# adobe-research/DiffusionHandles

Measured on AMD Instinct MI355X. Metric: guided-denoise steps/sec at 512x512 (SD2-depth), higher is better.
Workload: dtype f16; 1 GPU; single 512x512 edit per GPU, SD2-depth (865.9M params, seeded random weights), guided phase: 3 x (fwd + energy + bwd-to-latent) + CFG fwd (B=2) + DDIM step; resolution=512, edits_per_gpu=1, correspondences=24906, parallelism=independent edits, one process per GPU, no collectives

## Files before the change

diffusionhandles_amd/_lib.py:

```python
import ctypes
import os

import torch

_HERE = os.path.dirname(os.path.abspath(__file__))
LIB_PATH = os.environ.get("DIFFHANDLES_LIB") or os.path.join(_HERE, "libdiffhandles_hip.so")
_LIB = None

c_p = ctypes.c_void_p
c_i = ctypes.c_int
c_f = ctypes.c_float
c_d = ctypes.c_double
c_sz = ctypes.c_size_t


class UNetConfig(ctypes.Structure):
    _fields_ = [("in_channels", c_i), ("out_channels", c_i), ("n_levels", c_i),
                ("block_out_channels", c_i * 4), ("layers_per_block", c_i), ("heads", c_i * 4),
                ("cross_attention_dim", c_i), ("norm_groups", c_i), ("sample_size", c_i),
                ("text_len", c_i), ("max_batch", c_i), ("dtype", c_i), ("max_diff_batch", c_i)]


class VAEConfig(ctypes.Structure):
    _fields_ = [("latent_channels", c_i), ("out_channels", c_i), ("block_out_channels", c_i * 4),
# ... 46 lines not shown
    "dh_vae_decoder_create": (c_i, [c_p, ctypes.POINTER(c_p)]),
    "dh_vae_decoder_destroy": (None, [c_p]),
    "dh_vae_decoder_num_params": (c_i, [c_p]),
    "dh_vae_decoder_param_info": (c_i, [c_p, c_i, ctypes.POINTER(ctypes.c_char_p), ctypes.POINTER(c_i),
                                        ctypes.POINTER(ctypes.c_int64)]),
    "dh_vae_decoder_load_param": (c_i, [c_p, c_i, c_p, c_p]),
    "dh_vae_decoder_bytes": (c_sz, [c_p]),
    "dh_vae_decoder_decode": (c_i, [c_p, c_p, c_i, c_p, c_p]),
    "dh_vae_encoder_create": (c_i, [c_p, ctypes.POINTER(c_p)]),
    "dh_vae_encoder_encode": (c_i, [c_p, c_p, c_i, c_p, c_p]),
    "dh_text_encoder_create": (c_i, [c_p, ctypes.POINTER(c_p)]),
    "dh_text_encoder_destroy": (None, [c_p]),
    "dh_text_encoder_num_params": (c_i, [c_p]),
    "dh_text_encoder_param_info": (c_i, [c_p, c_i, ctypes.POINTER(ctypes.c_char_p), ctypes.POINTER(c_i),
                                         ctypes.POINTER(ctypes.c_int64)]),
    "dh_text_encoder_load_param": (c_i, [c_p, c_i, c_p, c_p]),
    "dh_text_encoder_bytes": (c_sz, [c_p]),
    "dh_text_encoder_encode": (c_i, [c_p, c_p, c_i, c_i, c_p, c_p]),
    "dh_gemm_profile_begin": (c_i, []),
    "dh_gemm_profile_end": (c_i, [ctypes.POINTER(c_d), ctypes.POINTER(ctypes.c_int64), ctypes.POINTER(c_d)]),
    "dh_gemm_profile_bytes": (c_i, [ctypes.POINTER(c_d)]),
    "dh_ddim_cfg_step": (c_i, [c_p, c_p, c_p, c_p, c_f, c_f, c_f, c_i, c_p]),
    "dh_latent_update": (c_i, [c_p, c_p, c_p, c_f, c_f, c_i, c_p]),
    "dh_adam_step": (c_i, [c_p, c_p, c_p, c_p, c_f, c_f, c_f, c_f, c_i, c_i, c_p]),
    "dh_mse_fwd_bwd": (c_i, [c_p, c_p, c_i, c_p, c_p, c_p]),
    "dh_latent_update_strided": (c_i, [c_p, c_p, c_p, c_i, c_i, c_f, c_f, c_i, c_p]),
    "dh_pack_sample": (c_i, [c_p, c_p, c_i, c_i, c_p, c_i, c_i, c_i, c_i, c_p]),
    "dh_unet_io_ptr": (c_i, [c_p, c_i, c_i, ctypes.POINTER(c_p), ctypes.POINTER(c_sz)]),
    "dh_mse_cotangent": (c_i, [c_p, c_p, c_i, c_f, c_f, c_p, c_p, c_p, c_p]),
    "dh_adam_step_scaled": (c_i, [c_p, c_p, c_p, c_p, c_p, c_f, c_f, c_f, c_f, c_i, c_i, c_p]),
    "dh_mse_cotangent_batch": (c_i, [c_p, c_p, c_i, c_i, c_f, c_f, c_d, c_p, c_p, c_p, c_p, c_p, c_p]),
    "dh_adam_step_scaled_batch": (c_i, [c_p, c_p, c_p, c_p, c_p, c_p, c_f, c_f, c_f, c_f, c_i, c_i, c_i, c_p]),
    "dh_latent_update_guarded": (c_i, [c_p, c_p, c_p, c_i, c_i, c_f, c_i, c_i, c_p, c_i, c_i, c_p, c_p, c_i, c_i, c_p]),
    "dh_ddim_cfg_step_flagged": (c_i, [c_p, c_p, c_p, c_p, c_f, c_f, c_f, c_i, c_i, c_p, c_i, c_i, c_p]),
}

c_l = ctypes.c_long
DEBUG_SIGNATURES = {
    "dh_dbg_gemm": (c_i, [c_i, c_p, c_l, c_p, c_i, c_i, c_i, c_i, c_i, c_i, c_i, c_i, c_i, c_i, c_i, c_p, c_p, c_i, c_i,
                          c_p, c_l, c_p, c_l, c_i, c_p, c_sz, c_p]),
    "dh_dbg_gemm_groupnorm": (c_i, [c_i, c_p, c_l, c_p, c_i, c_i, c_i, c_i, c_i, c_i, c_i, c_p, c_p, c_p, c_sz, c_i, c_i, c_p, c_p, c_f, c_i,
                                    c_p, c_p, c_p, ctypes.POINTER(c_i), c_p]),
    "dh_dbg_gemm_groupnorm_bwd": (c_i, [c_i, c_p, c_l, c_p, c_i, c_i, c_i, c_i, c_i, c_i, c_i, c_p, c_p, c_sz, c_i, c_i, c_p, c_p, c_p, c_p, c_i,
                                        c_p, c_p, ctypes.POINTER(c_i), c_p]),
    "dh_dbg_gemm_groupnorm_res": (c_i, [c_i, c_p, c_l, c_p, c_i, c_i, c_i, c_i, c_i, c_i, c_i, c_p, c_p, c_l, c_p, c_p, c_sz, c_i, c_i, c_p, c_p,
                                    c_f, c_i, c_p, c_p, c_p, ctypes.POINTER(c_i), c_p]),
    "dh_dbg_gemm_groupnorm_bwd_res": (c_i, [c_i, c_p, c_l, c_p, c_i, c_i, c_i, c_i, c_i, c_i, c_i, c_p, c_l, c_p, c_p, c_sz, c_i, c_i, c_p, c_p, c_p,
                                        c_p, c_i, c_p, c_p, ctypes.POINTER(c_i), c_p]),
    "dh_dbg_concat_groupnorm": (c_i, [c_i, c_p, c_i, c_p, c_i, c_p, c_i, c_i, c_i, c_p, c_p, c_f, c_i, c_p, c_p, c_p, c_p]),
    "dh_dbg_gemm_last_tile": (c_i, [ctypes.POINTER(c_i)]),
    "dh_dbg_unet_concat_ops": (c_i, [ctypes.POINTER(UNetConfig), ctypes.POINTER(c_i), c_i, ctypes.POINTER(c_i)]),
    "dh_dbg_gemm_lnfold": (c_i, [c_i, c_p, c_l, c_p, c_i, c_i, c_i, c_p, c_p, c_p, c_f, c_p, c_l, c_p]),
    "dh_dbg_gemm_glu": (c_i, [c_i, c_i, c_p, c_l, c_p, c_i, c_i, c_i, c_p, c_p, c_p, c_p, c_p, c_p]),
    "dh_dbg_gemm_family": (c_i, [c_i]),
    "dh_dbg_gemm_stage": (c_i, [c_i]),
    "dh_dbg_gemm_pp_variant": (c_i, [c_i, c_p]),
    "dh_dbg_gemm_pp_ablate": (c_i, [c_i]),
    "dh_dbg_gemm_pp_persist": (c_i, [c_i]),
    "dh_dbg_gemm_pp_glu": (c_i, [c_i]),
    "dh_dbg_gemm_pp_plan": (c_i, [c_i, c_i, c_i, c_i, c_i, c_i, c_sz, ctypes.POINTER(c_i), ctypes.POINTER(c_i), ctypes.POINTER(c_i)]),
    "dh_dbg_touch_tiled": (c_i, [c_sz, c_p]),
    "dh_dbg_groupnorm": (c_i, [c_i, c_p, c_p, c_p, c_p, c_p, c_p, c_p, c_p, c_i, c_i, c_i, c_i, c_f, c_i, c_i, c_p]),
    "dh_dbg_layernorm": (c_i, [c_i, c_p, c_p, c_p, c_p, c_p, c_p, c_p, c_p, c_i, c_i, c_f, c_p]),
    "dh_dbg_geglu": (c_i, [c_i, c_p, c_p, c_p, c_p, c_i, c_i, c_p]),
    "dh_dbg_attention": (c_i, [c_i, c_p, c_l, c_p, c_p, c_l, c_p, c_l, c_p, c_p, c_p, c_p, c_p, c_p, c_i, c_i, c_i, c_i, c_p]),
    "dh_dbg_attention_bwd_pair": (c_i, [c_i, c_p, c_l, c_p, c_p, c_l, c_p, c_l, c_p, c_p, c_p, c_p, c_p, c_p, c_i, c_i, c_i, c_i, c_p, c_p]),
    "dh_dbg_pool2x2": (c_i, [c_i, c_p, c_p, c_i, c_i, c_i, c_i, c_i, c_p]),
    "dh_dbg_ellipse_offsets": (c_i, [c_i, ctypes.POINTER(ctypes.c_int32), c_i, ctypes.POINTER(c_i)]),
    "dh_dbg_lane_ops": (c_i, [c_p, c_p, c_p, c_p]),
}


def lib():
    global _LIB
    if _LIB is None:
        if not os.path.exists(LIB_PATH):
            raise RuntimeError(
                f"native HIP library not found at {LIB_PATH}; build it with "
                "`python -c 'import __graft_entry__ as g; g.build()'` (there is no CPU fallback)")
        handle = ctypes.CDLL(LIB_PATH)
        missing = []
        for name, (res, args) in list(SIGNATURES.items()) + list(DEBUG_SIGNATURES.items()):
            try:
                fn = getattr(handle, name)
            except AttributeError:
                missing.append(name)
                continue
            fn.restype = res
            fn.argtypes = args
        handle.dh_missing_symbols = missing
        for env, fn in (("DH_GEMM_FAMILY", "dh_dbg_gemm_family"), ("DH_PP_GLU", "dh_dbg_gemm_pp_glu"),
                        ("DH_PP_PERSIST", "dh_dbg_gemm_pp_persist"), ("DH_GEMM_STAGE", "dh_dbg_gemm_stage")):
            if os.environ.get(env) and fn not in missing:
                getattr(handle, fn)(int(os.environ[env]))
        _LIB = handle
    return _LIB


def check(rc, what=""):
    if rc != 0:
        raise RuntimeError(f"{what} failed ({rc}): {lib().dh_last_error().decode()}")


def require_gpu(t=None):
    if not torch.cuda.is_available():
        raise RuntimeError("diffusionhandles_amd needs a HIP device (MI355X); there is no CPU fallback")
# ... 15 lines not shown
```

diffusionhandles_amd/csrc/debug_api.cpp:

```cpp
#include <stdlib.h>

#include "unet_kernels.h"
using namespace dh;

static void* g_dbg_tiled = nullptr;

__global__ void k_dbg_touch(const uint4* p, size_t n16, unsigned* sink) {
  unsigned acc = 0;
  for (size_t i = (size_t)blockIdx.x * blockDim.x + threadIdx.x; i < n16; i += (size_t)gridDim.x * blockDim.x) { const uint4 v = p[i]; acc ^= v.x ^ v.y ^ v.z ^ v.w; }
  if (acc == 0x9e3779b9u && sink) sink[0] = acc;
}
extern "C" int dh_dbg_touch_tiled(size_t bytes, void* stream) {
  DH_REQUIRE(g_dbg_tiled != nullptr, "no tiled weights yet (call dh_dbg_gemm first)");
  hipLaunchKernelGGL(k_dbg_touch, dim3(512), dim3(256), 0, (hipStream_t)stream, (const uint4*)g_dbg_tiled, bytes / 16, (unsigned*)nullptr);
  DH_LAUNCH_CHECK();
  return DH_OK;
}

extern "C" int dh_dbg_gemm(int dtype, const void* A, long lda, const void* W, int M, int N, int K, int mode, int Hin,
                           int Win, int Cin, int Hout, int Wout, int stride, int up, const float* bias,
                           const float* rowvec, int rowvec_ld, int rows_per_batch, const void* R, long ldr, void* C,
                           long ldc, int act_silu, float* partial, size_t partial_elems, void* stream) {
  DH_REQUIRE(A && W && C && K % 64 == 0 && N % 64 == 0, "bad arguments (N, K must be multiples of 64)");
  void*& tiled = g_dbg_tiled;
// ... 83 lines not shown
                                         const float* gamma, const float* beta, const float* stats, int silu, void* dx,
                                         float* scratch, int* have_out, void* stream) {
  return dh_dbg_gemm_groupnorm_bwd_res(dtype, A, lda, W, M, N, K, mode, Hin, Win, Cin, nullptr, N, C, partial, partial_elems, HW, G, x,
                                       gamma, beta, stats, silu, dx, scratch, have_out, stream);
}
extern "C" int dh_dbg_concat_groupnorm(int dtype, const void* a, int Ca, const void* b, int Cb, void* out, int B, int HW, int G,
                                       const float* gamma, const float* beta, float eps, int silu, void* Y, float* stats,
                                       float* scratch, void* stream) {
  DH_REQUIRE(a && b && out && Y && stats && scratch && gamma && beta && B > 0 && HW > 0 && G > 0, "bad arguments");
  DH_REQUIRE(Ca % 8 == 0 && Cb % 8 == 0 && (Ca + Cb) % G == 0 && (GN_GB * ((Ca + Cb) / G)) % 8 == 0 && GN_GB * ((Ca + Cb) / G) <= 2048,
             "shape the fused concatenation does not take");
  launch_concat_gn(dtype, a, Ca, b, Cb, out, scratch, B, HW, G, (hipStream_t)stream);
  launch_groupnorm_fwd(dtype, out, gamma, beta, Y, stats, scratch, B, HW, Ca + Cb, G, eps, silu, (hipStream_t)stream, 1);
  DH_LAUNCH_CHECK();
  return DH_OK;
}
extern "C" int dh_dbg_gemm_lnfold(int dtype, const void* A, long lda, const void* W, int M, int N, int K, const float* ln_s,
                                  const float* ln_t, float* ln_stats, float ln_eps, void* C, long ldc, void* stream) {
  DH_REQUIRE(A && W && C && ln_s && ln_t && ln_stats && K % 64 == 0 && N % 64 == 0, "bad arguments (N, K must be multiples of 64)");
  static void* tiled = nullptr;
  static size_t tiled_cap = 0;
  const size_t need = (size_t)N * K * 2;
  if (need > tiled_cap) {
    if (tiled) (void)hipFree(tiled);
    DH_CHECK_HIP(hipMalloc(&tiled, need));
    tiled_cap = need;
  }
  launch_tile_weights(dtype, W, tiled, N, K, (hipStream_t)stream);
  GemmArgs g;
  g.A = A; g.lda = lda; g.W = tiled; g.M = M; g.N = N; g.K = K; g.mode = A_DENSE; g.C = C; g.ldc = ldc;
  g.ln_s = ln_s; g.ln_t = ln_t; g.ln_stats = ln_stats; g.ln_eps = ln_eps;
  launch_gemm(dtype, g, (hipStream_t)stream);
  DH_LAUNCH_CHECK();
  return DH_OK;
}
extern "C" int dh_dbg_gemm_glu(int dtype, int bwd, const void* A, long lda, const void* W, int M, int N, int K, const float* bias,
                               void* C, void* y, const void* x, void* dx, void* stream) {
  DH_REQUIRE(A && W && K % 64 == 0 && N % 128 == 0, "bad arguments (K % 64, N % 128)");
  DH_REQUIRE(bwd ? (x && dx) : (y != nullptr), "missing output");
  static void* tiled = nullptr;
  static size_t tiled_cap = 0;
  const size_t need = (size_t)N * K * 2;
  if (need > tiled_cap) {
    if (tiled) (void)hipFree(tiled);
    DH_CHECK_HIP(hipMalloc(&tiled, need));
    tiled_cap = need;
  }
  launch_tile_weights(dtype, W, tiled, N, K, (hipStream_t)stream);
  GemmArgs g;
  g.A = A; g.lda = lda; g.W = tiled; g.M = M; g.N = N; g.K = K; g.mode = A_DENSE; g.bias = bias;
  if (bwd) { g.glub_x = x; g.glub_dx = dx; }
  else { g.C = C; g.ldc = N; g.glu_y = y; g.glu_ldy = N / 2; }
  launch_gemm(dtype, g, (hipStream_t)stream);
  DH_LAUNCH_CHECK();
  return DH_OK;
}
extern "C" int dh_dbg_groupnorm(int dtype, const void* x, const float* gamma, const float* beta, void* y, float* stats,
                                const void* dy, void* dx, float* scratch, int B, int HW, int C, int G, float eps,
                                int silu, int accumulate, void* stream) {
  launch_groupnorm_fwd(dtype, x, gamma, beta, y, stats, scratch, B, HW, C, G, eps, silu, (hipStream_t)stream);
  if (dy && dx)
    launch_groupnorm_bwd(dtype, x, dy, gamma, beta, stats, dx, scratch, B, HW, C, G, silu, accumulate, (hipStream_t)stream);
  DH_LAUNCH_CHECK();
  return DH_OK;
}
extern "C" int dh_dbg_layernorm(int dtype, const void* x, const float* gamma, const float* beta, void* y, float* stats,
                                const void* dy, const void* add, void* dx, int rows, int C, float eps, void* stream) {
  launch_layernorm_fwd(dtype, x, gamma, beta, y, stats, rows, C, eps, (hipStream_t)stream);
  if (dy && dx) launch_layernorm_bwd(dtype, x, dy, gamma, stats, add, dx, rows, C, (hipStream_t)stream);
  DH_LAUNCH_CHECK();
  return DH_OK;
}
extern "C" int dh_dbg_geglu(int dtype, const void* x, void* y, const void* dy, void* dx, int rows, int F, void* stream) {
  launch_geglu_fwd(dtype, x, y, rows, F, (hipStream_t)stream);
  if (dy && dx) launch_geglu_bwd(dtype, x, dy, dx, rows, F, (hipStream_t)stream);
  DH_LAUNCH_CHECK();
  return DH_OK;
}
extern "C" int dh_dbg_attention(int dtype, const void* q, long ldq, const void* k, const void* v, long ldk, void* o,
                                long ldo, float* lse, const void* d_o, float* delta, void* dq, void* dk, void* dv,
                                int B, int H, int Nq, int Nk, void* stream) {
  hipStream_t st = (hipStream_t)stream;
  launch_attention_fwd(dtype, q, ldq, k, v, ldk, o, ldo, lse, B, H, Nq, Nk, st);
  if (d_o) {
    if (dq) launch_attention_bwd_dq(dtype, q, ldq, k, v, ldk, o, ldo, d_o, ldo, lse, delta, dq, ldq, B, H, Nq, Nk, st);
    else launch_attention_delta(dtype, o, ldo, d_o, ldo, delta, B, H, Nq, st);
    if (dk && dv) {
      static float* scratch = nullptr;
      constexpr size_t kScratch = (size_t)16 << 20;
      if (!scratch && hipMalloc((void**)&scratch, kScratch * sizeof(float)) != hipSuccess) scratch = nullptr;
      launch_attention_bwd_dkv(dtype, q, ldq, k, v, ldk, d_o, ldo, lse, delta, dk, dv, ldk, B, H, Nq, Nk, st, scratch,
                               scratch ? kScratch : 0);
    }
  }
  DH_LAUNCH_CHECK();
  return DH_OK;
}
extern "C" int dh_dbg_attention_bwd_pair(int dtype, const void* q, long ldq, const void* k, const void* v, long ldk, const void* o,
                                         long ldo, const float* lse, const void* d_o, float* delta, void* dq, void* dk, void* dv,
                                         int B, int H, int Nq, int Nk, void* stream, void* stream2) {
  hipStream_t st = (hipStream_t)stream, s2 = (hipStream_t)stream2;
  if (!s2) {
    launch_attention_bwd_dq(dtype, q, ldq, k, v, ldk, o, ldo, d_o, ldo, lse, delta, dq, ldq, B, H, Nq, Nk, st);
    launch_attention_bwd_dkv(dtype, q, ldq, k, v, ldk, d_o, ldo, lse, delta, dk, dv, ldk, B, H, Nq, Nk, st, nullptr, 0);
  } else {
    static hipEvent_t fork = nullptr, join = nullptr;
// ... 23 lines not shown
```

diffusionhandles_amd/csrc/gemm.hip:

```cpp
#include <stdlib.h>

#include <vector>

#include <hip/hip_ext.h>

#include "gemm_k.h"

namespace dh {

struct GemmProf {
  bool on = false;
  std::vector<hipEvent_t> ev;
  size_t used = 0;
  double flops = 0;
  double bytes = 0;
  hipEvent_t e0 = nullptr, e1 = nullptr;
};
static GemmProf g_prof;
static int g_buf_stage = 1;
static int g_pp_force = 0;
struct GemmTileReport {
  int bm, bn, kg, stages, mw, splits, pp, gn_epi, reduce_gn;
};
static thread_local GemmTileReport g_last_tile;
// ... 295 lines not shown
          sy = ty >> 1; sx = tx >> 1;
        }
        sy = sy < 0 ? 0 : (sy >= p.Hin ? p.Hin - 1 : sy);
        sx = sx < 0 ? 0 : (sx >= p.Win ? p.Win - 1 : sx);
        const T* ptr = Ag + (a_off[j] + (long)sy * p.Win + sx) * p.lda + c0 + lchunk * 8;
        dma16(ok ? ptr : zero, sbase + (j * WG + grp) * (NWV * 1024));
      }
    } else {
      const int j = q - NPA;
#ifdef DH_TUNING
      if (p.w_nt) dma16_nt(b_ptr[j] + (size_t)(k0 >> 6) * 4096, sbase + BM * 128 + (j * WG + grp) * (NWV * 1024));
      else
#endif
      dma16(b_ptr[j] + (size_t)(k0 >> 6) * 4096, sbase + BM * 128 + (j * WG + grp) * (NWV * 1024));
    }
  };
  auto next_tile = [&]() {
    if constexpr (BUF && MODE == GM_CONV_S1) {
      ++tap; ++bs_kx;
      const bool row_end = bs_kx == 3;
      bs_tap += row_end ? bs_step_row : bs_step_px;
      bs_kx = row_end ? 0 : bs_kx;
      if (tap == 9) { tap = 0; c0 += BK; bs_tap = (unsigned)c0 * 2u; }
      bs_sh = 31u - (unsigned)tap;
      return;
    }
    if (MODE != GM_DENSE) { if (++tap == 9) { tap = 0; c0 += BK; } }
  };
  auto issue = [&](int kt, int stage) {
#pragma unroll
    for (int q = 0; q < NP; ++q) issue_piece(kt, stage, q);
    next_tile();
  };

  v16f acc[TM][TN];
#pragma unroll
  for (int i = 0; i < TM; ++i)
#pragma unroll
    for (int j = 0; j < TN; ++j)
#pragma unroll
      for (int r = 0; r < 16; ++r) acc[i][j][r] = 0.f;

  const int wn_u = __builtin_amdgcn_readfirstlane(wn);
  float ln1[TM], ln2[TM];
#pragma unroll
  for (int i = 0; i < TM; ++i) { ln1[i] = 0.f; ln2[i] = 0.f; }

#pragma unroll
  for (int s = 0; s < ST - 1; ++s)
    if (s < ntiles) issue(s, s);
  DH_STAMP(1);

  constexpr bool PRE = TM * TN <= 8;
  const bool pre_r = PRE && p.R != nullptr && p.pre_r && p.splits == 1 && (WG == 1 || grp == 0) && (KG == 1 || kg == 0);
  constexpr bool PRE_B = PRE && !(MW == 2 && BN == 320) && WNS == 2;
  const bool pre_b = PRE_B && p.bias != nullptr && p.pre_r && p.splits == 1;
  float4 bpre[PRE_B ? TN : 1][4];
  if (pre_b) {
#pragma unroll
    for (int j = 0; j < TN; ++j)
#pragma unroll
      for (int g = 0; g < 4; ++g) {
        const int n = n0 + wn * CPW + j * 32 + 8 * g + 4 * hi;
        bpre[PRE_B ? j : 0][g] = n < p.N ? *reinterpret_cast<const float4*>(p.bias + n) : make_float4(0.f, 0.f, 0.f, 0.f);
      }
  }
  constexpr bool PRE_LN = LNF && PRE && !(MW == 2 && BM == 256);
  float4 lsp[PRE_LN ? TN : 1][4], ltp[PRE_LN ? TN : 1][4];
  if (PRE_LN) {
#pragma unroll
    for (int j = 0; j < TN; ++j)
#pragma unroll
      for (int g = 0; g < 4; ++g) {
        const int n = n0 + wn * CPW + j * 32 + 8 * g + 4 * hi;
        lsp[PRE_LN ? j : 0][g] = n < p.N ? *reinterpret_cast<const float4*>(p.ln_s + n) : make_float4(0.f, 0.f, 0.f, 0.f);
        ltp[PRE_LN ? j : 0][g] = n < p.N ? *reinterpret_cast<const float4*>(p.ln_t + n) : make_float4(0.f, 0.f, 0.f, 0.f);
      }
  }
  constexpr bool GNB = gn_epi_bwd_tile(BM, BN, WG, GLU, LNF);
  static_assert(!GNB || (PRE && WNS == 2), "the backward form carries the GroupNorm input tile in the residual's prefetch registers");
  const bool gnb = GNB && p.gn_epi == 2 && p.splits == 1;
  const bool pre_x = gnb && (KG == 1 || kg == 0);
  float4 gnb_col = make_float4(0.f, 0.f, 0.f, 0.f);
  if (GNB && pre_x && tid < BN) {
    const int n = n0 + tid, grp_n = (int)(((float)n + 0.5f) / (float)p.gn_cpg);
    const float2 st2 = *reinterpret_cast<const float2*>(p.gnb_stats + 2 * ((m0 / p.gn_HW) * p.gn_G + grp_n));
    gnb_col = make_float4(p.gnb_gamma[n], p.gnb_beta[n], st2.x, st2.y);
  }
  uint2 rpre[TM][TN][4];
  if (pre_r || pre_x) {
    const T* rsrc = reinterpret_cast<const T*>(pre_x ? p.gnb_x : p.R);
    const long rld = pre_x ? p.gnb_ldx : p.ldr;
#pragma unroll
    for (int i = 0; i < TM; ++i) {
      const int m = m0 + wm * RPW + i * 32 + ln;
#pragma unroll
      for (int j = 0; j < TN; ++j)
#pragma unroll
        for (int g = 0; g < 4; ++g) {
          const int n = n0 + wn * CPW + j * 32 + 8 * g + 4 * hi;
          rpre[i][j][g] = (m < p.M && n < p.N) ? *reinterpret_cast<const uint2*>(rsrc + (size_t)m * rld + n) : make_uint2(0, 0);
        }
    }
  }

  constexpr int KK = BK / 16 / WG;
  const int kk0 = grp * KK;
// ... 132 lines not shown
          acc[i][j][4 * g + 2] = rstd * (acc[i][j][4 * g + 2] - mean * sv.z) + tv.z;
          acc[i][j][4 * g + 3] = rstd * (acc[i][j][4 * g + 3] - mean * sv.w) + tv.w;
        }
    }
  }


  if constexpr (GLU == 1) {
    typedef T T4 __attribute__((ext_vector_type(4)));
    const bool hb = p.bias != nullptr;
    T* Y = reinterpret_cast<T*>(p.glu_y);
#pragma unroll
    for (int i = 0; i < TM; ++i) {
      const int m = m0 + wm * RPW + i * 32 + ln;
      if (m >= p.M) continue;
#pragma unroll
      for (int j = 0; j < TN; ++j) {
        const int nb = n0 + wn * CPW + j * 32;
        if (nb >= p.N) continue;
        uint2 w[4];
        float pv[4][4];
#pragma unroll
        for (int g = 0; g < 4; ++g) {
          float v0 = acc[i][j][4 * g], v1 = acc[i][j][4 * g + 1], v2 = acc[i][j][4 * g + 2], v3 = acc[i][j][4 * g + 3];
          if (hb) {
            float4 b = bpre[PRE_B ? j : 0][g];
            if (!pre_b) b = *reinterpret_cast<const float4*>(p.bias + nb + 8 * g + 4 * hi);
            v0 += b.x; v1 += b.y; v2 += b.z; v3 += b.w;
          }
          T4 o;
          o[0] = from_f32<T>(v0); o[1] = from_f32<T>(v1); o[2] = from_f32<T>(v2); o[3] = from_f32<T>(v3);
          w[g] = __builtin_bit_cast(uint2, o);
#pragma unroll
          for (int c = 0; c < 4; ++c) pv[g][c] = to_f32<T>(o[c]);
        }
        if (p.C) {
          T* out = reinterpret_cast<T*>(p.C) + (size_t)m * p.ldc + nb + 8 * hi;
          *reinterpret_cast<uint4*>(out) = half_exchange(w[0], w[1]);
          *reinterpret_cast<uint4*>(out + 16) = half_exchange(w[2], w[3]);
        }
        uint2 y[2];
#pragma unroll
        for (int q = 0; q < 2; ++q) {
          T4 o;
#pragma unroll
          for (int c = 0; c < 4; ++c) o[c] = from_f32<T>(pv[q][c] * gelu_f(pv[q + 2][c]));
          y[q] = __builtin_bit_cast(uint2, o);
        }
        *reinterpret_cast<uint4*>(Y + (size_t)m * p.glu_ldy + (nb >> 1) + 8 * hi) = half_exchange(y[0], y[1]);
      }
    }
    return;
  }
  if constexpr (GLU == 2) {
    typedef T T4 __attribute__((ext_vector_type(4)));
    const T* X = reinterpret_cast<const T*>(p.glub_x);
    T* DX = reinterpret_cast<T*>(p.glub_dx);
    const size_t ldx = 2 * (size_t)p.N;
    uint4 Hc[TM][TN][2], Gc[TM][TN][2];
#pragma unroll
    for (int i = 0; i < TM; ++i) {
      const int m = m0 + wm * RPW + i * 32 + ln;
      const int mc = m < p.M ? m : p.M - 1;
#pragma unroll
      for (int j = 0; j < TN; ++j) {
        int nb = n0 + wn * CPW + j * 32;
        if (nb >= p.N) nb = 0;
#pragma unroll
        for (int q = 0; q < 2; ++q) {
          const T* src = X + (size_t)mc * ldx + 2 * nb + 32 * q + 8 * hi;
          Hc[i][j][q] = *reinterpret_cast<const uint4*>(src);
          Gc[i][j][q] = *reinterpret_cast<const uint4*>(src + 16);
        }
      }
    }
#pragma unroll
    for (int i = 0; i < TM; ++i) {
      const int m = m0 + wm * RPW + i * 32 + ln;
      if (m >= p.M) continue;
#pragma unroll
      for (int j = 0; j < TN; ++j) {
        const int nb = n0 + wn * CPW + j * 32;
        if (nb >= p.N) continue;
#pragma unroll
        for (int q = 0; q < 2; ++q) {
          const uint4 hc = Hc[i][j][q], gc = Gc[i][j][q];
          const uint4 hx = half_exchange(make_uint2(hc.x, hc.y), make_uint2(hc.z, hc.w));
          const uint4 gx = half_exchange(make_uint2(gc.x, gc.y), make_uint2(gc.z, gc.w));
          uint2 dh[2], dg[2];
#pragma unroll
          for (int s2 = 0; s2 < 2; ++s2) {
            const int g = 2 * q + s2;
            const T4 hh = __builtin_bit_cast(T4, s2 ? make_uint2(hx.z, hx.w) : make_uint2(hx.x, hx.y));
            const T4 gg = __builtin_bit_cast(T4, s2 ? make_uint2(gx.z, gx.w) : make_uint2(gx.x, gx.y));
            T4 oh, og;
#pragma unroll
            for (int c = 0; c < 4; ++c) {
              const float dy = acc[i][j][4 * g + c], gate = to_f32<T>(gg[c]);
              const GeluParts gp = gelu_parts(gate);
              oh[c] = from_f32<T>(dy * gate * gp.Phi);
              og[c] = from_f32<T>(dy * to_f32<T>(hh[c]) * fmaf(gate, gp.pdf, gp.Phi));
            }
            dh[s2] = __builtin_bit_cast(uint2, oh);
            dg[s2] = __builtin_bit_cast(uint2, og);
          }
          T* dst = DX + (size_t)m * ldx + 2 * nb + 32 * q + 8 * hi;
          *reinterpret_cast<uint4*>(dst) = half_exchange(dh[0], dh[1]);
          *reinterpret_cast<uint4*>(dst + 16) = half_exchange(dg[0], dg[1]);
        }
      }
    }
    return;
  }
  DH_STAMP(5);
  constexpr bool GNE = gn_epi_fwd_tile(BN, GLU, LNF);
  const bool gn_epi = GNE && p.splits == 1 && (p.gn_epi == 1 || (GNB && p.gn_epi == 2));
  static_assert(!GNE || NWV * CPW * 4 <= KG * ST * STAGE - 4096, "the pivot table lies below the column-sum scratch");
  float* gpt = reinterpret_cast<float*>(smem_all) + wave * CPW;
  if (GNE && gn_epi && !(GNB && gnb)) __syncthreads();
  float gsa[GNE ? TN : 1][16], gsq[GNE ? TN : 1][16];
  if (GNE) {
#pragma unroll
    for (int j = 0; j < (GNE ? TN : 1); ++j)
#pragma unroll
      for (int r = 0; r < 16; ++r) { gsa[j][r] = 0.f; gsq[j][r] = 0.f; }
  }
  auto gn_acc = [&](int i, int j, int g, uint2 packed) {
    if constexpr (GNE) {
      typedef T T4g __attribute__((ext_vector_type(4)));
      const T4g ov = __builtin_bit_cast(T4g, packed);
      float v[4], pv[4];
#pragma unroll
      for (int c = 0; c < 4; ++c) v[c] = to_f32<T>(ov[c]);
      float4* pt = reinterpret_cast<float4*>(gpt + j * 32 + 8 * g + 4 * hi);
      if (i == 0) {
#pragma unroll
// ... 422 lines not shown
  } else if (gm == GM_CONV_S1) {
    DH_GEMM_LAUNCH((k_gemm_dma<T, BM, BN, ST, GM_CONV_S1, 0, WG, KG, MW, false, 0, BUF>));
  } else {
    DH_GEMM_LAUNCH((k_gemm_dma<T, BM, BN, ST, GM_GENERIC, 0, WG, KG, MW>));
  }
}
template <class T, int BM, int BN, int ST, int WG, int KG, int MW>
static void launch_tile(int gm, bool lnf, dim3 grid, hipStream_t st, const GemmK& k, int glu = 0) {
  g_last_tile.bm = BM; g_last_tile.bn = BN; g_last_tile.kg = KG; g_last_tile.stages = ST; g_last_tile.mw = MW;
  if (k.pp_a_bytes != 0 && gm != GM_GENERIC) launch_tile_b<T, BM, BN, ST, WG, KG, MW, true>(gm, lnf, grid, st, k, glu);
  else launch_tile_b<T, BM, BN, ST, WG, KG, MW, false>(gm, lnf, grid, st, k, glu);
}
#undef DH_GEMM_LAUNCH

#ifdef DH_TUNING
#define DH_KNOB(name, env, dflt) static const int name = getenv(env) ? atoi(getenv(env)) : (dflt)
#else
#define DH_KNOB(name, env, dflt) constexpr int name = (dflt)
#endif

template <class T>
static void gemm_dispatch(GemmK k, size_t partial_elems, hipStream_t st, int* gn_done, int* lnb_done, int dtype) {
  DH_KNOB(kSplitTiles, "DH_SPLITK_TILES", 200);
  DH_KNOB(kSplitMinK, "DH_SPLITK_MINKT", 32);
  DH_KNOB(kSplitTarget, "DH_SPLITK_TARGET", 256);
  DH_KNOB(kBigTiles, "DH_BIG_TILES", 128);
  DH_KNOB(kNarrowTiles, "DH_NARROW_TILES", 40);
  DH_KNOB(kN320, "DH_GEMM_N320", 224);
  DH_KNOB(kMwBlocks, "DH_GEMM_MW", 64);
  DH_KNOB(kKg2MinKt, "DH_KG2_MINKT", 4);
  DH_KNOB(kManyBlocks, "DH_GEMM_MANY", 512);
  DH_KNOB(kMw128, "DH_GEMM_MW128", 1);
  DH_KNOB(kTwoPerCu, "DH_GEMM_TWO_PER_CU", 1);
#ifdef DH_TUNING
  DH_KNOB(kWnt, "DH_W_NT", 0);
#endif
  const bool lnf = k.ln_s != nullptr;
  g_last_tile = GemmTileReport{};
  int BM = 128, BN = (k.N % 128 == 0) ? 128 : 64;
  const int ktiles = k.K / BK;
  PpPlan pp;
  const bool use_pp = gemm_pp_plan(k, partial_elems, g_pp_force, &pp);
  if (BN == 128 && ktiles >= 16 && cdiv(k.M, 128) * cdiv(k.N, 128) <= kNarrowTiles) BN = 64;
  if (k.M <= 64 || (cdiv(k.M, 128) * cdiv(k.N, BN) < kBigTiles && ktiles < kSplitMinK)) { BM = 64; BN = 64; }
  const bool n320 = kN320 > 0 && k.N % 320 == 0 && k.N <= 960 && !lnf && BM == 128 && BN == 64 && cdiv(k.M, 128) >= kN320;
  if (n320) BN = 320;
  DH_KNOB(kMwShortK, "DH_GEMM_MW_SHORTK", 128);
  const long tiles256 = (long)cdiv(k.M, 256) * cdiv(k.N, 128);
  const bool mw2 = kMwBlocks > 0 && k.N % 128 == 0 && tiles256 >= kMwBlocks &&
                   !(k.M <= 256 && k.M > 128 && cdiv(k.N, 128) < 128) && (tiles256 >= kMwShortK || ktiles >= kSplitMinK);
  if (mw2) { BM = 256; BN = 128; }
  const int glu = k.glu_y ? 1 : (k.glub_x ? 2 : 0);
  if (glu && !(BM == 64 && BN == 64)) { BM = mw2 ? 256 : 128; BN = 128; }
  DH_KNOB(kT160, "DH_GEMM_T160", 224);
  const long tiles160 = (long)cdiv(k.M, 128) * (k.N / 160);
  const bool t160 = kT160 > 0 && k.N % 160 == 0 && !lnf && !glu && !n320 && BM != 64 && tiles160 >= kT160 && tiles160 <= 256;
  if (t160) { BM = 128; BN = 160; }
  if (use_pp) { BM = pp.bm; BN = pp.bn; }
  const int tm = cdiv(k.M, BM), tn = cdiv(k.N, BN), tiles = tm * tn;
  int splits = 1;
  if (use_pp) splits = pp.splits;
  else if (k.partial && !lnf && !glu && tiles < kSplitTiles && ktiles >= kSplitMinK) {
    splits = kSplitTarget / tiles;
    if (splits > ktiles / 4) splits = ktiles / 4;
    if (splits > 32) splits = 32;
    const size_t fit = partial_elems / ((size_t)k.M * k.N);
    if ((size_t)splits > fit) splits = (int)fit;
    if (splits < 1) splits = 1;
  }
#ifdef DH_TUNING
  static const int kLog = getenv("DH_GEMM_LOG") ? atoi(getenv("DH_GEMM_LOG")) : 0;
  const int kForceTile = getenv("DH_FORCE_TILE") ? atoi(getenv("DH_FORCE_TILE")) : 0;
  const int kForceSplits = getenv("DH_FORCE_SPLITS") ? atoi(getenv("DH_FORCE_SPLITS")) : 0;
  int force_tile = 0;
  if (kForceTile && !use_pp && !(k.glu_y || k.glub_x)) {
    const int fbm = kForceTile == 1 ? 64 : (kForceTile == 6 ? 256 : 128), fbn = kForceTile == 7 ? 160 : ((kForceTile <= 3) ? 64 : 128);
    if ((k.N % fbn == 0 || fbn == 64) && !(fbn == 160 && lnf)) { BM = fbm; BN = fbn; force_tile = kForceTile; }
  }
  if (kForceSplits && !use_pp && k.partial && !lnf) {
    splits = kForceSplits;
    if (splits > ktiles / 2) splits = ktiles / 2 > 0 ? ktiles / 2 : 1;
    const size_t fit = partial_elems / ((size_t)k.M * k.N);
    if ((size_t)splits > fit) splits = (int)fit;
    if (splits < 1) splits = 1;
  }
  if (kLog) fprintf(stderr, "GEMMLOG M=%d N=%d K=%d mode=%d lnf=%d gn=%d gnb=%d bias=%d R=%d rowvec=%d | pp=%d BM=%d BN=%d splits=%d\n", k.M, k.N, k.K,
                    k.mode == A_DENSE ? 0 : (k.mode == A_CONV3 && k.stride == 1 && k.up == 0 ? 1 : 2), (int)lnf, k.gn_part != nullptr,
                    k.gnb_x != nullptr, k.bias != nullptr, k.R != nullptr, k.rowvec != nullptr, (int)use_pp, BM, BN, splits);
#endif
  const int tiles_per_split = cdiv(ktiles, splits);
  splits = cdiv(ktiles, tiles_per_split);
  k.splits = splits;
  k.k_per_split = tiles_per_split * BK;
  k.gn_epi = 0; k.gn_cpg = 0;
  if ((g_buf_stage & 4) == 0 && splits == 1 && !use_pp && gn_epi_fwd_tile(BN, glu, lnf) && k.gn_part && !k.gnb_x && gn_done && k.gn_G > 0 &&
      k.gn_HW > 0 && k.C && k.wide_store && k.M % k.gn_HW == 0 && k.gn_HW % BM == 0 && k.N % k.gn_G == 0 && k.N % BN == 0) {
    const int cpg = k.N / k.gn_G, sx = 2 * (k.gn_HW / BM);
    if (cpg >= 8 && cpg <= BN && sx <= 64) { k.gn_epi = 1; k.gn_cpg = cpg; k.gn_S = sx; }
  }
  if ((g_buf_stage & 8) == 0 && splits == 1 && !use_pp && gn_epi_bwd_tile(BM, BN, 1, glu, lnf) && k.gn_part && k.gnb_x && gn_done && k.gn_G > 0 &&
      k.gn_HW > 0 && k.C && k.wide_store && k.pre_r && !k.R && !k.bias && !k.rowvec && !k.act_silu && k.M % k.gn_HW == 0 && k.gn_HW % BM == 0 &&
      k.N % k.gn_G == 0 && k.N % BN == 0 && (((size_t)k.gnb_x | (size_t)(k.gnb_ldx * 2)) & 7) == 0) {
    const int cpg = k.N / k.gn_G, sx = 2 * (k.gn_HW / BM);
    if (cpg >= 8 && cpg <= BN && sx <= 64) { k.gn_epi = 2; k.gn_cpg = cpg; k.gn_S = sx; }
  }
#ifdef DH_TUNING
  k.w_nt = kWnt > 0 && tm <= kWnt;
  static const int kLnfAbl = getenv("DH_LNF_ABL") ? atoi(getenv("DH_LNF_ABL")) : 0;
  k.lnf_abl = kLnfAbl;
  k.ts = g_gemm_ts;
#endif
#ifdef DH_TUNING
  dim3 grid(force_tile ? cdiv(k.M, BM) : tm, force_tile ? cdiv(k.N, BN) : tn, splits);
#else
  dim3 grid(tm, tn, splits);
#endif
  hipEvent_t e0 = nullptr, e1 = nullptr;
  if (g_prof.on) {
    if (g_prof.used + 2 > g_prof.ev.size()) {
      const size_t old = g_prof.ev.size();
      g_prof.ev.resize(old + 4096);
      for (size_t i = old; i < g_prof.ev.size(); ++i) (void)hipEventCreate(&g_prof.ev[i]);
    }
    e0 = g_prof.ev[g_prof.used++];
    e1 = g_prof.ev[g_prof.used++];
    g_prof.flops += 2.0 * (double)k.M * (double)k.N * (double)k.K;
    const double esz = 2.0;
    double a_elems = (double)k.M * k.K;
    if (k.mode != A_DENSE && k.Hout > 0 && k.Wout > 0) a_elems = (double)k.M / ((double)k.Hout * k.Wout) * k.Hin * k.Win * k.Cin;
    double c_elems = (double)k.M * k.N * (k.C ? 1.0 : 0.0) + (k.R ? (double)k.M * k.N : 0.0);
    if (k.glu_y) c_elems += 0.5 * (double)k.M * k.N;
    if (k.glub_x) c_elems += 4.0 * (double)k.M * k.N;
    if (k.gn_epi == 2) c_elems += (double)k.M * k.N;
    g_prof.bytes += esz * (a_elems + (double)k.N * k.K + c_elems);
    g_prof.e0 = e0; g_prof.e1 = e1;
  }
  int gm = GM_GENERIC;
  if (k.mode == A_DENSE) gm = GM_DENSE;
  else if (k.mode == A_CONV3 && k.stride == 1 && k.up == 0 && k.pad == 1) gm = GM_CONV_S1;
  if (!use_pp) {
    k.pp_a_bytes = 0; k.pp_w_bytes = 0;
    size_t ab = 0;
    if (k.mode == A_DENSE) ab = ((size_t)(k.M - 1) * k.lda + k.K) * 2;
    else if (k.Hout > 0 && k.Wout > 0 && k.M % (k.Hout * k.Wout) == 0)
      ab = (size_t)(k.M / (k.Hout * k.Wout)) * k.Hin * k.Win * (size_t)k.lda * 2;
    const size_t wb = (size_t)align_up((size_t)k.N, 64) * k.K * 2;
    const bool conv_ok = k.mode == A_DENSE || (k.Cin % 64 == 0 && k.K == 9 * k.Cin);
    if ((g_buf_stage & 1) && ab > 0 && conv_ok && ab + (size_t)(k.Win + 1) * k.lda * 2 < 0x7ff00000ull && wb < 0x7ff00000ull && k.lda % 8 == 0 &&
        ((size_t)k.A & 15) == 0 && ((size_t)k.W & 15) == 0) {
      k.pp_a_bytes = (unsigned)ab; k.pp_w_bytes = (unsigned)wb;
    }
  }
#ifdef DH_TUNING
  static const int kAbl = getenv("DH_GEMM_ABLATE") ? atoi(getenv("DH_GEMM_ABLATE")) : 0;
  if (kAbl == 1 && BM == 128 && BN == 128) { hipLaunchKernelGGL((k_gemm_dma<T, 128, 128, 4, GM_CONV_S1, 1>), grid, dim3(256), 0, st, k); }
  else if (kAbl == 2 && BM == 128 && BN == 128) { hipLaunchKernelGGL((k_gemm_dma<T, 128, 128, 4, GM_CONV_S1, 2>), grid, dim3(256), 0, st, k); }
  else if (kAbl == 3 && BM == 128 && BN == 128) { hipLaunchKernelGGL((k_gemm_dma<T, 128, 128, 4, GM_DENSE, 1>), grid, dim3(256), 0, st, k); }
  else if (kAbl == 1 && mw2 && gm == GM_CONV_S1) { hipLaunchKernelGGL((k_gemm_dma<T, 256, 128, 3, GM_CONV_S1, 1, 1, 1, 2>), grid, dim3(512), 0, st, k); }
  else if (kAbl == 2 && mw2 && gm == GM_CONV_S1) { hipLaunchKernelGGL((k_gemm_dma<T, 256, 128, 3, GM_CONV_S1, 2, 1, 1, 2>), grid, dim3(512), 0, st, k); }
  else if (kAbl == 1 && mw2 && gm == GM_DENSE && !lnf) { hipLaunchKernelGGL((k_gemm_dma<T, 256, 128, 3, GM_DENSE, 1, 1, 1, 2>), grid, dim3(512), 0, st, k); }
  else if (kAbl == 2 && mw2 && gm == GM_DENSE && !lnf) { hipLaunchKernelGGL((k_gemm_dma<T, 256, 128, 3, GM_DENSE, 2, 1, 1, 2>), grid, dim3(512), 0, st, k); }
  else if (force_tile == 1) launch_tile<T, 64, 64, 4, 1, 1, 1>(gm, lnf, grid, st, k);
  else if (force_tile == 2) launch_tile<T, 128, 64, 3, 1, 2, 1>(gm, lnf, grid, st, k);
  else if (force_tile == 3) launch_tile<T, 128, 64, 5, 1, 1, 1>(gm, lnf, grid, st, k);
  else if (force_tile == 4) launch_tile<T, 128, 128, 4, 1, 1, 2>(gm, lnf, grid, st, k);
  else if (force_tile == 5) launch_tile<T, 128, 128, 4, 1, 1, 1>(gm, lnf, grid, st, k);
  else if (force_tile == 6) launch_tile<T, 256, 128, 3, 1, 1, 2>(gm, lnf, grid, st, k);
  else if (force_tile == 7) launch_tile<T, 128, 160, 4, 1, 1, 1>(gm, false, grid, st, k);
  else
#endif
  if (use_pp) { pp.splits = splits; g_last_tile.bm = pp.bm; g_last_tile.bn = pp.bn; launch_gemm_pp(dtype, k, pp, st, g_prof.e0, g_prof.e1); }
  else if (t160) launch_tile<T, 128, 160, 4, 1, 1, 1>(gm, false, grid, st, k);
  else if (mw2) launch_tile<T, 256, 128, 3, 1, 1, 2>(gm, lnf, grid, st, k, glu);
  else if (BM == 128 && BN == 128 && (glu || (kMw128 && tiles_per_split >= kMw128))) launch_tile<T, 128, 128, 4, 1, 1, 2>(gm, lnf, grid, st, k, glu);
  else if (kTwoPerCu && BM == 128 && BN == 64 && tiles * splits > 256 && tiles * splits <= 512)
    launch_tile<T, 128, 64, 3, 1, 1, 1>(gm, lnf, grid, st, k);
  else if (BM == 128 && BN == 64 && tiles_per_split >= kKg2MinKt) launch_tile<T, 128, 64, 3, 1, 2, 1>(gm, lnf, grid, st, k);
  else if (BN == 320) launch_tile<T, 128, 320, 2, 1, 1, 2>(gm, false, grid, st, k);
  else if (BM == 64) launch_tile<T, 64, 64, 4, 1, 1, 1>(gm, lnf, grid, st, k, glu);
  else if (BN == 128 && kManyBlocks > 0 && tiles * splits >= kManyBlocks) launch_tile<T, 128, 128, 2, 1, 1, 1>(gm, lnf, grid, st, k);
  else if (BN == 128) launch_tile<T, 128, 128, 4, 1, 1, 1>(gm, lnf, grid, st, k);
  else launch_tile<T, 128, 64, 5, 1, 1, 1>(gm, lnf, grid, st, k);
  g_prof.e0 = g_prof.e1 = nullptr;
  g_last_tile.splits = splits; g_last_tile.pp = use_pp ? 1 : 0; g_last_tile.gn_epi = k.gn_epi;
  if (k.gn_epi) *gn_done = k.gn_S;
  if (splits > 1) {
    if (k.gn_part && k.gn_G > 0 && k.gn_HW > 0 && k.N % k.gn_G == 0 && (GN_GB * (k.N / k.gn_G)) % 8 == 0 &&
        GN_GB * (k.N / k.gn_G) <= 2048 && k.M % k.gn_HW == 0) {
      k.gn_S = gn_slices(k.gn_HW, k.M / k.gn_HW);
      if (k.gnb_x) hipLaunchKernelGGL((k_splitk_reduce_gn<T, true>), dim3(k.gn_S, cdiv(k.gn_G, GN_GB), k.M / k.gn_HW), dim3(256), 0, st, k);
      else hipLaunchKernelGGL((k_splitk_reduce_gn<T, false>), dim3(k.gn_S, cdiv(k.gn_G, GN_GB), k.M / k.gn_HW), dim3(256), 0, st, k);
      g_last_tile.reduce_gn = 1;
      if (gn_done) *gn_done = 1;
    } else if (k.lnb_x && lnb_done && !k.bias && !k.rowvec && !k.R && !k.act_silu && k.N % 8 == 0 && k.ldc == k.N) {
      launch_splitk_reduce_ln_bwd(dtype, k.partial, splits, k.lnb_x, k.lnb_gamma, k.lnb_stats, k.lnb_add, k.lnb_dx, k.M, k.N, st);
      *lnb_done = 1;
    } else {
      const size_t groups = (size_t)k.M * k.N / 4;
      hipLaunchKernelGGL((k_splitk_reduce<T>), dim3((unsigned)((groups + 255) / 256)), dim3(256), 0, st, k);
    }
  }
}
#undef DH_KNOB

double launch_gemm(int dtype, const GemmArgs& a, hipStream_t st) {
  GemmK k;
  k.A = a.A; k.lda = a.lda; k.W = a.W; k.M = a.M; k.N = a.N; k.K = a.K;
  k.mode = a.mode; k.Hin = a.Hin; k.Win = a.Win; k.Cin = a.Cin; k.Hout = a.Hout; k.Wout = a.Wout;
  k.stride = a.stride; k.up = a.up; k.pad = a.pad;
  k.bias = a.bias; k.rowvec = a.rowvec; k.rowvec_ld = a.rowvec_ld;
  k.rows_per_batch = a.rows_per_batch > 0 ? a.rows_per_batch : 1;
  k.inv_rows_per_batch = 1.f / (float)k.rows_per_batch;
  k.R = a.R; k.ldr = a.ldr; k.C = a.C; k.ldc = a.ldc; k.act_silu = a.act_silu;
  k.partial = a.partial; k.splits = 1; k.k_per_split = a.K;
  k.pre_r = 1;
  k.wide_store = a.N % 32 == 0 && a.ldc % 8 == 0 && ((size_t)a.C & 15) == 0;
  k.ln_s = a.ln_s; k.ln_t = a.ln_t; k.ln_stats = a.ln_stats; k.ln_eps = a.ln_eps;
  k.gn_part = a.gn_part; k.gn_HW = a.gn_HW; k.gn_G = a.gn_G; k.gn_S = 0;
  k.gnb_x = a.gnb_x; k.gnb_ldx = a.gnb_ldx; k.gnb_gamma = a.gnb_gamma; k.gnb_beta = a.gnb_beta; k.gnb_stats = a.gnb_stats;
  k.gnb_silu = a.gnb_silu;
  k.lnb_x = a.lnb_x; k.lnb_gamma = a.lnb_gamma; k.lnb_stats = a.lnb_stats; k.lnb_add = a.lnb_add; k.lnb_dx = a.lnb_dx;
  k.glu_y = a.glu_y; k.glu_ldy = a.glu_ldy; k.glub_x = a.glub_x; k.glub_dx = a.glub_dx;
  if (a.gn_done) *a.gn_done = 0;
  if (a.lnb_done) *a.lnb_done = 0;
  if (dtype == DH_DTYPE_F16) gemm_dispatch<f16>(k, a.partial_elems, st, a.gn_done, a.lnb_done, dtype);
  else gemm_dispatch<bf16>(k, a.partial_elems, st, a.gn_done, a.lnb_done, dtype);
  return 2.0 * (double)a.M * (double)a.N * (double)a.K;
}

}

#ifdef DH_TUNING
extern "C" int dh_dbg_gemm_timeline(unsigned long long* ts) { dh::g_gemm_ts = ts; return DH_OK; }
#endif

extern "C" int dh_dbg_gemm_family(int force) {
  DH_REQUIRE(force >= 0 && force <= 2, "family: 0 policy, 1 k_gemm_dma, 2 k_gemm_pp");
  dh::g_pp_force = force;
  return DH_OK;
}

extern "C" int dh_dbg_gemm_stage(int buf) {
  dh::g_buf_stage = buf;
  return DH_OK;
}

extern "C" int dh_dbg_gemm_last_tile(int* out) {
  DH_REQUIRE(out != nullptr, "null pointer");
  const dh::GemmTileReport& r = dh::g_last_tile;
  const int v[9] = {r.bm, r.bn, r.kg, r.stages, r.mw, r.splits, r.pp, r.gn_epi, r.reduce_gn};
  for (int i = 0; i < 9; ++i) out[i] = v[i];
  return DH_OK;
}

extern "C" int dh_gemm_profile_begin(void) {
  dh::g_prof.on = true;
  dh::g_prof.used = 0;
  dh::g_prof.flops = 0;
  dh::g_prof.bytes = 0;
  return DH_OK;
}
extern "C" int dh_gemm_profile_bytes(double* bytes) {
  if (bytes) *bytes = dh::g_prof.bytes;
  return DH_OK;
}
extern "C" int dh_gemm_profile_end(double* ms_total, int64_t* launches, double* flops) {
  using namespace dh;
  g_prof.on = false;
  double ms = 0;
  if (g_prof.used >= 2) DH_CHECK_HIP(hipEventSynchronize(g_prof.ev[g_prof.used - 1]));
  for (size_t i = 0; i + 1 < g_prof.used; i += 2) {
    float t = 0;
    DH_CHECK_HIP(hipEventElapsedTime(&t, g_prof.ev[i], g_prof.ev[i + 1]));
    ms += t;
  }
// ... 6 lines not shown
```

diffusionhandles_amd/csrc/gemm_k.h:

```cpp
#pragma once
#include "unet_kernels.h"

namespace dh {

typedef _Float16 v8h __attribute__((ext_vector_type(8)));
typedef __bf16 v8b __attribute__((ext_vector_type(8)));
typedef float v16f __attribute__((ext_vector_type(16)));

template <class T> struct Mfma;
template <> struct Mfma<f16> {
  static __device__ __forceinline__ v16f run(uint4 a, uint4 b, v16f c) {
    return __builtin_amdgcn_mfma_f32_32x32x16_f16(__builtin_bit_cast(v8h, a), __builtin_bit_cast(v8h, b), c, 0, 0, 0);
  }
};
template <> struct Mfma<bf16> {
  static __device__ __forceinline__ v16f run(uint4 a, uint4 b, v16f c) {
    return __builtin_amdgcn_mfma_f32_32x32x16_bf16(__builtin_bit_cast(v8b, a), __builtin_bit_cast(v8b, b), c, 0, 0, 0);
  }
};

struct GemmK {
  const void* A; long lda;
  const void* W;
  int M, N, K;
  int mode, Hin, Win, Cin, Hout, Wout, stride, up, pad;
  const float* bias;
  const float* rowvec; int rowvec_ld; int rows_per_batch; float inv_rows_per_batch;
  const void* R; long ldr;
  void* C; long ldc;
  int act_silu;
  int pre_r;
  int wide_store;
#ifdef DH_TUNING
  int w_nt;
  unsigned long long* ts;
  int lnf_abl;
#endif
  const float* ln_s; const float* ln_t; float* ln_stats; float ln_eps;
  float* partial;
  int splits, k_per_split;
  float* gn_part; int gn_HW, gn_G, gn_S;
  int gn_epi, gn_cpg;
  const void* gnb_x; long gnb_ldx; const float *gnb_gamma, *gnb_beta, *gnb_stats; int gnb_silu;
  const void* lnb_x; const float *lnb_gamma, *lnb_stats; const void* lnb_add; void* lnb_dx;
  void* glu_y; long glu_ldy; const void* glub_x; void* glub_dx;
  int pp_tm, pp_tn, pp_order, pp_nwork; unsigned pp_a_bytes, pp_w_bytes;
  unsigned long long* pp_ts;
};


struct PpPlan { int bm = 0, bn = 0, splits = 1; };
bool gemm_pp_plan(const GemmK& k, size_t partial_elems, int force, PpPlan* plan);
void launch_gemm_pp(int dtype, const GemmK& k, const PpPlan& plan, hipStream_t st, hipEvent_t e0, hipEvent_t e1);

}
```

diffusionhandles_amd/csrc/gemm_pp.hip:

```cpp
#include <hip/hip_ext.h>

#include <type_traits>
#include <utility>

#include "gemm_k.h"

namespace dh {

typedef float v4f __attribute__((ext_vector_type(4)));
typedef int v4i __attribute__((ext_vector_type(4)));
typedef unsigned lane_u2p __attribute__((ext_vector_type(2)));

template <class T> struct Mfma16;
template <> struct Mfma16<f16> {
  typedef v8h frag;
  static __device__ __forceinline__ v4f run(frag a, frag b, v4f c) { return __builtin_amdgcn_mfma_f32_16x16x32_f16(a, b, c, 0, 0, 0); }
};
template <> struct Mfma16<bf16> {
  typedef v8b frag;
  static __device__ __forceinline__ v4f run(frag a, frag b, v4f c) { return __builtin_amdgcn_mfma_f32_16x16x32_bf16(a, b, c, 0, 0, 0); }
};

constexpr unsigned PP_OOB = 0x80000000u;

// ... 497 lines not shown
        *reinterpret_cast<uint2*>(ctail) = __builtin_bit_cast(uint2, o);
      }
      __builtin_amdgcn_sched_barrier(0);
      stamp();
    }
  };
  if (has_r) { if (hv_rows) rows(std::true_type{}, std::true_type{}); else rows(std::true_type{}, std::false_type{}); }
  else       { if (hv_rows) rows(std::false_type{}, std::true_type{}); else rows(std::false_type{}, std::false_type{}); }
  {
    constexpr int CPR = CPW / 8, NCH = RPW * CPR;
    static_assert(NCH % 64 == 0, "whole store instructions");
    T* cw = reinterpret_cast<T*>(p.C) + (size_t)(m0 + wm * RPW) * p.ldc + nb;
    const int mleft = p.M - (m0 + wm * RPW);
#pragma unroll
    for (int k = 0; k < NCH / 64; ++k) {
      const int c = 64 * k + lane_e, row = c / CPR, cc = c - row * CPR;
      const uint4 v = *reinterpret_cast<const uint4*>(stg + row * SPITCH + cc * 16);
      if (row < mleft) *reinterpret_cast<uint4*>(cw + (size_t)row * p.ldc + cc * 8) = v;
    }
  }
  stamp();
  }
}

static int pp_mode(const GemmK& k) {
  if (k.mode == A_DENSE) return PP_DENSE;
  if (k.mode == A_CONV3 && k.stride == 1 && k.up == 0 && k.pad == 1) return PP_CONV_S1;
  return PP_GENERIC;
}

static size_t pp_a_bytes(const GemmK& k) {
  if (k.mode == A_DENSE) return ((size_t)(k.M - 1) * k.lda + k.K) * 2;
  const size_t B = (size_t)k.M / ((size_t)k.Hout * k.Wout);
  return B * k.Hin * k.Win * (size_t)k.lda * 2;
}

static int pp_device_cus() {
  static int cus = 0;
  if (cus == 0) {
    int dev = 0, n = 0;
    if (hipGetDevice(&dev) == hipSuccess && hipDeviceGetAttribute(&n, hipDeviceAttributeMultiprocessorCount, dev) == hipSuccess && n >= 8) cus = n - n % 8;
    else { (void)hipGetLastError(); cus = 256; }
  }
  return cus;
}

static int g_pp_glu = -1;
bool gemm_pp_plan(const GemmK& k, size_t partial_elems, int force, PpPlan* plan) {
  if (force == 1) return false;
  if (k.ln_s || k.act_silu) return false;
  const int glu = k.glu_y ? 1 : (k.glub_x ? 2 : 0);
  const bool glu_here = force == 2 || g_pp_glu > 0 || (g_pp_glu < 0 && ((glu == 1 && k.M >= 2048) || k.M >= 32768));
  if (glu && !glu_here) return false;
  if (glu && (k.mode != A_DENSE || k.N % 128 || k.rowvec || k.R || (glu == 1 && (k.glu_ldy % 8 || ((size_t)k.glu_y & 15))) ||
              (glu == 2 && (((size_t)k.glub_x & 15) || ((size_t)k.glub_dx & 15))))) return false;
  if (k.rowvec && (k.rowvec_ld % 4 || ((size_t)k.rowvec & 15))) return false;
  if (k.K % 64 || k.M <= 0 || (!k.C && !glu)) return false;
  if (k.N % 160 && k.N % 128) return false;
  if (k.N % 64) return false;
  if (k.bias && ((size_t)k.bias & 15)) return false;
  if ((k.C && (k.ldc % 8 || ((size_t)k.C & 15))) || k.lda % 8 || ((size_t)k.A & 15) || ((size_t)k.W & 15)) return false;
  if (k.R && (k.ldr % 8 || ((size_t)k.R & 15))) return false;
  if (k.mode != A_DENSE && (k.Hout <= 0 || k.Wout <= 0 || k.M % (k.Hout * k.Wout) || k.Cin % 64 || k.K != 9 * k.Cin)) return false;
  const size_t ab = pp_a_bytes(k) + (size_t)(k.Win + 1) * k.lda * 2, wb = (size_t)k.N * k.K * 2;
  if (ab >= 0x7ff00000ull || wb >= 0x7ff00000ull) return false;
  const int ktiles = k.K / 64;
  const int bn = (k.N % 160 == 0 && !glu) ? 160 : 128;
  const int tn = k.N / bn;
  const long t256 = (long)cdiv(k.M, 256) * tn, t128 = (long)cdiv(k.M, 128) * tn;
  int bm = 0, splits = 1;
  const int cus = pp_device_cus(), fill = cus - cus / 8;
  if (t256 >= fill) bm = 256;
  else if (t128 >= fill) bm = 128;
  else if (!glu && k.partial && ktiles >= 64 && t256 >= 64 && k.M >= 1024 && k.M <= 4096) {
    bm = 256;
    splits = (int)(cus / t256);
    if (splits > ktiles / 8) splits = ktiles / 8;
    if (splits > 8) splits = 8;
    const size_t fit = partial_elems / ((size_t)k.M * k.N);
    if ((size_t)splits > fit) splits = (int)fit;
    if (splits < 2) bm = 0;
  }
  if (force == 2 && bm == 0) { bm = k.M > 128 ? 256 : 128; splits = 1; }
  if (bm == 0) return false;
  plan->bm = bm; plan->bn = bn; plan->splits = splits;
  return true;
}

constexpr int PP_SHIP_256 = PPV_K64 | (1 << PPV_NDIM_SHIFT), PP_SHIP_128 = PPV_K64 | (3 << PPV_NDIM_SHIFT);
static int g_pp_persist = 1;
static int g_pp_ablate = 0;
static int g_pp_variant = -1;
static unsigned long long* g_pp_ts = nullptr;

template <class T, int BM, int BN, int NST, int VAR>
static void pp_launch_tile(int mode, dim3 grid, hipStream_t st, const GemmK& k, hipEvent_t e0, hipEvent_t e1) {
#define DH_PP_LAUNCH(KERNEL)                                                                      \
  do {                                                                                            \
    if (e0) hipExtLaunchKernelGGL(KERNEL, grid, dim3(512), 0, st, e0, e1, 0, k);                  \
    else hipLaunchKernelGGL(KERNEL, grid, dim3(512), 0, st, k);                                   \
  } while (0)
  if constexpr (BN == 128 && VAR == (BM == 256 ? PP_SHIP_256 : PP_SHIP_128)) {
    if (k.glu_y) { DH_PP_LAUNCH((k_gemm_pp<T, BM, BN, PP_DENSE, NST, VAR, 1>)); return; }
    if (k.glub_x) { DH_PP_LAUNCH((k_gemm_pp<T, BM, BN, PP_DENSE, NST, VAR, 2>)); return; }
  }
  if (mode == PP_DENSE) DH_PP_LAUNCH((k_gemm_pp<T, BM, BN, PP_DENSE, NST, VAR>));
// ... 103 lines not shown
```

diffusionhandles_amd/csrc/unet_engine.cpp:

```cpp
#include <stdlib.h>

#include <algorithm>
#include <map>
#include <numeric>
#include <vector>

#include "unet_kernels.h"

namespace dh {

enum OpType { OP_CONV_IN, OP_CONV_OUT, OP_GEMM, OP_GN, OP_LN, OP_ATTN, OP_GEGLU, OP_CONCAT, OP_TIMESTEP, OP_T2F };
enum ParamKind { PK_F32, PK_MAT };

struct Ten {
  size_t off = 0, goff = 0;
  size_t off_fo = 0;
  int rows = 0, C = 0;
  bool req_grad = true;
  bool persistent = false;
};

struct Wt {
  size_t fwd_off = 0, bwd_off = 0;
  int N = 0, K = 0, taps = 1;
  bool has_bwd = true, f32 = false;
  int glu_F = 0;
};

struct ParamInfo {
  std::string name;
  int ndim = 0;
  int64_t shape[4] = {0, 0, 0, 0};
  int kind = PK_F32;
  size_t f32_off = 0;
  int wt = -1;
  int row_off = 0;
  int glu_F = 0;
};

struct Op {
  int type = OP_GEMM;
  int in0 = -1, in1 = -1, out = -1, res = -1;
  int wt = -1;
  long bias_off = -1;
  long gamma_off = -1, beta_off = -1;
  int mode = A_DENSE, Hin = 0, Win = 0, Cin = 0, Hout = 0, Wout = 0, stride = 1, up = 0;
  int in_col = 0, in_cols = 0;
  long rowvec_off = -1; int rowvec_ld = 0;
  int act_silu = 0;
  float eps = 1e-5f; int silu = 0; int groups = 32; size_t stats_off = 0;
  int heads = 0, Nq = 0, Nk = 0, cross = 0, kv_col = 0; size_t lse_off = 0;
  int gn_next = -1;
  int ln_fold = -1, folded = 0;
  long ln_s_off = -1, ln_t_off = -1;
  int glu_op = -1, glub_op = -1;
};

}

using namespace dh;

struct dh_unet {
  dh_unet_config cfg;
  int dtype = DH_DTYPE_F16;
  std::vector<Ten> tens;
  std::vector<Wt> wts;
  std::vector<ParamInfo> params;
  std::vector<Op> ops;
  std::map<std::string, int> pindex;
  size_t w16_elems = 0, pf_elems = 0, act_elems = 0, grad_elems = 0, f32_elems = 0;
  size_t fo_elems = 0;
  size_t partial_elems = 0, scratch_elems = 0, small_elems = 0;
  unsigned short *w16 = nullptr, *act = nullptr, *grad = nullptr, *scratch = nullptr;
  float *pf = nullptr, *f32a = nullptr, *partial = nullptr, *small = nullptr;
  int t_text = -1, t_kv = -1, t_conv_in_out = -1, t_final = -1, act_ids[3] = {-1, -1, -1};
  int act_op_end[3] = {0, 0, 0};
  int first_cross_op = 0;
  int saved_ops = 0;
  int temb_ops = 0, temb_rows = 0;
  float temb_t = 0.f;
  hipStream_t temb_stream = nullptr;
  uint64_t text_key = 0, kv_key = 0;
  int kv_rows = 0;
  hipStream_t kv_stream = nullptr;
  long temb_f32_off = -1;
  int temb_total = 0, kv_total = 0;
  float *in_sample = nullptr, *in_text = nullptr, *io_eps = nullptr, *out_dsample = nullptr, *out_dtext = nullptr, *t_dev = nullptr;
  std::map<uint64_t, hipGraphExec_t> graphs;
  std::map<uint64_t, double> graph_flops;
  bool use_graphs = true;
  long ones_off = -1, zeros_off = -1;
  bool fold_dirty = true;
  bool owns_weights = true;
  int n_shared = 0;
  int saved_batch = 0;
  const float* saved_sample = nullptr;
  std::vector<char> gready;
  double flops_fwd = 0, flops_bwd = 0;
  int64_t launches = 0;

  bool fo_mode = false;
  unsigned short* aptr(int t, int B_unused = 0) { return act + (fo_mode && !tens[t].persistent ? tens[t].off_fo : tens[t].off); }
  std::vector<int> galias;
  unsigned short* gptr(int t) {
    while (galias[t] != t) t = galias[t];
    return grad + tens[t].goff;
  }
};

namespace {

struct Builder {
  dh_unet& u;
  int maxB, maxBd;
  explicit Builder(dh_unet& uu) : u(uu), maxB(uu.cfg.max_batch), maxBd(uu.cfg.max_diff_batch) {}

  int tensor(int rows, int C, bool req_grad = true) {
    Ten t;
    t.rows = rows; t.C = C; t.req_grad = req_grad;
    u.tens.push_back(t);
    return (int)u.tens.size() - 1;
  }
  size_t f32_slot(size_t n) { size_t o = u.f32_elems; u.f32_elems += align_up(n, 64); return o; }

  long param_f32(const std::string& name, int n) {
    ParamInfo p;
    p.name = name; p.ndim = 1; p.shape[0] = n; p.kind = PK_F32;
    p.f32_off = u.pf_elems;
    u.pf_elems += align_up((size_t)n, 64);
    u.pindex[name] = (int)u.params.size();
    u.params.push_back(p);
    return (long)p.f32_off;
  }
  void param_f32_at(const std::string& name, int n, size_t off) {
    ParamInfo p;
    p.name = name; p.ndim = 1; p.shape[0] = n; p.kind = PK_F32; p.f32_off = off;
    u.pindex[name] = (int)u.params.size();
    u.params.push_back(p);
  }
  int weight(int N, int K, int taps = 1, bool has_bwd = true, bool f32 = false) {
    Wt w;
    w.N = N; w.K = K; w.taps = taps; w.has_bwd = has_bwd; w.f32 = f32;
    size_t& arena = f32 ? u.pf_elems : u.w16_elems;
    w.fwd_off = arena; arena += align_up((size_t)N * K, 128);
    if (has_bwd) { w.bwd_off = arena; arena += align_up((size_t)N * K, 128); }
    u.wts.push_back(w);
    return (int)u.wts.size() - 1;
  }
  void bind_mat(const std::string& name, int wt, int rows, int row_off, int cin, int taps) {
    ParamInfo p;
    p.name = name; p.kind = PK_MAT; p.wt = wt; p.row_off = row_off;
    if (taps == 9) { p.ndim = 4; p.shape[0] = rows; p.shape[1] = cin; p.shape[2] = 3; p.shape[3] = 3; }
    else { p.ndim = 2; p.shape[0] = rows; p.shape[1] = cin; }
    u.pindex[name] = (int)u.params.size();
    u.params.push_back(p);
  }
  void bind_conv1x1(const std::string& name, int wt, int rows, int cin) {
    bind_mat(name, wt, rows, 0, cin, 1);
    ParamInfo& p = u.params.back();
    p.ndim = 4; p.shape[2] = 1; p.shape[3] = 1;
  }

  int gn(int x, const std::string& pre, float eps, bool silu) {
    const Ten tx = u.tens[x];
    Op o;
    o.type = OP_GN; o.in0 = x; o.out = tensor(tx.rows, tx.C);
    o.gamma_off = param_f32(pre + ".weight", tx.C);
    o.beta_off = param_f32(pre + ".bias", tx.C);
    o.eps = eps; o.silu = silu; o.groups = u.cfg.norm_groups;
    o.stats_off = f32_slot((size_t)maxB * o.groups * 2);
    u.ops.push_back(o);
    return o.out;
  }
  int ln(int x, const std::string& pre) {
    const Ten tx = u.tens[x];
    Op o;
    o.type = OP_LN; o.in0 = x; o.out = tensor(tx.rows, tx.C);
    o.gamma_off = param_f32(pre + ".weight", tx.C);
    o.beta_off = param_f32(pre + ".bias", tx.C);
    o.eps = 1e-5f;
    o.stats_off = f32_slot((size_t)maxB * tx.rows * 2);
    u.ops.push_back(o);
    return o.out;
  }
  int conv3(int x, const std::string& pre, int Cout, int Hs, int stride, int up, long temb_off, int res) {
    const Ten& tx = u.tens[x];
    const int Cin = tx.C;
    const int Hv = Hs << up, Ho = stride == 2 ? Hv / 2 : Hv;
    Op o;
    o.type = OP_GEMM; o.mode = A_CONV3; o.in0 = x; o.res = res;
    o.Hin = Hs; o.Win = Hs; o.Cin = Cin; o.Hout = Ho; o.Wout = Ho; o.stride = stride; o.up = up;
    o.wt = weight(Cout, 9 * Cin, 9);
    bind_mat(pre + ".weight", o.wt, Cout, 0, Cin, 9);
    o.bias_off = param_f32(pre + ".bias", Cout);
    if (temb_off >= 0) { o.rowvec_off = u.temb_f32_off + temb_off; o.rowvec_ld = u.temb_total; }
    o.out = tensor(Ho * Ho, Cout);
    u.ops.push_back(o);
    return o.out;
// ... 32 lines not shown
    g.ln_fold = li; l.folded = 1;
    g.ln_s_off = (long)u.pf_elems; u.pf_elems += align_up((size_t)N, 64);
    g.ln_t_off = (long)u.pf_elems; u.pf_elems += align_up((size_t)N, 64);
  }

  int temb_cursor = 0, kv_cursor = 0;
  int wt_temb = -1, wt_kv = -1;
  size_t temb_bias_off = 0;

  int resnet(int x, const std::string& pre, int Cout, int H) {
    const int Cin = u.tens[x].C;
    int h = gn(x, pre + ".norm1", 1e-5f, true);
    bind_mat(pre + ".time_emb_proj.weight", wt_temb, Cout, temb_cursor, u.cfg.block_out_channels[0] * 4, 1);
    param_f32_at(pre + ".time_emb_proj.bias", Cout, temb_bias_off + temb_cursor);
    const long toff = temb_cursor;
    temb_cursor += Cout;
    h = conv3(h, pre + ".conv1", Cout, H, 1, 0, toff, -1);
    h = gn(h, pre + ".norm2", 1e-5f, true);
    int sc = x;
    if (Cin != Cout) sc = linear(x, pre + ".conv_shortcut", Cout, true, -1, true);
    return conv3(h, pre + ".conv2", Cout, H, 1, 0, -1, sc);
  }

  int transformer(int x, const std::string& pre, int heads, int H) {
    const int C = u.tens[x].C, N = H * H;
    int h = gn(x, pre + ".norm", 1e-6f, false);
    int t0 = linear(h, pre + ".proj_in", C, true, -1);
    const std::string b = pre + ".transformer_blocks.0";
    int n1 = ln(t0, b + ".norm1");
    const int wqkv = weight(3 * C, C);
    bind_mat(b + ".attn1.to_q.weight", wqkv, C, 0, C, 1);
    bind_mat(b + ".attn1.to_k.weight", wqkv, C, C, C, 1);
    bind_mat(b + ".attn1.to_v.weight", wqkv, C, 2 * C, C, 1);
    int qkv = linear_w(n1, wqkv, -1, -1);
    fold_ln_into_last_gemm();
    Op a;
    a.type = OP_ATTN; a.in0 = qkv; a.heads = heads; a.Nq = N; a.Nk = N; a.cross = 0;
    a.out = tensor(N, C);
    a.lse_off = f32_slot((size_t)maxB * heads * N);
    u.ops.push_back(a);
    int t1 = linear(a.out, b + ".attn1.to_out.0", C, true, t0);
    int n2 = ln(t1, b + ".norm2");
    int q2 = linear(n2, b + ".attn2.to_q", C, false, -1);
    fold_ln_into_last_gemm();
    bind_mat(b + ".attn2.to_k.weight", wt_kv, C, kv_cursor, u.cfg.cross_attention_dim, 1);
    bind_mat(b + ".attn2.to_v.weight", wt_kv, C, kv_cursor + C, u.cfg.cross_attention_dim, 1);
    Op c;
    c.type = OP_ATTN; c.in0 = q2; c.in1 = u.t_kv; c.heads = heads; c.Nq = N; c.Nk = u.cfg.text_len; c.cross = 1;
    c.kv_col = kv_cursor;
    kv_cursor += 2 * C;
    c.out = tensor(N, C);
    c.lse_off = f32_slot((size_t)maxB * heads * N);
    u.ops.push_back(c);
    int t2 = linear(c.out, b + ".attn2.to_out.0", C, true, t1);
    int n3 = ln(t2, b + ".norm3");
    int gg = linear(n3, b + ".ff.net.0.proj", 8 * C, true, -1);
    fold_ln_into_last_gemm();
    const int ff1 = (int)u.ops.size() - 1;
    u.wts[u.ops[ff1].wt].glu_F = 4 * C;
    u.params[u.pindex[b + ".ff.net.0.proj.weight"]].glu_F = 4 * C;
    u.params[u.pindex[b + ".ff.net.0.proj.bias"]].glu_F = 4 * C;
    Op g;
    g.type = OP_GEGLU; g.in0 = gg; g.out = tensor(N, 4 * C);
    u.ops.push_back(g);
    u.ops[ff1].glu_op = (int)u.ops.size() - 1;
    int t3 = linear(g.out, b + ".ff.net.2", C, true, t2);
    u.ops.back().glub_op = u.ops[ff1].glu_op;
    return linear(t3, pre + ".proj_out", C, true, x);
  }
};

void count_fused(const dh_unet_config& c, int& temb_total, int& kv_total) {
  const int L = c.n_levels, n = c.layers_per_block;
  temb_total = 0; kv_total = 0;
  for (int i = 0; i < L; ++i) {
    temb_total += n * c.block_out_channels[i];
    if (i < L - 1) kv_total += n * 2 * c.block_out_channels[i];
  }
  temb_total += 2 * c.block_out_channels[L - 1];
  kv_total += 2 * c.block_out_channels[L - 1];
  for (int i = 0; i < L; ++i) {
    const int ch = c.block_out_channels[L - 1 - i];
    temb_total += (n + 1) * ch;
    if (i > 0) kv_total += (n + 1) * 2 * ch;
  }
}

static void layout_tensors(dh_unet& u);

int build(dh_unet& u) {
  const dh_unet_config& c = u.cfg;
  Builder b(u);
  const int L = c.n_levels, n = c.layers_per_block, S = c.sample_size;
  const int* ch = c.block_out_channels;
  const int temb_dim = ch[0] * 4;
  count_fused(c, u.temb_total, u.kv_total);

  int t_sin = b.tensor(1, ch[0], false);
  { Op o; o.type = OP_TIMESTEP; o.out = t_sin; u.ops.push_back(o); }
  const int w1 = b.weight(temb_dim, ch[0], 1, false);
  b.bind_mat("time_embedding.linear_1.weight", w1, temb_dim, 0, ch[0], 1);
  int e1 = b.linear_w(t_sin, w1, b.param_f32("time_embedding.linear_1.bias", temb_dim), -1, 0, 0, true, false);
  const int w2 = b.weight(temb_dim, temb_dim, 1, false);
  b.bind_mat("time_embedding.linear_2.weight", w2, temb_dim, 0, temb_dim, 1);
  int e2 = b.linear_w(e1, w2, b.param_f32("time_embedding.linear_2.bias", temb_dim), -1, 0, 0, true, false);
  b.wt_temb = b.weight(u.temb_total, temb_dim, 1, false);
  b.temb_bias_off = u.pf_elems;
  u.pf_elems += align_up((size_t)u.temb_total, 64);
  int t_temb = b.linear_w(e2, b.wt_temb, (long)b.temb_bias_off, -1, 0, 0, false, false);
  u.temb_f32_off = (long)b.f32_slot((size_t)c.max_batch * u.temb_total);
  { Op o; o.type = OP_T2F; o.in0 = t_temb; u.ops.push_back(o); }
  u.temb_ops = (int)u.ops.size();

  u.t_text = b.tensor(c.text_len, c.cross_attention_dim, true);
  b.wt_kv = b.weight(u.kv_total, c.cross_attention_dim);
  u.t_kv = b.linear_w(u.t_text, b.wt_kv, -1, -1);

  { Op o;
    o.type = OP_CONV_IN;
    o.wt = b.weight(ch[0], 9 * c.in_channels, 9, true, true);
    b.bind_mat("conv_in.weight", o.wt, ch[0], 0, c.in_channels, 9);
    o.bias_off = b.param_f32("conv_in.bias", ch[0]);
    o.Hin = S; o.Cin = c.in_channels;
    o.out = b.tensor(S * S, ch[0]);
    u.t_conv_in_out = o.out;
    u.ops.push_back(o); }
  int x = u.t_conv_in_out;
  std::vector<int> skips{x};
  int H = S;
  for (int i = 0; i < L; ++i) {
    const std::string pre = "down_blocks." + std::to_string(i);
    const bool attn = i < L - 1, down = i < L - 1;
    for (int j = 0; j < n; ++j) {
      x = b.resnet(x, pre + ".resnets." + std::to_string(j), ch[i], H);
      if (attn) x = b.transformer(x, pre + ".attentions." + std::to_string(j), c.heads[i], H);
      skips.push_back(x);
    }
    if (down) {
      x = b.conv3(x, pre + ".downsamplers.0.conv", ch[i], H, 2, 0, -1, -1);
      H /= 2;
      skips.push_back(x);
// ... 2 lines not shown
  x = b.resnet(x, "mid_block.resnets.0", ch[L - 1], H);
  x = b.transformer(x, "mid_block.attentions.0", c.heads[L - 1], H);
  x = b.resnet(x, "mid_block.resnets.1", ch[L - 1], H);
  int n_act = 0;
  for (int i = 0; i < L; ++i) {
    const std::string pre = "up_blocks." + std::to_string(i);
    const int co = ch[L - 1 - i];
    const bool attn = i > 0, up = i < L - 1;
    for (int j = 0; j < n + 1; ++j) {
      const int sk = skips.back();
      skips.pop_back();
      x = b.concat(x, sk);
      x = b.resnet(x, pre + ".resnets." + std::to_string(j), co, H);
      if (attn) x = b.transformer(x, pre + ".attentions." + std::to_string(j), c.heads[L - 1 - i], H);
    }
    if (up) {
      x = b.conv3(x, pre + ".upsamplers.0.conv", co, H, 1, 1, -1, -1);
      H *= 2;
    }
    if (attn && n_act < 3) {
      u.act_op_end[n_act] = (int)u.ops.size();
      u.act_ids[n_act++] = x;
    }
  }
  x = b.gn(x, "conv_norm_out", 1e-5f, true);
  u.t_final = x;
  { Op o;
    o.type = OP_CONV_OUT; o.in0 = x;
    o.wt = b.weight(c.out_channels, 9 * ch[0], 9, true, true);
    b.bind_mat("conv_out.weight", o.wt, c.out_channels, 0, ch[0], 9);
    o.bias_off = b.param_f32("conv_out.bias", c.out_channels);
    o.Hin = S; o.Cin = ch[0];
    u.ops.push_back(o); }
  if (b.temb_cursor != u.temb_total || b.kv_cursor != u.kv_total) {
    set_error("internal: fused projection sizes do not match");
    return DH_ERR_STATE;
  }
  u.first_cross_op = 0;
  for (size_t i = 0; i < u.ops.size(); ++i)
    if (u.ops[i].type == OP_ATTN && u.ops[i].cross) { u.first_cross_op = (int)i; break; }
  for (size_t i = 0; i + 1 < u.ops.size(); ++i) {
    Op& o = u.ops[i];
    const Op& nx = u.ops[i + 1];
    if (nx.type == OP_GN && nx.in0 == o.out && (o.type == OP_GEMM || o.type == OP_CONCAT)) o.gn_next = (int)(i + 1);
  }
  { int cmax = 0;
    for (const Op& o : u.ops) if (o.type == OP_LN) cmax = std::max(cmax, u.tens[o.in0].C);
    u.ones_off = (long)u.pf_elems; u.pf_elems += align_up((size_t)cmax, 64);
    u.zeros_off = (long)u.pf_elems; u.pf_elems += align_up((size_t)cmax, 64); }
  layout_tensors(u);
  size_t biggest = 0;
  for (const Ten& t : u.tens) biggest = std::max(biggest, (size_t)t.rows * t.C * c.max_diff_batch);
  u.scratch_elems = biggest * 4 + 1024;
  u.partial_elems = std::max<size_t>((size_t)48 << 20, biggest * 2);
  u.small_elems = (size_t)c.max_batch * 64 * 4096 + (size_t)c.max_batch * c.norm_groups * 4 + 4096;
  return DH_OK;
}


static void layout_tensors(dh_unet& u) {
  const size_t maxB = (size_t)u.cfg.max_batch, maxBd = (size_t)u.cfg.max_diff_batch;
  const int nt = (int)u.tens.size(), nops = (int)u.ops.size();
  u.tens[u.t_text].persistent = true;
  u.tens[u.t_kv].persistent = true;
  for (int i = 0; i < 3; ++i)
    if (u.act_ids[i] >= 0) u.tens[u.act_ids[i]].persistent = true;
  std::vector<int> first(nt, nops), last(nt, -1);
  auto rd = [&](int t, int oi) { if (t >= 0) { last[t] = std::max(last[t], oi); first[t] = std::min(first[t], oi); } };
  auto wr = [&](int t, int oi) { if (t >= 0) { first[t] = std::min(first[t], oi); last[t] = std::max(last[t], oi); } };
  for (int oi = 0; oi < nops; ++oi) {
    const Op& o = u.ops[oi];
    rd(o.in0, oi); rd(o.in1, oi); rd(o.res, oi); wr(o.out, oi);
    if (o.ln_fold >= 0) rd(u.ops[o.ln_fold].in0, oi);
    if (o.glu_op >= 0) wr(u.ops[o.glu_op].out, oi);
  }
  std::vector<char> written(nt, 0);
  for (const Op& o : u.ops) { if (o.out >= 0) written[o.out] = 1; if (o.glu_op >= 0) written[u.ops[o.glu_op].out] = 1; }
  for (int t = 0; t < nt; ++t)
    if (!written[t] || t == u.t_final) { first[t] = 0; last[t] = nops; u.tens[t].persistent = u.tens[t].persistent || !written[t]; }
  u.act_elems = 0; u.grad_elems = 0;
  for (Ten& t : u.tens) {
    t.off = u.act_elems;
    u.act_elems += align_up((size_t)t.rows * t.C * (t.persistent ? maxB : maxBd), 128);
    if (t.req_grad) { t.goff = u.grad_elems; u.grad_elems += align_up((size_t)t.rows * t.C * maxBd, 128); }
  }
  struct Live { size_t off, end; int last; };
  std::vector<Live> live;
  for (const Ten& t : u.tens)
    if (t.persistent) live.push_back({t.off, t.off + align_up((size_t)t.rows * t.C * maxB, 128), nops + 1});
  std::vector<int> order(nt);
  std::iota(order.begin(), order.end(), 0);
  std::stable_sort(order.begin(), order.end(), [&](int a, int b) { return first[a] < first[b]; });
  size_t fo_end = 0;
  for (const Live& l : live) fo_end = std::max(fo_end, l.end);
  for (int t : order) {
    Ten& tt = u.tens[t];
    if (tt.persistent) { tt.off_fo = tt.off; continue; }
    if (last[t] < 0) { tt.off_fo = 0; continue; }
    const size_t size = align_up((size_t)tt.rows * tt.C * maxB, 128);
    live.erase(std::remove_if(live.begin(), live.end(), [&](const Live& l) { return l.last < first[t]; }), live.end());
    std::sort(live.begin(), live.end(), [](const Live& a, const Live& b) { return a.off < b.off; });
    size_t pos = 0;
    for (const Live& l : live) {
      if (pos + size <= l.off) break;
      pos = std::max(pos, l.end);
    }
    tt.off_fo = pos;
    live.push_back({pos, pos + size, last[t]});
    fo_end = std::max(fo_end, pos + size);
  }
  u.fo_elems = fo_end;
  u.act_elems = std::max(u.act_elems, fo_end);
}

template <class D, bool TILED>
__global__ void k_load_weight(const float* src, int N, int C, int taps, D* fwd, long fwd_K, long row_off, D* bwd,
                              long bwd_K, long col_off, int Nb, float scale = 1.f, int glu_F = 0) {
  const size_t idx = (size_t)blockIdx.x * blockDim.x + threadIdx.x;
  if (idx >= (size_t)N * C * taps) return;
  const int tap = (int)(idx % taps);
  const int cc = (int)((idx / taps) % C);
  int nn = (int)(idx / ((size_t)taps * C));
  if (glu_F) nn = glu_col(nn >= glu_F ? nn - glu_F : nn, nn >= glu_F ? 1 : 0);
  const D v = from_f32<D>(src[idx] * scale);
  int fk = tap * C + cc, bk = (taps - 1 - tap) * Nb + (int)col_off + nn;
  if (TILED && taps == 9) { fk = conv_k_index(tap, cc); bk = conv_k_index(taps - 1 - tap, (int)col_off + nn); }
  const int fr = (int)row_off + nn;
  if (TILED) {
    fwd[wt_index(fr, fk, (int)fwd_K)] = v;
    if (bwd) bwd[wt_index(cc, bk, (int)bwd_K)] = v;
  } else {
    fwd[(size_t)fr * fwd_K + fk] = v;
    if (bwd) bwd[(size_t)cc * bwd_K + bk] = v;
  }
}

}
namespace dh {
void launch_load_weight(int dtype, const float* src, int N, int C, int taps, void* fwd, long fwd_K, long row_off, void* bwd,
                        long bwd_K, long col_off, int Nb, float scale, hipStream_t st) {
  const size_t total = (size_t)N * C * taps;
  const unsigned nb = (unsigned)((total + 255) / 256);
  if (dtype == DH_DTYPE_F32)
    hipLaunchKernelGGL((k_load_weight<float, false>), dim3(nb), dim3(256), 0, st, src, N, C, taps, (float*)fwd, fwd_K, row_off, (float*)bwd, bwd_K, col_off, Nb, scale);
  else if (dtype == DH_DTYPE_F16)
    hipLaunchKernelGGL((k_load_weight<f16, true>), dim3(nb), dim3(256), 0, st, src, N, C, taps, (f16*)fwd, fwd_K, row_off, (f16*)bwd, bwd_K, col_off, Nb, scale);
  else
    hipLaunchKernelGGL((k_load_weight<bf16, true>), dim3(nb), dim3(256), 0, st, src, N, C, taps, (bf16*)fwd, fwd_K, row_off, (bf16*)bwd, bwd_K, col_off, Nb, scale);
}
}
namespace {

template <class D>
__global__ void __launch_bounds__(256) k_fold_ln(const D* bwd, int bwd_K, const float* gamma, const float* beta, const float* bias,
                                                 D* fwd, int K, float* s_out, float* t_out) {
  __shared__ float sm[8];
  const int n = blockIdx.x;
  float s = 0.f, t = 0.f;
  for (int k = threadIdx.x; k < K; k += blockDim.x) {
    const float w = to_f32<D>(bwd[wt_index(k, n, bwd_K)]);
    const D wf = from_f32<D>(w * gamma[k]);
    fwd[wt_index(n, k, K)] = wf;
    s += to_f32<D>(wf);
    t += beta[k] * w;
  }
  s = block_sum(s, sm);
  __syncthreads();
  t = block_sum(t, sm);
  if (threadIdx.x == 0) { s_out[n] = s; t_out[n] = t + (bias ? bias[n] : 0.f); }
}

__global__ void k_load_glu_bias(const float* src, float* dst, int F) {
  const int n = blockIdx.x * blockDim.x + threadIdx.x;
  if (n < 2 * F) dst[n] = src[glu_src_row(n, F)];
}

__global__ void k_fill_f32(float* p, int n, float v) {
  const int i = blockIdx.x * blockDim.x + threadIdx.x;
  if (i < n) p[i] = v;
}

static bool use_ln_fold(const dh_unet* u, int B) {
#ifdef DH_TUNING
  static const long lim = getenv("DH_LN_FOLD_MAXROWS") ? atol(getenv("DH_LN_FOLD_MAXROWS")) : 12288;
#else
  constexpr long lim = 12288;
#endif
  return (long)B * u->cfg.sample_size * u->cfg.sample_size <= lim;
}

static void fold_layernorms(dh_unet* u, hipStream_t st) {
  { int cmax = 0;
    for (const Op& o : u->ops) if (o.type == OP_LN) cmax = std::max(cmax, u->tens[o.in0].C);
    if (cmax > 0) {
      hipLaunchKernelGGL(k_fill_f32, dim3(cdiv(cmax, 256)), dim3(256), 0, st, u->pf + u->ones_off, cmax, 1.f);
      hipLaunchKernelGGL(k_fill_f32, dim3(cdiv(cmax, 256)), dim3(256), 0, st, u->pf + u->zeros_off, cmax, 0.f);
    } }
  for (const Op& g : u->ops) {
    if (g.type != OP_GEMM || g.ln_fold < 0) continue;
    const Op& l = u->ops[g.ln_fold];
    const Wt& w = u->wts[g.wt];
    const float* bias = g.bias_off >= 0 ? u->pf + g.bias_off : nullptr;
    if (u->dtype == DH_DTYPE_F16)
      hipLaunchKernelGGL((k_fold_ln<f16>), dim3(w.N), dim3(256), 0, st, (const f16*)(u->w16 + w.bwd_off), w.N, u->pf + l.gamma_off,
                         u->pf + l.beta_off, bias, (f16*)(u->w16 + w.fwd_off), w.K, u->pf + g.ln_s_off, u->pf + g.ln_t_off);
    else
      hipLaunchKernelGGL((k_fold_ln<bf16>), dim3(w.N), dim3(256), 0, st, (const bf16*)(u->w16 + w.bwd_off), w.N, u->pf + l.gamma_off,
                         u->pf + l.beta_off, bias, (bf16*)(u->w16 + w.fwd_off), w.K, u->pf + g.ln_s_off, u->pf + g.ln_t_off);
  }
  u->fold_dirty = false;
}

}

static int create_engine(const dh_unet_config* cfg, dh_unet* parent, dh_unet** out);
extern "C" int dh_unet_create(const dh_unet_config* cfg, dh_unet** out) {
  DH_REQUIRE(cfg && out, "null pointer");
  DH_REQUIRE(cfg->n_levels == 4, "n_levels must be 4");
  DH_REQUIRE(cfg->dtype == DH_DTYPE_F16 || cfg->dtype == DH_DTYPE_BF16, "dtype must be f16 or bf16");
  DH_REQUIRE(cfg->max_batch >= 1 && cfg->max_batch < 4096 && cfg->sample_size % 8 == 0 && cfg->sample_size >= 8, "bad batch / sample size");
  DH_REQUIRE((long)cfg->max_batch * cfg->sample_size * cfg->sample_size < (1L << 21), "max_batch * sample_size^2 must stay below 2^21 rows");
  DH_REQUIRE(cfg->norm_groups >= 1 && cfg->norm_groups <= 32, "1..32 GroupNorm groups");
  DH_REQUIRE(cfg->in_channels <= 8 && cfg->out_channels <= 8, "in/out channels must be <= 8");
  DH_REQUIRE(cfg->block_out_channels[0] <= 2048, "block_out_channels[0] must be <= 2048 (few-channel convolutions)");
  DH_REQUIRE(cfg->cross_attention_dim % 64 == 0, "cross_attention_dim must be a multiple of 64");
  for (int i = 0; i < 4; ++i) {
    DH_REQUIRE(cfg->block_out_channels[i] % 64 == 0, "block_out_channels must be multiples of 64");
    DH_REQUIRE(cfg->block_out_channels[i] == cfg->heads[i] * 64, "head dim must be 64");
    DH_REQUIRE(cfg->block_out_channels[i] % cfg->norm_groups == 0, "channels must divide into norm groups");
  }
  return create_engine(cfg, nullptr, out);
}

static int create_engine(const dh_unet_config* cfg, dh_unet* parent, dh_unet** out) {
  dh_unet* u = new dh_unet();
  u->cfg = *cfg;
  if (u->cfg.max_diff_batch <= 0 || u->cfg.max_diff_batch > u->cfg.max_batch) u->cfg.max_diff_batch = u->cfg.max_batch;
  u->dtype = cfg->dtype;
  int rc = build(*u);
  if (rc != DH_OK) { delete u; return rc; }
  auto fail = [&](hipError_t e, const char* what) {
    set_error(std::string(what) + ": " + hipGetErrorString(e));
    dh_unet_destroy(u);
    return DH_ERR_HIP;
  };
  hipError_t e;
  if (parent) {
    if (u->w16_elems != parent->w16_elems || u->pf_elems != parent->pf_elems) {
      set_error("internal: shared engine lays its parameters out differently");
      delete u;
      return DH_ERR_STATE;
    }
    u->owns_weights = false;
    u->w16 = parent->w16; u->pf = parent->pf;
    u->fold_dirty = false;
  } else {
    if ((e = hipMalloc((void**)&u->w16, u->w16_elems * 2 + 256)) != hipSuccess) return fail(e, "hipMalloc weights");
    if ((e = hipMalloc((void**)&u->pf, u->pf_elems * 4 + 256)) != hipSuccess) return fail(e, "hipMalloc f32 params");
  }
  if ((e = hipMalloc((void**)&u->act, u->act_elems * 2 + 256)) != hipSuccess) return fail(e, "hipMalloc activations");
  if ((e = hipMalloc((void**)&u->grad, u->grad_elems * 2 + 256)) != hipSuccess) return fail(e, "hipMalloc gradients");
  if ((e = hipMalloc((void**)&u->f32a, u->f32_elems * 4 + 256)) != hipSuccess) return fail(e, "hipMalloc f32 arena");
// ... 63 lines not shown
extern "C" int dh_unet_load_param(dh_unet* u, int i, const float* src, void* stream) {
  DH_REQUIRE(u && src && i >= 0 && i < (int)u->params.size(), "bad arguments");
  if (!u->owns_weights || u->n_shared > 0) {
    set_error("dh_unet_load_param: the weights are shared (dh_unet_create_shared): load every parameter before sharing");
    return DH_ERR_STATE;
  }
  u->temb_rows = 0; u->fold_dirty = true; u->kv_key = 0;
  hipStream_t st = (hipStream_t)stream;
  const ParamInfo& p = u->params[i];
  if (p.kind == PK_F32) {
    if (p.glu_F) {
      hipLaunchKernelGGL(k_load_glu_bias, dim3(cdiv((int)p.shape[0], 256)), dim3(256), 0, st, src, u->pf + p.f32_off, p.glu_F);
      DH_LAUNCH_CHECK();
      return DH_OK;
    }
    DH_CHECK_HIP(hipMemcpyAsync(u->pf + p.f32_off, src, (size_t)p.shape[0] * 4, hipMemcpyDeviceToDevice, st));
    return DH_OK;
  }
  const Wt& w = u->wts[p.wt];
  const int N = (int)p.shape[0], C = (int)p.shape[1], taps = w.taps;
  const size_t total = (size_t)N * C * taps;
  const unsigned nb = (unsigned)((total + 255) / 256);
  const long fwd_ld = w.K;
  const long bwd_ld = (long)taps * w.N;
  if (w.f32) {
    float* f = u->pf + w.fwd_off;
    float* b = w.has_bwd ? u->pf + w.bwd_off : nullptr;
    hipLaunchKernelGGL((k_load_weight<float, false>), dim3(nb), dim3(256), 0, st, src, N, C, taps, f, fwd_ld, (long)p.row_off,
                       b, bwd_ld, (long)p.row_off, w.N);
  } else if (u->dtype == DH_DTYPE_F16) {
    f16* f = (f16*)(u->w16 + w.fwd_off);
    f16* b = w.has_bwd ? (f16*)(u->w16 + w.bwd_off) : nullptr;
    hipLaunchKernelGGL((k_load_weight<f16, true>), dim3(nb), dim3(256), 0, st, src, N, C, taps, f, fwd_ld, (long)p.row_off, b,
                       bwd_ld, (long)p.row_off, w.N, 1.f, w.glu_F);
  } else {
    bf16* f = (bf16*)(u->w16 + w.fwd_off);
    bf16* b = w.has_bwd ? (bf16*)(u->w16 + w.bwd_off) : nullptr;
    hipLaunchKernelGGL((k_load_weight<bf16, true>), dim3(nb), dim3(256), 0, st, src, N, C, taps, f, fwd_ld, (long)p.row_off, b,
                       bwd_ld, (long)p.row_off, w.N, 1.f, w.glu_F);
  }
  DH_LAUNCH_CHECK();
  return DH_OK;
}

extern "C" size_t dh_unet_weight_bytes(const dh_unet* u) { return u && u->owns_weights ? u->w16_elems * 2 + u->pf_elems * 4 : 0; }
extern "C" size_t dh_unet_workspace_bytes(const dh_unet* u) {
  return u ? (u->act_elems + u->grad_elems + u->scratch_elems) * 2 + (u->f32_elems + u->partial_elems + u->small_elems) * 4 : 0;
}

static void fill_gemm(dh_unet* u, const Op& o, int B, GemmArgs& g) {
  const Wt& w = u->wts[o.wt];
  const Ten& ti = u->tens[o.in0];
  const Ten& to = u->tens[o.out];
  g.A = u->aptr(o.in0) + o.in_col; g.lda = ti.C;
  g.W = u->w16 + w.fwd_off;
  g.M = B * to.rows; g.N = w.N; g.K = w.K;
  g.mode = o.mode; g.Hin = o.Hin; g.Win = o.Win; g.Cin = o.Cin; g.Hout = o.Hout; g.Wout = o.Wout;
  g.stride = o.stride; g.up = o.up;
  g.bias = o.bias_off >= 0 ? u->pf + o.bias_off : nullptr;
  if (o.rowvec_off >= 0) { g.rowvec = u->f32a + o.rowvec_off; g.rowvec_ld = o.rowvec_ld; g.rows_per_batch = to.rows; }
  if (o.res >= 0) { g.R = u->aptr(o.res); g.ldr = u->tens[o.res].C; }
  g.C = u->aptr(o.out); g.ldc = to.C;
  g.act_silu = o.act_silu;
  g.partial = u->partial; g.partial_elems = u->partial_elems;
  if (o.ln_fold >= 0) {
    const Op& l = u->ops[o.ln_fold];
    if (use_ln_fold(u, B)) {
      g.A = u->aptr(l.in0); g.lda = u->tens[l.in0].C;
      g.bias = nullptr;
      g.ln_s = u->pf + o.ln_s_off; g.ln_t = u->pf + o.ln_t_off; g.ln_stats = u->f32a + l.stats_off; g.ln_eps = l.eps;
    } else {
      g.bias = u->pf + o.ln_t_off;
    }
  }
}

static void forward_ops(dh_unet* u, int B, int n_ops, int first_op, bool kv_hit, bool save, hipStream_t st) {
  const int dt = u->dtype;
  const dh_unet_config& c = u->cfg;
  u->flops_fwd = 0;
  int gn_have = 0;
  if (!kv_hit) launch_f32_to_t(dt, u->in_text, u->aptr(u->t_text), (size_t)B * c.text_len * c.cross_attention_dim, st);
  for (int oi = first_op; oi < n_ops; ++oi) {
    const Op& o = u->ops[oi];
    if (kv_hit && oi == u->temb_ops) continue;
    switch (o.type) {
      case OP_TIMESTEP:
        launch_timestep_embedding(dt, u->t_dev, c.block_out_channels[0], B, u->aptr(o.out), st);
        break;
      case OP_T2F:
        launch_t_to_f32(dt, u->aptr(o.in0), u->f32a + u->temb_f32_off, (size_t)B * u->temb_total, 0, st);
        break;
      case OP_CONV_IN: {
        const Wt& w = u->wts[o.wt];
        launch_conv_small_fwd(dt, u->in_sample, 1, u->pf + w.fwd_off, u->pf + o.bias_off, u->aptr(o.out), 0, B, o.Hin, o.Hin,
                              o.Cin, w.N, st);
        u->flops_fwd += 2.0 * B * o.Hin * o.Hin * w.N * w.K;
        break;
      }
      case OP_CONV_OUT: {
        const Wt& w = u->wts[o.wt];
        launch_conv_small_fwd(dt, u->aptr(o.in0), 0, u->pf + w.fwd_off, u->pf + o.bias_off, u->io_eps, 1, B, o.Hin, o.Hin,
                              o.Cin, w.N, st);
        u->flops_fwd += 2.0 * B * o.Hin * o.Hin * w.N * w.K;
        break;
      }
      case OP_GEMM: {
        GemmArgs g;
        fill_gemm(u, o, B, g);
        gn_have = 0;
        if (o.gn_next >= 0 && oi + 1 < n_ops) {
          const Ten& to = u->tens[o.out];
          g.gn_part = u->small; g.gn_HW = to.rows; g.gn_G = u->ops[o.gn_next].groups; g.gn_done = &gn_have;
        }
        if (o.glu_op >= 0 && o.glu_op < n_ops) {
          const Op& ge = u->ops[o.glu_op];
          g.glu_y = u->aptr(ge.out); g.glu_ldy = u->tens[ge.out].C;
          if (!save) g.C = nullptr;
        }
        u->flops_fwd += launch_gemm(dt, g, st);
        break;
      }
      case OP_GN: {
        const Ten& t = u->tens[o.in0];
        const int have = (oi > 0 && u->ops[oi - 1].gn_next == oi) ? gn_have : 0;
        launch_groupnorm_fwd(dt, u->aptr(o.in0), u->pf + o.gamma_off, u->pf + o.beta_off, u->aptr(o.out),
                             u->f32a + o.stats_off, u->small, B, t.rows, t.C, o.groups, o.eps, o.silu, st, have);
        gn_have = 0;
        break;
      }
      case OP_LN: {
        if (o.folded && use_ln_fold(u, B)) break;
        const Ten& t = u->tens[o.in0];
        launch_layernorm_fwd(dt, u->aptr(o.in0), u->pf + (o.folded ? u->ones_off : o.gamma_off),
                             u->pf + (o.folded ? u->zeros_off : o.beta_off), u->aptr(o.out),
                             u->f32a + o.stats_off, B * t.rows, t.C, o.eps, st);
        break;
      }
      case OP_ATTN: {
        const Ten& tq = u->tens[o.in0];
        const int C = u->tens[o.out].C;
        if (!o.cross) {
          const unsigned short* qkv = u->aptr(o.in0);
          launch_attention_fwd(dt, qkv, tq.C, qkv + C, qkv + 2 * C, tq.C, u->aptr(o.out), C, u->f32a + o.lse_off, B,
                               o.heads, o.Nq, o.Nk, st);
        } else {
          const Ten& tkv = u->tens[o.in1];
          const unsigned short* kv = u->aptr(o.in1) + o.kv_col;
          launch_attention_fwd(dt, u->aptr(o.in0), tq.C, kv, kv + C, tkv.C, u->aptr(o.out), C, u->f32a + o.lse_off, B,
                               o.heads, o.Nq, o.Nk, st);
        }
        u->flops_fwd += 4.0 * B * o.heads * (double)o.Nq * o.Nk * 64;
        break;
      }
      case OP_GEGLU: {
        if (oi > 0 && u->ops[oi - 1].glu_op == oi) break;
        const Ten& t = u->tens[o.out];
        launch_geglu_fwd(dt, u->aptr(o.in0), u->aptr(o.out), B * t.rows, t.C, st);
        break;
      }
      case OP_CONCAT: {
        const Ten &a = u->tens[o.in0], &b2 = u->tens[o.in1], &t = u->tens[o.out];
        gn_have = 0;
        const int G = o.gn_next >= 0 ? u->ops[o.gn_next].groups : 0;
        if (o.gn_next >= 0 && oi + 1 < n_ops && a.C % 8 == 0 && b2.C % 8 == 0 && t.C % G == 0 &&
            (GN_GB * (t.C / G)) % 8 == 0 && GN_GB * (t.C / G) <= 2048) {
          launch_concat_gn(dt, u->aptr(o.in0), a.C, u->aptr(o.in1), b2.C, u->aptr(o.out), u->small, B, t.rows, G, st);
          gn_have = 1;
        } else {
          launch_copy_cols(dt, u->aptr(o.in0), a.C, u->aptr(o.out), t.C, B * t.rows, a.C, 0, st);
          launch_copy_cols(dt, u->aptr(o.in1), b2.C, u->aptr(o.out) + a.C, t.C, B * t.rows, b2.C, 0, st);
        }
        break;
      }
    }
  }
}

static uint64_t graph_key_fwd(int B, int n_ops, bool temb_hit, bool kv_hit, bool save) {
  return (uint64_t)B | ((uint64_t)n_ops << 12) | ((uint64_t)(temb_hit ? 1 : 0) << 34) | ((uint64_t)(kv_hit ? 1 : 0) << 36) |
         ((uint64_t)(save ? 1 : 0) << 37);
}
static uint64_t graph_key_bwd(int B, unsigned mask, bool eps, bool sample, bool text) {
  return (uint64_t)B | ((uint64_t)(mask & 7u) << 28) | ((uint64_t)(eps ? 1 : 0) << 31) | ((uint64_t)(sample ? 1 : 0) << 32) |
         ((uint64_t)(text ? 1 : 0) << 33) | (1ull << 35);
}

template <class F>
static int run_graphed(dh_unet* u, uint64_t key, hipStream_t st, double* flops_slot, F body) {
// ... 75 lines not shown
  void add_into(int t, const unsigned short* src, long lds_, int cols, int col_off = 0) {
    const Ten& tt = u->tens[t];
    launch_copy_cols(dt, src, lds_, u->gptr(t) + col_off, tt.C, B * tt.rows, cols, u->gready[t] ? 1 : 0, st);
  }
};
}

static void backward_ops(dh_unet* u, int B, unsigned act_mask, bool has_eps, bool want_sample, bool want_text,
                         hipStream_t st) {
  const int dt = u->dtype;
  const dh_unet_config& c = u->cfg;
  const float* d_eps = has_eps ? u->io_eps : nullptr;
  float* d_sample = want_sample ? u->out_dsample : nullptr;
  float* d_text = want_text ? u->out_dtext : nullptr;
  u->flops_bwd = 0;
  std::fill(u->gready.begin(), u->gready.end(), 0);
  for (int i = 0; i < 3; ++i)
    if (act_mask & (1u << i)) u->gready[u->act_ids[i]] = 1;
  Bwd bw{u, B, dt, st, d_text != nullptr};
  bool text_grad_written = false;
  int gnb_have = 0, gnb_for = -1;
  int lnb_have = 0, lnb_for = -1;
  int cat_done = -1;
  int glub_done = -1;
  for (int oi = (int)u->ops.size() - 1; oi >= 0; --oi) {
    const Op& o = u->ops[oi];
    if (!want_sample && oi < u->first_cross_op && o.out != u->t_kv) continue;
    switch (o.type) {
      case OP_CONV_OUT: {
        if (!d_eps) break;
        const Wt& w = u->wts[o.wt];
        launch_conv_small_bwd(dt, d_eps, 1, u->pf + w.bwd_off, u->gptr(o.in0), 0, 0, B, o.Hin, o.Hin, w.N, o.Cin, st);
        u->gready[o.in0] = 1;
        u->flops_bwd += 2.0 * B * o.Hin * o.Hin * w.N * w.K;
        break;
      }
      case OP_CONV_IN: {
        if (!d_sample || !u->gready[o.out]) break;
        const Wt& w = u->wts[o.wt];
        launch_conv_small_bwd(dt, u->gptr(o.out), 0, u->pf + w.bwd_off, d_sample, 1, 0, B, o.Hin, o.Hin, w.N, o.Cin, st);
        u->flops_bwd += 2.0 * B * o.Hin * o.Hin * w.N * w.K;
        break;
      }
      case OP_GEMM: {
        if (!u->tens[o.out].req_grad || !u->gready[o.out]) break;
        const Ten& to = u->tens[o.out];
        const Ten& ti = u->tens[o.in0];
        const Wt& w = u->wts[o.wt];
        if (o.res >= 0 && u->tens[o.res].req_grad) {
          if (u->gready[o.res]) bw.add_into(o.res, u->gptr(o.out), to.C, to.C);
          else u->galias[o.res] = o.out;
          u->gready[o.res] = 1;
        }
        if (!ti.req_grad || !w.has_bwd) break;
        if (o.in0 == u->t_text && !bw.need_text) break;
        GemmArgs g;
        g.A = u->gptr(o.out); g.lda = to.C;
        g.W = u->w16 + w.bwd_off;
        g.partial = u->partial; g.partial_elems = u->partial_elems;
        if (o.mode == A_DENSE) {
          g.mode = A_DENSE;
          g.M = B * to.rows; g.N = w.K; g.K = w.N;
          g.C = u->gptr(o.in0) + o.in_col; g.ldc = ti.C;
          if (u->gready[o.in0]) { g.R = g.C; g.ldr = ti.C; }
          lnb_have = 0;
          if (oi > 0 && u->ops[oi - 1].type == OP_LN && u->ops[oi - 1].out == o.in0 && !u->gready[o.in0] && o.in_col == 0 &&
              w.K == ti.C) {
            const Op& ln = u->ops[oi - 1];
            g.lnb_x = u->aptr(ln.in0); g.lnb_gamma = u->pf + ln.gamma_off; g.lnb_stats = u->f32a + ln.stats_off;
            g.lnb_add = u->gready[ln.in0] ? u->gptr(ln.in0) : nullptr; g.lnb_dx = u->gptr(ln.in0);
            g.lnb_done = &lnb_have;
            lnb_for = oi - 1;
          }
          if (oi > 0 && u->ops[oi - 1].type == OP_GN && u->ops[oi - 1].out == o.in0 && !u->gready[o.in0] && o.in_col == 0 &&
              w.K == ti.C) {
            const Op& gn = u->ops[oi - 1];
            const Ten& tx = u->tens[gn.in0];
            g.gnb_x = u->aptr(gn.in0); g.gnb_ldx = tx.C;
            g.gnb_gamma = u->pf + gn.gamma_off; g.gnb_beta = u->pf + gn.beta_off; g.gnb_stats = u->f32a + gn.stats_off;
            g.gnb_silu = gn.silu;
            g.gn_part = u->small; g.gn_HW = tx.rows; g.gn_G = gn.groups; g.gn_done = &gnb_have;
            gnb_have = 0;
            gnb_for = oi - 1;
          }
          if (o.glub_op >= 0 && o.glub_op == oi - 1 && !u->gready[o.in0] && o.in_col == 0 && w.K == ti.C) {
            const Op& ge = u->ops[o.glub_op];
            g.glub_x = u->aptr(ge.in0); g.glub_dx = u->gptr(ge.in0); g.C = nullptr;
            u->gready[ge.in0] = 1;
            glub_done = o.glub_op;
          }
          u->flops_bwd += launch_gemm(dt, g, st);
          u->gready[o.in0] = 1;
        } else if (o.up) {
          g.mode = A_CONV3; g.stride = 1; g.up = 0;
          g.Hin = o.Hout; g.Win = o.Wout; g.Cin = w.N; g.Hout = o.Hout; g.Wout = o.Wout;
          g.M = B * o.Hout * o.Wout; g.N = o.Cin; g.K = 9 * w.N;
          g.C = u->scratch; g.ldc = o.Cin;
          u->flops_bwd += launch_gemm(dt, g, st);
          launch_pool2x2_sum(dt, u->scratch, u->gptr(o.in0), B, o.Hin, o.Win, o.Cin, u->gready[o.in0] ? 1 : 0, st);
          u->gready[o.in0] = 1;
        } else {
          g.mode = o.stride == 2 ? A_CONVT2 : A_CONV3;
          g.stride = 1; g.up = 0;
          g.Hin = o.Hout; g.Win = o.Wout; g.Cin = w.N;
          g.Hout = o.Hin; g.Wout = o.Win;
          g.M = B * o.Hin * o.Win; g.N = o.Cin; g.K = 9 * w.N;
          g.C = u->gptr(o.in0); g.ldc = ti.C;
          if (u->gready[o.in0]) { g.R = g.C; g.ldr = ti.C; }
          gnb_have = 0;
          int gi = -1;
          if (oi > 0 && u->ops[oi - 1].type == OP_GN && u->ops[oi - 1].out == o.in0) gi = oi - 1;
          else if (oi > 1 && u->ops[oi - 1].type == OP_GEMM && u->ops[oi - 1].mode == A_DENSE && u->ops[oi - 1].out == o.res &&
                   u->ops[oi - 1].in0 != o.in0 && u->ops[oi - 2].type == OP_GN && u->ops[oi - 2].out == o.in0)
            gi = oi - 2;
          if (gi >= 0) {
            const Op& gn = u->ops[gi];
            const Ten& tx = u->tens[gn.in0];
            g.gnb_x = u->aptr(gn.in0); g.gnb_ldx = tx.C;
            g.gnb_gamma = u->pf + gn.gamma_off; g.gnb_beta = u->pf + gn.beta_off; g.gnb_stats = u->f32a + gn.stats_off;
            g.gnb_silu = gn.silu;
            g.gn_part = u->small; g.gn_HW = tx.rows; g.gn_G = gn.groups; g.gn_done = &gnb_have;
            gnb_for = gi;
          }
          u->flops_bwd += launch_gemm(dt, g, st);
          u->gready[o.in0] = 1;
        }
        if (o.in0 == u->t_text) text_grad_written = true;
        break;
      }
      case OP_GN: {
        if (!u->gready[o.out]) break;
        const Ten& t = u->tens[o.in0];
        GnBwdSplit split;
        if (oi > 0 && u->ops[oi - 1].type == OP_CONCAT && u->ops[oi - 1].out == o.in0) {
          const Op& cat = u->ops[oi - 1];
          const int ca = u->tens[cat.in0].C;
          if (!u->gready[cat.in0] && !u->gready[cat.in1] && ca % 8 == 0 && ca + u->tens[cat.in1].C == t.C) {
            split.out0 = u->gptr(cat.in0); split.out1 = u->gptr(cat.in1); split.split_c = ca;
            cat_done = oi - 1;
          }
        }
        launch_groupnorm_bwd(dt, u->aptr(o.in0), u->gptr(o.out), u->pf + o.gamma_off, u->pf + o.beta_off,
                             u->f32a + o.stats_off, u->gptr(o.in0), u->small, B, t.rows, t.C, o.groups, o.silu,
                             u->gready[o.in0] ? 1 : 0, st, gnb_for == oi ? gnb_have : 0, split);
        gnb_have = 0;
        u->gready[o.in0] = 1;
        if (split.out0) { u->gready[u->ops[oi - 1].in0] = 1; u->gready[u->ops[oi - 1].in1] = 1; }
        break;
      }
      case OP_LN: {
        if (!u->gready[o.out]) break;
        if (lnb_have && lnb_for == oi) {
          lnb_have = 0;
          u->gready[o.in0] = 1;
          break;
        }
        const Ten& t = u->tens[o.in0];
        launch_layernorm_bwd(dt, u->aptr(o.in0), u->gptr(o.out), u->pf + o.gamma_off, u->f32a + o.stats_off,
                             u->gready[o.in0] ? u->gptr(o.in0) : nullptr, u->gptr(o.in0), B * t.rows, t.C, st);
        u->gready[o.in0] = 1;
        break;
      }
      case OP_GEGLU: {
        if (!u->gready[o.out]) break;
        if (glub_done == oi) { glub_done = -1; break; }
        const Ten& t = u->tens[o.out];
        launch_geglu_bwd(dt, u->aptr(o.in0), u->gptr(o.out), u->gptr(o.in0), B * t.rows, t.C, st);
        u->gready[o.in0] = 1;
        break;
      }
      case OP_ATTN: {
        if (!u->gready[o.out]) break;
        const Ten& tq = u->tens[o.in0];
        const int C = u->tens[o.out].C;
        float* delta = u->small;
        if (!o.cross) {
          const unsigned short* qkv = u->aptr(o.in0);
          unsigned short* dqkv = u->gptr(o.in0);
          launch_attention_bwd_dq(dt, qkv, tq.C, qkv + C, qkv + 2 * C, tq.C, u->aptr(o.out), C, u->gptr(o.out), C,
                                  u->f32a + o.lse_off, delta, dqkv, tq.C, B, o.heads, o.Nq, o.Nk, st);
          launch_attention_bwd_dkv(dt, qkv, tq.C, qkv + C, qkv + 2 * C, tq.C, u->gptr(o.out), C, u->f32a + o.lse_off,
                                   delta, dqkv + C, dqkv + 2 * C, tq.C, B, o.heads, o.Nq, o.Nk, st);
          u->flops_bwd += 14.0 * B * o.heads * (double)o.Nq * o.Nk * 64;
        } else {
          const Ten& tkv = u->tens[o.in1];
          const unsigned short* kv = u->aptr(o.in1) + o.kv_col;
          launch_attention_bwd_dq(dt, u->aptr(o.in0), tq.C, kv, kv + C, tkv.C, u->aptr(o.out), C, u->gptr(o.out), C,
                                  u->f32a + o.lse_off, delta, u->gptr(o.in0), tq.C, B, o.heads, o.Nq, o.Nk, st);
          u->flops_bwd += 6.0 * B * o.heads * (double)o.Nq * o.Nk * 64;
          if (bw.need_text) {
            unsigned short* dkv = u->gptr(o.in1) + o.kv_col;
            launch_attention_bwd_dkv(dt, u->aptr(o.in0), tq.C, kv, kv + C, tkv.C, u->gptr(o.out), C,
                                     u->f32a + o.lse_off, delta, dkv, dkv + C, tkv.C, B, o.heads, o.Nq, o.Nk, st, u->partial,
                                     u->partial_elems);
            u->gready[o.in1] = 1;
            u->flops_bwd += 8.0 * B * o.heads * (double)o.Nq * o.Nk * 64;
          }
        }
        u->gready[o.in0] = 1;
        break;
      }
      case OP_CONCAT: {
        if (!u->gready[o.out]) break;
        if (cat_done == oi) { cat_done = -1; break; }
        const Ten &a = u->tens[o.in0], &b2 = u->tens[o.in1], &t = u->tens[o.out];
        launch_split_cols(dt, u->gptr(o.out), t.C, u->gptr(o.in0), a.C, a.C, u->gready[o.in0] ? 1 : 0, u->gptr(o.in1), b2.C,
                          b2.C, u->gready[o.in1] ? 1 : 0, B * t.rows, st);
        u->gready[o.in0] = 1;
        u->gready[o.in1] = 1;
        break;
      }
      default: break;
// ... 53 lines not shown
    case DH_IO_DSAMPLE: *ptr = u->out_dsample; n = ns * c.in_channels * 4; break;
    case DH_IO_DTEXT: *ptr = u->out_dtext; n = nt * 4; break;
    case DH_IO_ACT:
    case DH_IO_ACT_GRAD: {
      DH_REQUIRE(index >= 0 && index < 3 && u->act_ids[index] >= 0, "activation index out of range");
      const Ten& t = u->tens[u->act_ids[index]];
      *ptr = which == DH_IO_ACT ? (void*)(u->act + t.off) : (void*)(u->grad + t.goff);
      n = (size_t)(which == DH_IO_ACT ? c.max_batch : c.max_diff_batch) * t.rows * t.C * 2;
      break;
    }
    default: DH_REQUIRE(false, "unknown buffer");
  }
  if (bytes) *bytes = n;
  return DH_OK;
}

extern "C" int dh_unet_set_text_key(dh_unet* u, unsigned long long key) {
  DH_REQUIRE(u, "null engine");
  u->text_key = key;
  return DH_OK;
}

extern "C" int dh_unet_stats(const dh_unet* u, double* flops_fwd, double* flops_bwd, int64_t* launches) {
  DH_REQUIRE(u, "null engine");
  if (flops_fwd) *flops_fwd = u->flops_fwd;
  if (flops_bwd) *flops_bwd = u->flops_bwd;
  if (launches) *launches = (int64_t)u->ops.size();
  return DH_OK;
}

extern "C" int dh_dbg_unet_concat_ops(const dh_unet_config* cfg, int* out, int cap, int* n_out) {
  DH_REQUIRE(cfg && n_out && (out || cap == 0), "null pointer");
  dh_unet u;
  u.cfg = *cfg;
  const int rc = build(u);
  if (rc != DH_OK) return rc;
  int n = 0;
  for (size_t i = 0; i < u.ops.size(); ++i) {
    const Op& o = u.ops[i];
    if (o.type != OP_CONCAT) continue;
    const Ten &a = u.tens[o.in0], &b = u.tens[o.in1], &t = u.tens[o.out];
    const int G = o.gn_next >= 0 ? u.ops[o.gn_next].groups : 0;
    const bool fused = o.gn_next >= 0 && i + 1 < u.ops.size() && a.C % 8 == 0 && b.C % 8 == 0 && t.C % G == 0 &&
                       (GN_GB * (t.C / G)) % 8 == 0 && GN_GB * (t.C / G) <= 2048;
    if (n < cap) {
      int* e = out + 5 * n;
      e[0] = a.C; e[1] = b.C; e[2] = t.rows; e[3] = G; e[4] = fused ? 1 : 0;
    }
    ++n;
  }
  *n_out = n;
  return DH_OK;
}
```

diffusionhandles_amd/csrc/unet_kernels.h:

```cpp
#pragma once
#include "common.h"

namespace dh {

__device__ inline float silu_grad(float z) {
  const float s = 1.f / (1.f + __expf(-z));
  return s * (1.f + z * (1.f - s));
}

struct GeluParts { float Phi, pdf; };
__device__ __forceinline__ GeluParts gelu_parts(float g) {
  const float x = fabsf(g) * 0.70710678118654752f;
  const float t = __builtin_amdgcn_rcpf(fmaf(0.3275911f, x, 1.f));
  const float e = __expf(-x * x);
  const float poly = t * (0.254829592f + t * (-0.284496736f + t * (1.421413741f + t * (-1.453152027f + t * 1.061405429f))));
  const float q = 0.5f * poly * e;
  return {g < 0.f ? q : 1.f - q, e * 0.3989422804014327f};
}
__device__ __forceinline__ float gelu_f(float g) { return g * gelu_parts(g).Phi; }
__device__ __forceinline__ float gelu_grad(float g) { const GeluParts p = gelu_parts(g); return fmaf(g, p.pdf, p.Phi); }
__host__ __device__ inline int glu_col(int o, int gate) { return 32 * (o >> 4) + 16 * gate + (o & 15); }
__host__ __device__ inline int glu_src_row(int n, int F) { return ((n >> 4) & 1) * F + 16 * (n >> 5) + (n & 15); }

enum { A_DENSE = 0, A_CONV3 = 1, A_CONVT2 = 2 };

struct GemmArgs {
  const void* A = nullptr; long lda = 0;
  const void* W = nullptr;
  int M = 0, N = 0, K = 0;
  int mode = A_DENSE;
  int Hin = 0, Win = 0, Cin = 0;
  int Hout = 0, Wout = 0;
  int stride = 1, up = 0;
  int pad = 1;
  const float* bias = nullptr;
  const float* rowvec = nullptr; int rowvec_ld = 0; int rows_per_batch = 1;
  const void* R = nullptr; long ldr = 0;
  void* C = nullptr; long ldc = 0;
  int act_silu = 0;
  float* partial = nullptr; size_t partial_elems = 0;
  float* gn_part = nullptr; int gn_HW = 0, gn_G = 0; int* gn_done = nullptr;
  const void* gnb_x = nullptr; long gnb_ldx = 0; const float *gnb_gamma = nullptr, *gnb_beta = nullptr, *gnb_stats = nullptr;
  int gnb_silu = 0;
  const float* ln_s = nullptr; const float* ln_t = nullptr; float* ln_stats = nullptr; float ln_eps = 1e-5f;
  const void* lnb_x = nullptr; const float *lnb_gamma = nullptr, *lnb_stats = nullptr; const void* lnb_add = nullptr;
  void* lnb_dx = nullptr; int* lnb_done = nullptr;
  void* glu_y = nullptr; long glu_ldy = 0;
  const void* glub_x = nullptr; void* glub_dx = nullptr;
};
void launch_splitk_reduce_ln_bwd(int dtype, const float* partial, int splits, const void* x, const float* gamma,
                                 const float* stats, const void* add, void* dx, int rows, int C, hipStream_t st);
double launch_gemm(int dtype, const GemmArgs& a, hipStream_t st);
bool gemm_profiling_on();
void launch_tile_weights(int dtype, const void* src, void* dst, int N, int K, hipStream_t st, int conv_cin = 0);
__host__ __device__ inline size_t wt_index(int n, int k, int K) {
  const int r = n & 63, c = (k & 63) >> 3;
  return ((size_t)(n >> 6) * (K >> 6) + (k >> 6)) * 4096 + (size_t)r * 64 + (size_t)((c ^ ((r >> 1) & 7)) << 3) + (k & 7);
}

__host__ __device__ inline int conv_k_index(int tap, int c) { return (c >> 6) * 576 + tap * 64 + (c & 63); }

void launch_load_weight(int dtype, const float* src, int N, int C, int taps, void* fwd, long fwd_K, long row_off, void* bwd,
                        long bwd_K, long col_off, int Nb, float scale, hipStream_t st);

void launch_conv_small_fwd(int dtype, const void* x, int x_is_f32, const float* w, const float* bias, void* y,
                           int y_is_f32, int B, int H, int W, int Cin, int Cout, hipStream_t st);
void launch_conv_small_bwd(int dtype, const void* dy, int dy_is_f32, const float* w, void* dx, int dx_is_f32,
                           int accumulate, int B, int H, int W, int Cin, int Cout, hipStream_t st);

void launch_groupnorm_fwd(int dtype, const void* x, const float* gamma, const float* beta, void* y, float* stats,
                          float* scratch, int B, int HW, int C, int G, float eps, int silu, hipStream_t st,
                          int have_partials = 0);
int gn_slices(int HW, int B);
constexpr int GN_GB = 4;
void launch_concat_gn(int dtype, const void* a, int Ca, const void* b, int Cb, void* out, float* gn_part, int B, int HW,
                      int G, hipStream_t st);
struct GnBwdSplit { void* out0 = nullptr; void* out1 = nullptr; int split_c = 0; };
void launch_groupnorm_bwd(int dtype, const void* x, const void* dy, const float* gamma, const float* beta,
                          const float* stats, void* dx, float* scratch, int B, int HW, int C, int G, int silu,
                          int accumulate, hipStream_t st, int have_partials = 0, GnBwdSplit split = GnBwdSplit());
void launch_gelu(int dtype, const void* x, void* y, size_t n, hipStream_t st);
void launch_layernorm_fwd(int dtype, const void* x, const float* gamma, const float* beta, void* y, float* stats,
                          int rows, int C, float eps, hipStream_t st);
void launch_layernorm_bwd(int dtype, const void* x, const void* dy, const float* gamma, const float* stats,
                          const void* add, void* dx, int rows, int C, hipStream_t st);
void launch_geglu_fwd(int dtype, const void* x, void* y, int rows, int F, hipStream_t st);
void launch_geglu_bwd(int dtype, const void* x, const void* dy, void* dx, int rows, int F, hipStream_t st);
void launch_copy_cols(int dtype, const void* src, long lds, void* dst, long ldd, int rows, int cols, int accumulate,
                      hipStream_t st);
void launch_split_cols(int dtype, const void* src, long lds, void* dstA, long ldA, int colsA, int accA, void* dstB, long ldB,
                       int colsB, int accB, int rows, hipStream_t st);
void launch_lane_ops_probe(const float* in, float* out, unsigned* ex, hipStream_t st);
void launch_pool2x2_sum(int dtype, const void* src, void* dst, int B, int h, int w, int C, int accumulate,
                        hipStream_t st);
void launch_f32_to_t(int dtype, const float* src, void* dst, size_t n, hipStream_t st);
void launch_t_to_f32(int dtype, const void* src, float* dst, size_t n, int accumulate, hipStream_t st);
void launch_timestep_embedding(int dtype, const float* t_dev, int dim, int B, void* out, hipStream_t st);
void launch_set_scalar(float* p, float v, hipStream_t st);

void launch_attention_fwd(int dtype, const void* q, long ldq, const void* k, const void* v, long ldk, void* o,
                          long ldo, float* lse, int B, int H, int Nq, int Nk, hipStream_t st, int causal = 0);
void launch_attention_delta(int dtype, const void* o, long ldo, const void* d_o, long lddo, float* delta, int B,
                            int H, int Nq, hipStream_t st);
void launch_attention_bwd_dq(int dtype, const void* q, long ldq, const void* k, const void* v, long ldk, const void* o,
                             long ldo, const void* d_o, long lddo, const float* lse, float* delta, void* dq, long lddq,
                             int B, int H, int Nq, int Nk, hipStream_t st);
void launch_attention_bwd_dkv(int dtype, const void* q, long ldq, const void* k, const void* v, long ldk,
                              const void* d_o, long lddo, const float* lse, const float* delta, void* dk, void* dv,
                              long lddk, int B, int H, int Nq, int Nk, hipStream_t st, float* scratch = nullptr,
                              size_t scratch_elems = 0);

}
```

diffusionhandles_amd/csrc/unet_kernels.hip:

```cpp
#include "unet_kernels.h"

namespace dh {

#ifdef DH_TUNING
static int ablate_mask() { static const int m = getenv("DH_ABLATE_SKIP") ? atoi(getenv("DH_ABLATE_SKIP")) : 0; return m; }
__global__ void k_noop() {}
static int ablate_empty() { static const int m = getenv("DH_ABLATE_EMPTY") ? atoi(getenv("DH_ABLATE_EMPTY")) : 0; return m; }
#define DH_ABLATE(bit) do { if (ablate_mask() & (bit)) { if (ablate_empty()) hipLaunchKernelGGL(k_noop, dim3(1), dim3(64), 0, st); return; } } while (0)
#else
#define DH_ABLATE(bit) do { } while (0)
#endif

constexpr int CF_PIX = 4;
template <class T>
__global__ void k_conv_few_in(const float* x, const float* w, const float* bias, T* y, int B, int H, int W, int Ci,
                              int Co) {
  __shared__ float patch[CF_PIX][9 * 8];
  const int K = 9 * Ci, total = B * H * W;
  const int p0 = blockIdx.x * CF_PIX;
  for (int i = threadIdx.x; i < CF_PIX * K; i += blockDim.x) {
    const int lp = i / K, k = i - lp * K, p = p0 + lp;
    float v = 0.f;
    if (p < total) {
      const int b = p / (H * W), r = p - b * H * W, oy = r / W, ox = r - oy * W;
// ... 479 lines not shown
      for (int gl = 0; gl < GN_GB; ++gl) pv[i] = gi[i] == gl ? pg[gl] : pv[i];
    }
    for (int r = r0 + rr; r < r1; r += RP) {
      const size_t m = (size_t)b * HW + r;
      const uint4 raw = load8(m, n);
      *reinterpret_cast<uint4*>(out + m * C + n) = raw;
      const T* v = reinterpret_cast<const T*>(&raw);
#pragma unroll
      for (int i = 0; i < 8; ++i) { const float d = to_f32<T>(v[i]) - pv[i]; av[i] += d; qv[i] += d * d; }
    }
#pragma unroll
    for (int i = 0; i < 8; ++i)
#pragma unroll
      for (int gl = 0; gl < GN_GB; ++gl) {
        ga[gl] += gi[i] == gl ? av[i] : 0.f;
        gq[gl] += gi[i] == gl ? qv[i] : 0.f;
      }
  }
#pragma unroll
  for (int gl = 0; gl < GN_GB; ++gl) { ga[gl] = wave_sum(ga[gl]); gq[gl] = wave_sum(gq[gl]); }
  if ((threadIdx.x & 63) == 0) {
#pragma unroll
    for (int gl = 0; gl < GN_GB; ++gl) { sm_red[threadIdx.x >> 6][2 * gl] = ga[gl]; sm_red[threadIdx.x >> 6][2 * gl + 1] = gq[gl]; }
  }
  __syncthreads();
  if ((int)threadIdx.x < GN_GB && g0 + (int)threadIdx.x < G) {
    const int gl = threadIdx.x, g = g0 + gl;
    float sa = 0.f, sq = 0.f;
    for (int w = 0; w < 4; ++w) { sa += sm_red[w][2 * gl]; sq += sm_red[w][2 * gl + 1]; }
    const float n = (float)(r1 - r0) * (float)cpg;
    float piv = 0.f;
#pragma unroll
    for (int k = 0; k < GN_GB; ++k) piv = gl == k ? pg[k] : piv;
    float* o = part + ((size_t)(b * G + g) * 3) * S + s;
    o[0] = n; o[S] = piv + sa / n; o[2 * S] = sq - sa * sa / n;
  }
}

void launch_concat_gn(int dtype, const void* a, int Ca, const void* b, int Cb, void* out, float* gn_part, int B, int HW,
                      int G, hipStream_t st) {
  DH_ABLATE(8);
  const int S = gn_slices(HW, B);
  dim3 grid(S, cdiv(G, GN_GB), B);
  if (dtype == DH_DTYPE_F16)
    hipLaunchKernelGGL((k_concat_gn<f16>), grid, dim3(256), 0, st, (const f16*)a, Ca, (const f16*)b, Cb, (f16*)out, gn_part, HW, G, S);
  else
    hipLaunchKernelGGL((k_concat_gn<bf16>), grid, dim3(256), 0, st, (const bf16*)a, Ca, (const bf16*)b, Cb, (bf16*)out, gn_part, HW, G, S);
}

constexpr int LN_MAXCH = 8;

template <class T, int NCH>
__global__ void __launch_bounds__(256, NCH <= 3 ? 4 : 1) k_ln_fwd(const T* x, const float* gamma, const float* beta, T* y, float* stats, int rows, int C,
                         float eps) {
  const int lane = threadIdx.x & 63;
  const int row = blockIdx.x * (blockDim.x >> 6) + (threadIdx.x >> 6);
  if (row >= rows) return;
  const int nch = C / 8;
  uint4 raw[NCH];
  float s = 0.f;
#pragma unroll
  for (int k = 0; k < NCH; ++k) {
    const int ch = lane + 64 * k;
    if (ch < nch) {
      raw[k] = *reinterpret_cast<const uint4*>(x + (size_t)row * C + ch * 8);
      const T* v = reinterpret_cast<const T*>(&raw[k]);
#pragma unroll
      for (int i = 0; i < 8; ++i) s += to_f32<T>(v[i]);
    }
  }
  const float mean = wave_sum(s) / (float)C;
  float q = 0.f;
#pragma unroll
  for (int k = 0; k < NCH; ++k) {
    const int ch = lane + 64 * k;
    if (ch < nch) {
      const T* v = reinterpret_cast<const T*>(&raw[k]);
#pragma unroll
      for (int i = 0; i < 8; ++i) { const float d = to_f32<T>(v[i]) - mean; q += d * d; }
    }
  }
  const float rstd = rsqrtf(wave_sum(q) / (float)C + eps);
  if (lane == 0 && stats) { stats[2 * (size_t)row] = mean; stats[2 * (size_t)row + 1] = rstd; }
#pragma unroll
  for (int k = 0; k < NCH; ++k) {
    const int ch = lane + 64 * k;
    if (ch < nch) {
      const T* v = reinterpret_cast<const T*>(&raw[k]);
      T o[8];
#pragma unroll
      for (int i = 0; i < 8; ++i) {
        const int c = ch * 8 + i;
        o[i] = from_f32<T>((to_f32<T>(v[i]) - mean) * rstd * gamma[c] + beta[c]);
      }
      *reinterpret_cast<uint4*>(y + (size_t)row * C + ch * 8) = *reinterpret_cast<uint4*>(o);
    }
  }
}

template <class T, int NCH>
__global__ void __launch_bounds__(256, NCH == 1 ? 8 : (NCH <= 3 ? 4 : 1)) k_ln_bwd(const T* x, const T* dy, const float* gamma, const float* stats,
                                                                  const T* add, T* dx, int rows, int C) {
  const int lane = threadIdx.x & 63;
  const int row = blockIdx.x * (blockDim.x >> 6) + (threadIdx.x >> 6);
  if (row >= rows) return;
  const int nch = C / 8;
  const size_t base = (size_t)row * C;
  uint4 rx[NCH], rd[NCH];
#pragma unroll
  for (int k = 0; k < NCH; ++k) {
    const int ch = lane + 64 * k;
    if (ch < nch) {
      rx[k] = *reinterpret_cast<const uint4*>(x + base + ch * 8);
      rd[k] = *reinterpret_cast<const uint4*>(dy + base + ch * 8);
    }
  }
  const float mean = stats[2 * (size_t)row], rstd = stats[2 * (size_t)row + 1];
  float s1 = 0.f, s2 = 0.f;
#pragma unroll
  for (int k = 0; k < NCH; ++k) {
    const int ch = lane + 64 * k;
    if (ch < nch) {
      const float4 g0 = *reinterpret_cast<const float4*>(gamma + ch * 8);
      const float4 g1 = *reinterpret_cast<const float4*>(gamma + ch * 8 + 4);
      const float g[8] = {g0.x, g0.y, g0.z, g0.w, g1.x, g1.y, g1.z, g1.w};
      const T* xv = reinterpret_cast<const T*>(&rx[k]);
      const T* dv = reinterpret_cast<const T*>(&rd[k]);
#pragma unroll
      for (int i = 0; i < 8; ++i) {
        const float xh = (to_f32<T>(xv[i]) - mean) * rstd;
        const float d = to_f32<T>(dv[i]) * g[i];
        s1 += d;
        s2 += d * xh;
      }
    }
  }
  s1 = wave_sum(s1) / (float)C;
  s2 = wave_sum(s2) / (float)C;
#pragma unroll
  for (int k = 0; k < NCH; ++k) {
    const int ch = lane + 64 * k;
    if (ch < nch) {
      const float4 g0 = *reinterpret_cast<const float4*>(gamma + ch * 8);
      const float4 g1 = *reinterpret_cast<const float4*>(gamma + ch * 8 + 4);
      const float g[8] = {g0.x, g0.y, g0.z, g0.w, g1.x, g1.y, g1.z, g1.w};
      uint4 ra = make_uint4(0, 0, 0, 0);
      if (add) ra = *reinterpret_cast<const uint4*>(add + base + ch * 8);
      const T* xv = reinterpret_cast<const T*>(&rx[k]);
      const T* dv = reinterpret_cast<const T*>(&rd[k]);
      const T* av = reinterpret_cast<const T*>(&ra);
      T o[8];
#pragma unroll
      for (int i = 0; i < 8; ++i) {
        const float xh = (to_f32<T>(xv[i]) - mean) * rstd;
        const float d = to_f32<T>(dv[i]) * g[i];
        float r = rstd * (d - s1 - xh * s2);
        if (add) r += to_f32<T>(av[i]);
        o[i] = from_f32<T>(r);
      }
      *reinterpret_cast<uint4*>(dx + base + ch * 8) = *reinterpret_cast<uint4*>(o);
    }
  }
}

template <class T, int NCH>
__global__ void __launch_bounds__(256, NCH == 1 ? 4 : (NCH <= 3 ? 2 : 1)) k_splitk_reduce_ln_bwd(const float* part, int splits, const T* x, const float* gamma,
                                                                       const float* stats, const T* add, T* dx, int rows, int C) {
  const int lane = threadIdx.x & 63;
  const int row = blockIdx.x * (blockDim.x >> 6) + (threadIdx.x >> 6);
  if (row >= rows) return;
  const int nch = C / 8;
  const size_t base = (size_t)row * C, slab = (size_t)rows * C;
  uint4 rx[NCH];
  float d[NCH][8];
#pragma unroll
  for (int k = 0; k < NCH; ++k) {
    const int ch = lane + 64 * k;
    if (ch < nch) rx[k] = *reinterpret_cast<const uint4*>(x + base + ch * 8);
#pragma unroll
    for (int i = 0; i < 8; ++i) d[k][i] = 0.f;
  }
  int z = 0;
  for (; z + 4 <= splits; z += 4) {
    float4 v[NCH][4][2];
#pragma unroll
    for (int k = 0; k < NCH; ++k) {
      const int ch = lane + 64 * k;
      if (ch < nch) {
#pragma unroll
        for (int j = 0; j < 4; ++j) {
          const float* p = part + (size_t)(z + j) * slab + base + ch * 8;
          v[k][j][0] = *reinterpret_cast<const float4*>(p);
          v[k][j][1] = *reinterpret_cast<const float4*>(p + 4);
        }
      }
    }
#pragma unroll
    for (int k = 0; k < NCH; ++k) {
      const int ch = lane + 64 * k;
      if (ch < nch) {
#pragma unroll
        for (int j = 0; j < 4; ++j) {
          d[k][0] += v[k][j][0].x; d[k][1] += v[k][j][0].y; d[k][2] += v[k][j][0].z; d[k][3] += v[k][j][0].w;
          d[k][4] += v[k][j][1].x; d[k][5] += v[k][j][1].y; d[k][6] += v[k][j][1].z; d[k][7] += v[k][j][1].w;
        }
      }
    }
  }
  for (; z < splits; ++z) {
#pragma unroll
    for (int k = 0; k < NCH; ++k) {
      const int ch = lane + 64 * k;
      if (ch < nch) {
        const float* p = part + (size_t)z * slab + base + ch * 8;
        const float4 a0 = *reinterpret_cast<const float4*>(p), a1 = *reinterpret_cast<const float4*>(p + 4);
        d[k][0] += a0.x; d[k][1] += a0.y; d[k][2] += a0.z; d[k][3] += a0.w;
        d[k][4] += a1.x; d[k][5] += a1.y; d[k][6] += a1.z; d[k][7] += a1.w;
      }
    }
  }
#pragma unroll
  for (int k = 0; k < NCH; ++k)
#pragma unroll
    for (int i = 0; i < 8; ++i) d[k][i] = to_f32<T>(from_f32<T>(d[k][i]));
  const float mean = stats[2 * (size_t)row], rstd = stats[2 * (size_t)row + 1];
  float s1 = 0.f, s2 = 0.f;
#pragma unroll
  for (int k = 0; k < NCH; ++k) {
    const int ch = lane + 64 * k;
    if (ch < nch) {
      const float4 g0 = *reinterpret_cast<const float4*>(gamma + ch * 8);
      const float4 g1 = *reinterpret_cast<const float4*>(gamma + ch * 8 + 4);
      const float g[8] = {g0.x, g0.y, g0.z, g0.w, g1.x, g1.y, g1.z, g1.w};
      const T* xv = reinterpret_cast<const T*>(&rx[k]);
#pragma unroll
      for (int i = 0; i < 8; ++i) {
        const float xh = (to_f32<T>(xv[i]) - mean) * rstd;
        d[k][i] *= g[i];
        s1 += d[k][i];
        s2 += d[k][i] * xh;
      }
    }
  }
  s1 = wave_sum(s1) / (float)C;
  s2 = wave_sum(s2) / (float)C;
#pragma unroll
  for (int k = 0; k < NCH; ++k) {
    const int ch = lane + 64 * k;
    if (ch < nch) {
      uint4 ra = make_uint4(0, 0, 0, 0);
      if (add) ra = *reinterpret_cast<const uint4*>(add + base + ch * 8);
      const T* xv = reinterpret_cast<const T*>(&rx[k]);
      const T* av = reinterpret_cast<const T*>(&ra);
      T o[8];
#pragma unroll
      for (int i = 0; i < 8; ++i) {
        const float xh = (to_f32<T>(xv[i]) - mean) * rstd;
        float r = rstd * (d[k][i] - s1 - xh * s2);
        if (add) r += to_f32<T>(av[i]);
        o[i] = from_f32<T>(r);
      }
      *reinterpret_cast<uint4*>(dx + base + ch * 8) = *reinterpret_cast<uint4*>(o);
    }
  }
}
void launch_splitk_reduce_ln_bwd(int dtype, const float* partial, int splits, const void* x, const float* gamma,
                                 const float* stats, const void* add, void* dx, int rows, int C, hipStream_t st) {
  const int wpb = rows <= 1024 ? 1 : 4;
#define DH_RLN(TT, N) hipLaunchKernelGGL((k_splitk_reduce_ln_bwd<TT, N>), dim3(cdiv(rows, wpb)), dim3(64 * wpb), 0, st, partial, splits, (const TT*)x, gamma, stats, (const TT*)add, (TT*)dx, rows, C)
  const int n = C <= 512 ? 1 : (C <= 1024 ? 2 : (C <= 1536 ? 3 : LN_MAXCH));
  if (dtype == DH_DTYPE_F16) {
    if (n == 1) DH_RLN(f16, 1); else if (n == 2) DH_RLN(f16, 2); else if (n == 3) DH_RLN(f16, 3); else DH_RLN(f16, LN_MAXCH);
  } else {
    if (n == 1) DH_RLN(bf16, 1); else if (n == 2) DH_RLN(bf16, 2); else if (n == 3) DH_RLN(bf16, 3); else DH_RLN(bf16, LN_MAXCH);
  }
#undef DH_RLN
}

void launch_layernorm_fwd(int dtype, const void* x, const float* gamma, const float* beta, void* y, float* stats,
                          int rows, int C, float eps, hipStream_t st) {
  DH_ABLATE(1);
#define DH_LN_FWD(TT, N) hipLaunchKernelGGL((k_ln_fwd<TT, N>), dim3(cdiv(rows, 4)), dim3(256), 0, st, (const TT*)x, gamma, beta, (TT*)y, stats, rows, C, eps)
  const int n = C <= 512 ? 1 : (C <= 1024 ? 2 : (C <= 1536 ? 3 : LN_MAXCH));
  if (dtype == DH_DTYPE_F16) {
    if (n == 1) DH_LN_FWD(f16, 1); else if (n == 2) DH_LN_FWD(f16, 2); else if (n == 3) DH_LN_FWD(f16, 3); else DH_LN_FWD(f16, LN_MAXCH);
  } else {
    if (n == 1) DH_LN_FWD(bf16, 1); else if (n == 2) DH_LN_FWD(bf16, 2); else if (n == 3) DH_LN_FWD(bf16, 3); else DH_LN_FWD(bf16, LN_MAXCH);
  }
#undef DH_LN_FWD
}
void launch_layernorm_bwd(int dtype, const void* x, const void* dy, const float* gamma, const float* stats,
                          const void* add, void* dx, int rows, int C, hipStream_t st) {
  DH_ABLATE(1);
  const int wpb = rows <= 1024 ? 1 : 4;
#define DH_LN_BWD(TT, N) hipLaunchKernelGGL((k_ln_bwd<TT, N>), dim3(cdiv(rows, wpb)), dim3(64 * wpb), 0, st, (const TT*)x, (const TT*)dy, gamma, stats, (const TT*)add, (TT*)dx, rows, C)
  const int n = C <= 512 ? 1 : (C <= 1024 ? 2 : (C <= 1536 ? 3 : LN_MAXCH));
  if (dtype == DH_DTYPE_F16) {
    if (n == 1) DH_LN_BWD(f16, 1); else if (n == 2) DH_LN_BWD(f16, 2); else if (n == 3) DH_LN_BWD(f16, 3); else DH_LN_BWD(f16, LN_MAXCH);
  } else {
    if (n == 1) DH_LN_BWD(bf16, 1); else if (n == 2) DH_LN_BWD(bf16, 2); else if (n == 3) DH_LN_BWD(bf16, 3); else DH_LN_BWD(bf16, LN_MAXCH);
  }
#undef DH_LN_BWD
}


template <class T>
__global__ void k_geglu_fwd(const T* x, T* y, size_t rows, int F) {
  const size_t idx = (size_t)blockIdx.x * blockDim.x + threadIdx.x;
  const int fch = F / 8;
  if (idx >= rows * fch) return;
  const unsigned row32 = (unsigned)idx / (unsigned)fch;
  const size_t row = row32;
  const int j0 = (int)((unsigned)idx - row32 * (unsigned)fch) * 8;
  uint4 rh = *reinterpret_cast<const uint4*>(x + row * 2 * F + glu_col(j0, 0));
  uint4 rg = *reinterpret_cast<const uint4*>(x + row * 2 * F + glu_col(j0, 1));
  const T* h = reinterpret_cast<const T*>(&rh);
  const T* g = reinterpret_cast<const T*>(&rg);
  T o[8];
#pragma unroll
  for (int i = 0; i < 8; ++i) o[i] = from_f32<T>(to_f32<T>(h[i]) * gelu_f(to_f32<T>(g[i])));
  *reinterpret_cast<uint4*>(y + row * F + j0) = *reinterpret_cast<uint4*>(o);
}

template <class T>
__global__ void k_geglu_bwd(const T* x, const T* dy, T* dx, size_t rows, int F) {
  const size_t idx = (size_t)blockIdx.x * blockDim.x + threadIdx.x;
  const int fch = F / 8;
  if (idx >= rows * fch) return;
  const unsigned row32 = (unsigned)idx / (unsigned)fch;
  const size_t row = row32;
  const int j0 = (int)((unsigned)idx - row32 * (unsigned)fch) * 8;
  uint4 rh = *reinterpret_cast<const uint4*>(x + row * 2 * F + glu_col(j0, 0));
  uint4 rg = *reinterpret_cast<const uint4*>(x + row * 2 * F + glu_col(j0, 1));
  uint4 rd = *reinterpret_cast<const uint4*>(dy + row * F + j0);
  const T* h = reinterpret_cast<const T*>(&rh);
  const T* g = reinterpret_cast<const T*>(&rg);
  const T* d = reinterpret_cast<const T*>(&rd);
  T oh[8], og[8];
#pragma unroll
  for (int i = 0; i < 8; ++i) {
    const float gv = to_f32<T>(g[i]), dv = to_f32<T>(d[i]);
    oh[i] = from_f32<T>(dv * gelu_f(gv));
    og[i] = from_f32<T>(dv * to_f32<T>(h[i]) * gelu_grad(gv));
  }
  *reinterpret_cast<uint4*>(dx + row * 2 * F + glu_col(j0, 0)) = *reinterpret_cast<uint4*>(oh);
  *reinterpret_cast<uint4*>(dx + row * 2 * F + glu_col(j0, 1)) = *reinterpret_cast<uint4*>(og);
}

// ... 188 lines not shown
```

Measured before the change: 36.59 steps/s.

## Fold ff.net.2 and proj_out into one concatenated-K GEMM per transformer block

Algebraically merges the feed-forward output projection (ff.net.2) and the transformer proj_out linear into one GEMM. The GEGLU output and the attn2 output are written as column views of a shared 5C-wide buffer, and their weights are pre-multiplied and packed into a C x 5C matrix with a folded bias. This removes one GEMM launch and one intermediate activation round trip per block in both forward and backward. To support it, the GLU-backward epilogue gains a split mode where only the first F columns apply GEGLU backward and the rest act as a plain output. LayerNorm kernels also gain a leading-dimension stride so they can read the strided view. The cost is an extra fold and pack step whenever weights load, plus GEMMs with a larger K, and the pre-multiplied weights may change fp16 rounding.

```diff
diff --git a/diffusionhandles_amd/_lib.py b/diffusionhandles_amd/_lib.py
--- a/diffusionhandles_amd/_lib.py
+++ b/diffusionhandles_amd/_lib.py
@@ -122,6 +122,8 @@
     "dh_dbg_unet_concat_ops": (c_i, [ctypes.POINTER(UNetConfig), ctypes.POINTER(c_i), c_i, ctypes.POINTER(c_i)]),
     "dh_dbg_gemm_lnfold": (c_i, [c_i, c_p, c_l, c_p, c_i, c_i, c_i, c_p, c_p, c_p, c_f, c_p, c_l, c_p]),
     "dh_dbg_gemm_glu": (c_i, [c_i, c_i, c_p, c_l, c_p, c_i, c_i, c_i, c_p, c_p, c_p, c_p, c_p, c_p]),
+    "dh_dbg_gemm_glub_split": (c_i, [c_i, c_p, c_l, c_p, c_i, c_i, c_i, c_i, c_p, c_l, c_i, c_p, c_p, ctypes.POINTER(c_i), c_p]),
+    "dh_dbg_unet_ff_fold": (c_i, [c_p, c_i, ctypes.POINTER(c_i), ctypes.POINTER(c_i), c_p, c_p, c_p]),
     "dh_dbg_gemm_family": (c_i, [c_i]),
     "dh_dbg_gemm_stage": (c_i, [c_i]),
     "dh_dbg_gemm_pp_variant": (c_i, [c_i, c_p]),
diff --git a/diffusionhandles_amd/csrc/debug_api.cpp b/diffusionhandles_amd/csrc/debug_api.cpp
--- a/diffusionhandles_amd/csrc/debug_api.cpp
+++ b/diffusionhandles_amd/csrc/debug_api.cpp
@@ -159,6 +159,31 @@
   if (bwd) { g.glub_x = x; g.glub_dx = dx; }
   else { g.C = C; g.ldc = N; g.glu_y = y; g.glu_ldy = N / 2; }
   launch_gemm(dtype, g, (hipStream_t)stream);
+  DH_LAUNCH_CHECK();
+  return DH_OK;
+}
+extern "C" int dh_dbg_gemm_last_tile(int* out);
+extern "C" int dh_dbg_gemm_glub_split(int dtype, const void* A, long lda, const void* W, int M, int N, int K, int F, void* C,
+                                      long ldc, int accumulate, const void* x, void* dx, int* tile, void* stream) {
+  DH_REQUIRE(A && W && C && x && dx && K % 64 == 0 && N % 64 == 0 && F % 64 == 0 && F > 0 && F < N, "bad arguments (K, N, F % 64; 0 < F < N)");
+  static void* tiled = nullptr;
+  static size_t tiled_cap = 0;
+  const int Np = (int)align_up((size_t)N, 128);
+  const size_t need = (size_t)Np * K * 2;
+  if (need > tiled_cap) {
+    if (tiled) (void)hipFree(tiled);
+    DH_CHECK_HIP(hipMalloc(&tiled, need));
+    tiled_cap = need;
+  }
+  DH_CHECK_HIP(hipMemsetAsync(tiled, 0, need, (hipStream_t)stream));
+  launch_tile_weights(dtype, W, tiled, N, K, (hipStream_t)stream);
+  GemmArgs g;
+  g.A = A; g.lda = lda; g.W = tiled; g.M = M; g.N = N; g.K = K; g.mode = A_DENSE;
+  g.glub_x = x; g.glub_dx = dx; g.glub_f = F;
+  g.C = C; g.ldc = ldc;
+  if (accumulate) { g.R = C; g.ldr = ldc; }
+  launch_gemm(dtype, g, (hipStream_t)stream);
+  if (tile) dh_dbg_gemm_last_tile(tile);
   DH_LAUNCH_CHECK();
   return DH_OK;
 }
diff --git a/diffusionhandles_amd/csrc/gemm.hip b/diffusionhandles_amd/csrc/gemm.hip
--- a/diffusionhandles_amd/csrc/gemm.hip
+++ b/diffusionhandles_amd/csrc/gemm.hip
@@ -371,7 +371,8 @@
   DH_STAMP(1);
 
   constexpr bool PRE = TM * TN <= 8;
-  const bool pre_r = PRE && p.R != nullptr && p.pre_r && p.splits == 1 && (WG == 1 || grp == 0) && (KG == 1 || kg == 0);
+  const bool pre_r = PRE && p.R != nullptr && p.pre_r && p.splits == 1 && (WG == 1 || grp == 0) && (KG == 1 || kg == 0) &&
+                     (GLU != 2 || !glub_tile_is_glu(n0, p.glub_f));
   constexpr bool PRE_B = PRE && !(MW == 2 && BN == 320) && WNS == 2;
   const bool pre_b = PRE_B && p.bias != nullptr && p.pre_r && p.splits == 1;
   float4 bpre[PRE_B ? TN : 1][4];
@@ -610,11 +611,11 @@
     }
     return;
   }
-  if constexpr (GLU == 2) {
+  if (GLU == 2 && glub_tile_is_glu(n0, p.glub_f)) {
     typedef T T4 __attribute__((ext_vector_type(4)));
     const T* X = reinterpret_cast<const T*>(p.glub_x);
     T* DX = reinterpret_cast<T*>(p.glub_dx);
-    const size_t ldx = 2 * (size_t)p.N;
+    const size_t ldx = 2 * (size_t)p.glub_f;
     uint4 Hc[TM][TN][2], Gc[TM][TN][2];
 #pragma unroll
     for (int i = 0; i < TM; ++i) {
@@ -623,7 +624,7 @@
 #pragma unroll
       for (int j = 0; j < TN; ++j) {
         int nb = n0 + wn * CPW + j * 32;
-        if (nb >= p.N) nb = 0;
+        if (nb >= p.glub_f) nb = 0;
 #pragma unroll
         for (int q = 0; q < 2; ++q) {
           const T* src = X + (size_t)mc * ldx + 2 * nb + 32 * q + 8 * hi;
@@ -639,7 +640,7 @@
 #pragma unroll
       for (int j = 0; j < TN; ++j) {
         const int nb = n0 + wn * CPW + j * 32;
-        if (nb >= p.N) continue;
+        if (nb >= p.glub_f) continue;
 #pragma unroll
         for (int q = 0; q < 2; ++q) {
           const uint4 hc = Hc[i][j][q], gc = Gc[i][j][q];
@@ -1168,6 +1169,7 @@
   if (mw2) { BM = 256; BN = 128; }
   const int glu = k.glu_y ? 1 : (k.glub_x ? 2 : 0);
   if (glu && !(BM == 64 && BN == 64)) { BM = mw2 ? 256 : 128; BN = 128; }
+  if (glu == 2 && !glub_split_ok(BN, k.glub_f)) { BM = 64; BN = 64; }
   DH_KNOB(kT160, "DH_GEMM_T160", 224);
   const long tiles160 = (long)cdiv(k.M, 128) * (k.N / 160);
   const bool t160 = kT160 > 0 && k.N % 160 == 0 && !lnf && !glu && !n320 && BM != 64 && tiles160 >= kT160 && tiles160 <= 256;
@@ -1246,7 +1248,7 @@
     if (k.mode != A_DENSE && k.Hout > 0 && k.Wout > 0) a_elems = (double)k.M / ((double)k.Hout * k.Wout) * k.Hin * k.Win * k.Cin;
     double c_elems = (double)k.M * k.N * (k.C ? 1.0 : 0.0) + (k.R ? (double)k.M * k.N : 0.0);
     if (k.glu_y) c_elems += 0.5 * (double)k.M * k.N;
-    if (k.glub_x) c_elems += 4.0 * (double)k.M * k.N;
+    if (k.glub_x) c_elems += 4.0 * (double)k.M * k.glub_f - (k.C ? (double)k.M * k.glub_f : 0.0);
     if (k.gn_epi == 2) c_elems += (double)k.M * k.N;
     g_prof.bytes += esz * (a_elems + (double)k.N * k.K + c_elems);
     g_prof.e0 = e0; g_prof.e1 = e1;
@@ -1309,7 +1311,7 @@
       g_last_tile.reduce_gn = 1;
       if (gn_done) *gn_done = 1;
     } else if (k.lnb_x && lnb_done && !k.bias && !k.rowvec && !k.R && !k.act_silu && k.N % 8 == 0 && k.ldc == k.N) {
-      launch_splitk_reduce_ln_bwd(dtype, k.partial, splits, k.lnb_x, k.lnb_gamma, k.lnb_stats, k.lnb_add, k.lnb_dx, k.M, k.N, st);
+      launch_splitk_reduce_ln_bwd(dtype, k.partial, splits, k.lnb_x, k.lnb_gamma, k.lnb_stats, k.lnb_add, k.lnb_dx, k.M, k.N, st, k.lnb_ldx);
       *lnb_done = 1;
     } else {
       const size_t groups = (size_t)k.M * k.N / 4;
@@ -1335,8 +1337,16 @@
   k.gn_part = a.gn_part; k.gn_HW = a.gn_HW; k.gn_G = a.gn_G; k.gn_S = 0;
   k.gnb_x = a.gnb_x; k.gnb_ldx = a.gnb_ldx; k.gnb_gamma = a.gnb_gamma; k.gnb_beta = a.gnb_beta; k.gnb_stats = a.gnb_stats;
   k.gnb_silu = a.gnb_silu;
-  k.lnb_x = a.lnb_x; k.lnb_gamma = a.lnb_gamma; k.lnb_stats = a.lnb_stats; k.lnb_add = a.lnb_add; k.lnb_dx = a.lnb_dx;
+  k.lnb_x = a.lnb_x; k.lnb_ldx = a.lnb_ldx > 0 ? a.lnb_ldx : a.N;
+  k.lnb_gamma = a.lnb_gamma; k.lnb_stats = a.lnb_stats; k.lnb_add = a.lnb_add; k.lnb_dx = a.lnb_dx;
   k.glu_y = a.glu_y; k.glu_ldy = a.glu_ldy; k.glub_x = a.glub_x; k.glub_dx = a.glub_dx;
+  k.glub_f = a.glub_x && a.glub_f > 0 && a.glub_f < a.N ? a.glub_f : a.N;
+  if (k.glub_f < a.N) {
+    if (k.C) k.C = reinterpret_cast<unsigned short*>(k.C) - k.glub_f;
+    if (k.R) k.R = reinterpret_cast<const unsigned short*>(k.R) - k.glub_f;
+  } else if (a.glub_x) {
+    k.C = nullptr;
+  }
   if (a.gn_done) *a.gn_done = 0;
   if (a.lnb_done) *a.lnb_done = 0;
   if (dtype == DH_DTYPE_F16) gemm_dispatch<f16>(k, a.partial_elems, st, a.gn_done, a.lnb_done, dtype);
diff --git a/diffusionhandles_amd/csrc/gemm_k.h b/diffusionhandles_amd/csrc/gemm_k.h
--- a/diffusionhandles_amd/csrc/gemm_k.h
+++ b/diffusionhandles_amd/csrc/gemm_k.h
@@ -42,12 +42,16 @@
   float* gn_part; int gn_HW, gn_G, gn_S;
   int gn_epi, gn_cpg;
   const void* gnb_x; long gnb_ldx; const float *gnb_gamma, *gnb_beta, *gnb_stats; int gnb_silu;
-  const void* lnb_x; const float *lnb_gamma, *lnb_stats; const void* lnb_add; void* lnb_dx;
+  const void* lnb_x; long lnb_ldx; const float *lnb_gamma, *lnb_stats; const void* lnb_add; void* lnb_dx;
   void* glu_y; long glu_ldy; const void* glub_x; void* glub_dx;
+  int glub_f;
   int pp_tm, pp_tn, pp_order, pp_nwork; unsigned pp_a_bytes, pp_w_bytes;
   unsigned long long* pp_ts;
 };
 
+
+__host__ __device__ constexpr bool glub_tile_is_glu(int n0, int glub_f) { return n0 < glub_f; }
+__host__ __device__ constexpr bool glub_split_ok(int BN, int glub_f) { return BN > 0 && glub_f % BN == 0; }
 
 struct PpPlan { int bm = 0, bn = 0, splits = 1; };
 bool gemm_pp_plan(const GemmK& k, size_t partial_elems, int force, PpPlan* plan);
diff --git a/diffusionhandles_amd/csrc/gemm_pp.hip b/diffusionhandles_amd/csrc/gemm_pp.hip
--- a/diffusionhandles_amd/csrc/gemm_pp.hip
+++ b/diffusionhandles_amd/csrc/gemm_pp.hip
@@ -573,6 +573,7 @@
   const int glu = k.glu_y ? 1 : (k.glub_x ? 2 : 0);
   const bool glu_here = force == 2 || g_pp_glu > 0 || (g_pp_glu < 0 && ((glu == 1 && k.M >= 2048) || k.M >= 32768));
   if (glu && !glu_here) return false;
+  if (glu == 2 && k.glub_f > 0 && k.glub_f < k.N) return false;
   if (glu && (k.mode != A_DENSE || k.N % 128 || k.rowvec || k.R || (glu == 1 && (k.glu_ldy % 8 || ((size_t)k.glu_y & 15))) ||
               (glu == 2 && (((size_t)k.glub_x & 15) || ((size_t)k.glub_dx & 15))))) return false;
   if (k.rowvec && (k.rowvec_ld % 4 || ((size_t)k.rowvec & 15))) return false;
diff --git a/diffusionhandles_amd/csrc/unet_engine.cpp b/diffusionhandles_amd/csrc/unet_engine.cpp
--- a/diffusionhandles_amd/csrc/unet_engine.cpp
+++ b/diffusionhandles_amd/csrc/unet_engine.cpp
@@ -16,6 +16,8 @@
   size_t off = 0, goff = 0;
   size_t off_fo = 0;
   int rows = 0, C = 0;
+  int ld = 0;
+  int view = -1, col = 0;
   bool req_grad = true;
   bool persistent = false;
 };
@@ -56,6 +58,11 @@
   int glu_op = -1, glub_op = -1;
 };
 
+struct FfFold {
+  int wt_po = -1, wt_ffo = -1, wt = -1;
+  long b_po = -1, b_ffo = -1, bias = -1;
+};
+
 }
 
 using namespace dh;
@@ -67,6 +74,7 @@
   std::vector<Wt> wts;
   std::vector<ParamInfo> params;
   std::vector<Op> ops;
+  std::vector<FfFold> ffolds;
   std::map<std::string, int> pindex;
   size_t w16_elems = 0, pf_elems = 0, act_elems = 0, grad_elems = 0, f32_elems = 0;
   size_t fo_elems = 0;
@@ -117,9 +125,13 @@
 
   int tensor(int rows, int C, bool req_grad = true) {
     Ten t;
-    t.rows = rows; t.C = C; t.req_grad = req_grad;
+    t.rows = rows; t.C = C; t.ld = C; t.req_grad = req_grad;
     u.tens.push_back(t);
     return (int)u.tens.size() - 1;
+  }
+  void set_view(int t, int root, int col) {
+    Ten& tt = u.tens[t];
+    tt.view = root; tt.col = col; tt.ld = u.tens[root].C;
   }
   size_t f32_slot(size_t n) { size_t o = u.f32_elems; u.f32_elems += align_up(n, 64); return o; }
 
@@ -138,12 +150,12 @@
     u.pindex[name] = (int)u.params.size();
     u.params.push_back(p);
   }
-  int weight(int N, int K, int taps = 1, bool has_bwd = true, bool f32 = false) {
+  int weight(int N, int K, int taps = 1, bool has_bwd = true, bool f32 = false, bool pad_bwd = false) {
     Wt w;
     w.N = N; w.K = K; w.taps = taps; w.has_bwd = has_bwd; w.f32 = f32;
     size_t& arena = f32 ? u.pf_elems : u.w16_elems;
     w.fwd_off = arena; arena += align_up((size_t)N * K, 128);
-    if (has_bwd) { w.bwd_off = arena; arena += align_up((size_t)N * K, 128); }
+    if (has_bwd) { w.bwd_off = arena; arena += align_up((size_t)N * (pad_bwd ? align_up((size_t)K, 128) : (size_t)K), 128); }
     u.wts.push_back(w);
     return (int)u.wts.size() - 1;
   }
@@ -282,7 +294,9 @@
     c.out = tensor(N, C);
     c.lse_off = f32_slot((size_t)maxB * heads * N);
     u.ops.push_back(c);
+    const int tg = tensor(N, 5 * C, false);
     int t2 = linear(c.out, b + ".attn2.to_out.0", C, true, t1);
+    set_view(t2, tg, 4 * C);
     int n3 = ln(t2, b + ".norm3");
     int gg = linear(n3, b + ".ff.net.0.proj", 8 * C, true, -1);
     fold_ln_into_last_gemm();
@@ -292,11 +306,23 @@
     u.params[u.pindex[b + ".ff.net.0.proj.bias"]].glu_F = 4 * C;
     Op g;
     g.type = OP_GEGLU; g.in0 = gg; g.out = tensor(N, 4 * C);
+    set_view(g.out, tg, 0);
     u.ops.push_back(g);
     u.ops[ff1].glu_op = (int)u.ops.size() - 1;
-    int t3 = linear(g.out, b + ".ff.net.2", C, true, t2);
+    FfFold f;
+    f.wt_ffo = weight(C, 4 * C);
+    bind_mat(b + ".ff.net.2.weight", f.wt_ffo, C, 0, 4 * C, 1);
+    f.b_ffo = param_f32(b + ".ff.net.2.bias", C);
+    f.wt_po = weight(C, C, 1, false);
+    bind_mat(pre + ".proj_out.weight", f.wt_po, C, 0, C, 1);
+    f.b_po = param_f32(pre + ".proj_out.bias", C);
+    f.wt = weight(C, 5 * C, 1, true, false, true);
+    f.bias = (long)u.pf_elems; u.pf_elems += align_up((size_t)C, 64);
+    u.ffolds.push_back(f);
+    const int out = linear_w(tg, f.wt, f.bias, x);
     u.ops.back().glub_op = u.ops[ff1].glu_op;
-    return linear(t3, pre + ".proj_out", C, true, x);
+    u.ops.back().in1 = t2;
+    return out;
   }
 };
 
@@ -317,6 +343,7 @@
 }
 
 static void layout_tensors(dh_unet& u);
+static size_t ff_fold_scratch(int C);
 
 int build(dh_unet& u) {
   const dh_unet_config& c = u.cfg;
@@ -425,6 +452,7 @@
   size_t biggest = 0;
   for (const Ten& t : u.tens) biggest = std::max(biggest, (size_t)t.rows * t.C * c.max_diff_batch);
   u.scratch_elems = biggest * 4 + 1024;
+  for (const FfFold& f : u.ffolds) u.scratch_elems = std::max(u.scratch_elems, ff_fold_scratch(u.wts[f.wt_po].N));
   u.partial_elems = std::max<size_t>((size_t)48 << 20, biggest * 2);
   u.small_elems = (size_t)c.max_batch * 64 * 4096 + (size_t)c.max_batch * c.norm_groups * 4 + 4096;
   return DH_OK;
@@ -438,9 +466,10 @@
   u.tens[u.t_kv].persistent = true;
   for (int i = 0; i < 3; ++i)
     if (u.act_ids[i] >= 0) u.tens[u.act_ids[i]].persistent = true;
+  auto root = [&](int t) { return t >= 0 && u.tens[t].view >= 0 ? u.tens[t].view : t; };
   std::vector<int> first(nt, nops), last(nt, -1);
-  auto rd = [&](int t, int oi) { if (t >= 0) { last[t] = std::max(last[t], oi); first[t] = std::min(first[t], oi); } };
-  auto wr = [&](int t, int oi) { if (t >= 0) { first[t] = std::min(first[t], oi); last[t] = std::max(last[t], oi); } };
+  auto rd = [&](int t, int oi) { t = root(t); if (t >= 0) { last[t] = std::max(last[t], oi); first[t] = std::min(first[t], oi); } };
+  auto wr = [&](int t, int oi) { t = root(t); if (t >= 0) { first[t] = std::min(first[t], oi); last[t] = std::max(last[t], oi); } };
   for (int oi = 0; oi < nops; ++oi) {
     const Op& o = u.ops[oi];
     rd(o.in0, oi); rd(o.in1, oi); rd(o.res, oi); wr(o.out, oi);
@@ -448,13 +477,17 @@
     if (o.glu_op >= 0) wr(u.ops[o.glu_op].out, oi);
   }
   std::vector<char> written(nt, 0);
-  for (const Op& o : u.ops) { if (o.out >= 0) written[o.out] = 1; if (o.glu_op >= 0) written[u.ops[o.glu_op].out] = 1; }
+  for (const Op& o : u.ops) { if (o.out >= 0) written[root(o.out)] = 1; if (o.glu_op >= 0) written[root(u.ops[o.glu_op].out)] = 1; }
   for (int t = 0; t < nt; ++t)
-    if (!written[t] || t == u.t_final) { first[t] = 0; last[t] = nops; u.tens[t].persistent = u.tens[t].persistent || !written[t]; }
+    if (u.tens[t].view < 0 && (!written[t] || t == u.t_final)) {
+      first[t] = 0; last[t] = nops; u.tens[t].persistent = u.tens[t].persistent || !written[t];
+    }
   u.act_elems = 0; u.grad_elems = 0;
   for (Ten& t : u.tens) {
-    t.off = u.act_elems;
-    u.act_elems += align_up((size_t)t.rows * t.C * (t.persistent ? maxB : maxBd), 128);
+    if (t.view < 0) {
+      t.off = u.act_elems;
+      u.act_elems += align_up((size_t)t.rows * t.C * (t.persistent ? maxB : maxBd), 128);
+    }
     if (t.req_grad) { t.goff = u.grad_elems; u.grad_elems += align_up((size_t)t.rows * t.C * maxBd, 128); }
   }
   struct Live { size_t off, end; int last; };
@@ -468,6 +501,7 @@
   for (const Live& l : live) fo_end = std::max(fo_end, l.end);
   for (int t : order) {
     Ten& tt = u.tens[t];
+    if (tt.view >= 0) continue;
     if (tt.persistent) { tt.off_fo = tt.off; continue; }
     if (last[t] < 0) { tt.off_fo = 0; continue; }
     const size_t size = align_up((size_t)tt.rows * tt.C * maxB, 128);
@@ -484,6 +518,11 @@
   }
   u.fo_elems = fo_end;
   u.act_elems = std::max(u.act_elems, fo_end);
+  for (Ten& t : u.tens)
+    if (t.view >= 0) {
+      const Ten& r = u.tens[t.view];
+      t.off = r.off + t.col; t.off_fo = r.off_fo + t.col; t.persistent = r.persistent;
+    }
 }
 
 template <class D, bool TILED>
@@ -562,6 +601,58 @@
   return (long)B * u->cfg.sample_size * u->cfg.sample_size <= lim;
 }
 
+template <class D>
+__global__ void k_untile(const D* src, int N, int K, D* dst) {
+  const size_t idx = (size_t)blockIdx.x * blockDim.x + threadIdx.x;
+  if (idx >= (size_t)N * K) return;
+  const int n = (int)(idx / K), k = (int)(idx - (size_t)n * K);
+  dst[idx] = src[wt_index(n, k, K)];
+}
+template <class D>
+__global__ void k_pack_ff_fold(const D* prod, const D* po, int C, D* fwd, D* bwd) {
+  const size_t idx = (size_t)blockIdx.x * blockDim.x + threadIdx.x;
+  const int K = 5 * C;
+  if (idx >= (size_t)C * K) return;
+  const int n = (int)(idx / K), k = (int)(idx - (size_t)n * K);
+  const D v = k < 4 * C ? prod[(size_t)n * 4 * C + k] : po[(size_t)n * C + k - 4 * C];
+  fwd[wt_index(n, k, K)] = v;
+  bwd[wt_index(k, n, C)] = v;
+}
+template <class D>
+__global__ void __launch_bounds__(256) k_fold_ff_bias(const D* po, int C, const float* b_ffo, const float* b_po, float* out) {
+  __shared__ float sm[8];
+  const int n = blockIdx.x;
+  float s = 0.f;
+  for (int j = threadIdx.x; j < C; j += blockDim.x) s += to_f32<D>(po[(size_t)n * C + j]) * b_ffo[j];
+  s = block_sum(s, sm);
+  if (threadIdx.x == 0) out[n] = s + b_po[n];
+}
+
+static size_t ff_fold_scratch(int C) { return align_up((size_t)C * C, 128) + (size_t)4 * C * C; }
+
+template <class D>
+static void fold_ff_t(dh_unet* u, hipStream_t st) {
+  for (const FfFold& f : u->ffolds) {
+    const Wt& po = u->wts[f.wt_po];
+    const Wt& ffo = u->wts[f.wt_ffo];
+    const Wt& wf = u->wts[f.wt];
+    const int C = po.N;
+    D* po_plain = (D*)u->scratch;
+    D* prod = po_plain + align_up((size_t)C * C, 128);
+    hipLaunchKernelGGL((k_untile<D>), dim3(cdiv(C * C, 256)), dim3(256), 0, st, (const D*)(u->w16 + po.fwd_off), C, C, po_plain);
+    GemmArgs g;
+    g.A = po_plain; g.lda = C;
+    g.W = u->w16 + ffo.bwd_off;
+    g.mode = A_DENSE; g.M = C; g.N = 4 * C; g.K = C;
+    g.C = prod; g.ldc = 4 * C;
+    launch_gemm(u->dtype, g, st);
+    hipLaunchKernelGGL((k_pack_ff_fold<D>), dim3(cdiv(5 * C * C, 256)), dim3(256), 0, st, (const D*)prod, (const D*)po_plain, C,
+                       (D*)(u->w16 + wf.fwd_off), (D*)(u->w16 + wf.bwd_off));
+    hipLaunchKernelGGL((k_fold_ff_bias<D>), dim3(C), dim3(256), 0, st, (const D*)po_plain, C, u->pf + f.b_ffo, u->pf + f.b_po,
+                       u->pf + f.bias);
+  }
+}
+
 static void fold_layernorms(dh_unet* u, hipStream_t st) {
   { int cmax = 0;
     for (const Op& o : u->ops) if (o.type == OP_LN) cmax = std::max(cmax, u->tens[o.in0].C);
@@ -581,6 +672,8 @@
       hipLaunchKernelGGL((k_fold_ln<bf16>), dim3(w.N), dim3(256), 0, st, (const bf16*)(u->w16 + w.bwd_off), w.N, u->pf + l.gamma_off,
                          u->pf + l.beta_off, bias, (bf16*)(u->w16 + w.fwd_off), w.K, u->pf + g.ln_s_off, u->pf + g.ln_t_off);
   }
+  if (u->dtype == DH_DTYPE_F16) fold_ff_t<f16>(u, st);
+  else fold_ff_t<bf16>(u, st);
   u->fold_dirty = false;
 }
 
@@ -750,21 +843,21 @@
   const Wt& w = u->wts[o.wt];
   const Ten& ti = u->tens[o.in0];
   const Ten& to = u->tens[o.out];
-  g.A = u->aptr(o.in0) + o.in_col; g.lda = ti.C;
+  g.A = u->aptr(o.in0) + o.in_col; g.lda = ti.ld;
   g.W = u->w16 + w.fwd_off;
   g.M = B * to.rows; g.N = w.N; g.K = w.K;
   g.mode = o.mode; g.Hin = o.Hin; g.Win = o.Win; g.Cin = o.Cin; g.Hout = o.Hout; g.Wout = o.Wout;
   g.stride = o.stride; g.up = o.up;
   g.bias = o.bias_off >= 0 ? u->pf + o.bias_off : nullptr;
   if (o.rowvec_off >= 0) { g.rowvec = u->f32a + o.rowvec_off; g.rowvec_ld = o.rowvec_ld; g.rows_per_batch = to.rows; }
-  if (o.res >= 0) { g.R = u->aptr(o.res); g.ldr = u->tens[o.res].C; }
-  g.C = u->aptr(o.out); g.ldc = to.C;
+  if (o.res >= 0) { g.R = u->aptr(o.res); g.ldr = u->tens[o.res].ld; }
+  g.C = u->aptr(o.out); g.ldc = to.ld;
   g.act_silu = o.act_silu;
   g.partial = u->partial; g.partial_elems = u->partial_elems;
   if (o.ln_fold >= 0) {
     const Op& l = u->ops[o.ln_fold];
     if (use_ln_fold(u, B)) {
-      g.A = u->aptr(l.in0); g.lda = u->tens[l.in0].C;
+      g.A = u->aptr(l.in0); g.lda = u->tens[l.in0].ld;
       g.bias = nullptr;
       g.ln_s = u->pf + o.ln_s_off; g.ln_t = u->pf + o.ln_t_off; g.ln_stats = u->f32a + l.stats_off; g.ln_eps = l.eps;
     } else {
@@ -813,7 +906,7 @@
         }
         if (o.glu_op >= 0 && o.glu_op < n_ops) {
           const Op& ge = u->ops[o.glu_op];
-          g.glu_y = u->aptr(ge.out); g.glu_ldy = u->tens[ge.out].C;
+          g.glu_y = u->aptr(ge.out); g.glu_ldy = u->tens[ge.out].ld;
           if (!save) g.C = nullptr;
         }
         u->flops_fwd += launch_gemm(dt, g, st);
@@ -832,7 +925,7 @@
         const Ten& t = u->tens[o.in0];
         launch_layernorm_fwd(dt, u->aptr(o.in0), u->pf + (o.folded ? u->ones_off : o.gamma_off),
                              u->pf + (o.folded ? u->zeros_off : o.beta_off), u->aptr(o.out),
-                             u->f32a + o.stats_off, B * t.rows, t.C, o.eps, st);
+                             u->f32a + o.stats_off, B * t.rows, t.C, o.eps, st, t.ld);
         break;
       }
       case OP_ATTN: {
@@ -1014,6 +1107,22 @@
           else u->galias[o.res] = o.out;
           u->gready[o.res] = 1;
         }
+        if (o.glub_op >= 0 && o.in1 >= 0) {
+          const Op& ge = u->ops[o.glub_op];
+          const int t2 = o.in1;
+          GemmArgs g;
+          g.A = u->gptr(o.out); g.lda = to.C;
+          g.W = u->w16 + w.bwd_off;
+          g.mode = A_DENSE; g.M = B * to.rows; g.N = w.K; g.K = w.N;
+          g.partial = u->partial; g.partial_elems = u->partial_elems;
+          g.glub_x = u->aptr(ge.in0); g.glub_dx = u->gptr(ge.in0); g.glub_f = u->tens[ge.out].C;
+          g.C = u->gptr(t2); g.ldc = u->tens[t2].C;
+          if (u->gready[t2]) { g.R = g.C; g.ldr = g.ldc; }
+          u->flops_bwd += launch_gemm(dt, g, st);
+          u->gready[ge.in0] = 1; u->gready[ge.out] = 1; u->gready[t2] = 1;
+          glub_done = o.glub_op;
+          break;
+        }
         if (!ti.req_grad || !w.has_bwd) break;
         if (o.in0 == u->t_text && !bw.need_text) break;
         GemmArgs g;
@@ -1029,7 +1138,7 @@
           if (oi > 0 && u->ops[oi - 1].type == OP_LN && u->ops[oi - 1].out == o.in0 && !u->gready[o.in0] && o.in_col == 0 &&
               w.K == ti.C) {
             const Op& ln = u->ops[oi - 1];
-            g.lnb_x = u->aptr(ln.in0); g.lnb_gamma = u->pf + ln.gamma_off; g.lnb_stats = u->f32a + ln.stats_off;
+            g.lnb_x = u->aptr(ln.in0); g.lnb_ldx = u->tens[ln.in0].ld; g.lnb_gamma = u->pf + ln.gamma_off; g.lnb_stats = u->f32a + ln.stats_off;
             g.lnb_add = u->gready[ln.in0] ? u->gptr(ln.in0) : nullptr; g.lnb_dx = u->gptr(ln.in0);
             g.lnb_done = &lnb_have;
             lnb_for = oi - 1;
@@ -1038,18 +1147,12 @@
               w.K == ti.C) {
             const Op& gn = u->ops[oi - 1];
             const Ten& tx = u->tens[gn.in0];
-            g.gnb_x = u->aptr(gn.in0); g.gnb_ldx = tx.C;
+            g.gnb_x = u->aptr(gn.in0); g.gnb_ldx = tx.ld;
             g.gnb_gamma = u->pf + gn.gamma_off; g.gnb_beta = u->pf + gn.beta_off; g.gnb_stats = u->f32a + gn.stats_off;
             g.gnb_silu = gn.silu;
             g.gn_part = u->small; g.gn_HW = tx.rows; g.gn_G = gn.groups; g.gn_done = &gnb_have;
             gnb_have = 0;
             gnb_for = oi - 1;
-          }
-          if (o.glub_op >= 0 && o.glub_op == oi - 1 && !u->gready[o.in0] && o.in_col == 0 && w.K == ti.C) {
-            const Op& ge = u->ops[o.glub_op];
-            g.glub_x = u->aptr(ge.in0); g.glub_dx = u->gptr(ge.in0); g.C = nullptr;
-            u->gready[ge.in0] = 1;
-            glub_done = o.glub_op;
           }
           u->flops_bwd += launch_gemm(dt, g, st);
           u->gready[o.in0] = 1;
@@ -1078,7 +1181,7 @@
           if (gi >= 0) {
             const Op& gn = u->ops[gi];
             const Ten& tx = u->tens[gn.in0];
-            g.gnb_x = u->aptr(gn.in0); g.gnb_ldx = tx.C;
+            g.gnb_x = u->aptr(gn.in0); g.gnb_ldx = tx.ld;
             g.gnb_gamma = u->pf + gn.gamma_off; g.gnb_beta = u->pf + gn.beta_off; g.gnb_stats = u->f32a + gn.stats_off;
             g.gnb_silu = gn.silu;
             g.gn_part = u->small; g.gn_HW = tx.rows; g.gn_G = gn.groups; g.gn_done = &gnb_have;
@@ -1119,7 +1222,7 @@
         }
         const Ten& t = u->tens[o.in0];
         launch_layernorm_bwd(dt, u->aptr(o.in0), u->gptr(o.out), u->pf + o.gamma_off, u->f32a + o.stats_off,
-                             u->gready[o.in0] ? u->gptr(o.in0) : nullptr, u->gptr(o.in0), B * t.rows, t.C, st);
+                             u->gready[o.in0] ? u->gptr(o.in0) : nullptr, u->gptr(o.in0), B * t.rows, t.C, st, t.ld);
         u->gready[o.in0] = 1;
         break;
       }
@@ -1279,3 +1382,21 @@
   *n_out = n;
   return DH_OK;
 }
+
+extern "C" int dh_dbg_unet_ff_fold(dh_unet* u, int i, int* n_folds, int* C, void* w, float* bias, void* stream) {
+  DH_REQUIRE(u && n_folds && C, "null pointer");
+  hipStream_t st = (hipStream_t)stream;
+  *n_folds = (int)u->ffolds.size();
+  *C = 0;
+  if (i < 0 || i >= (int)u->ffolds.size()) return DH_OK;
+  if (u->fold_dirty) fold_layernorms(u, st);
+  const FfFold& f = u->ffolds[i];
+  const Wt& wf = u->wts[f.wt];
+  *C = wf.N;
+  if (w)
+    hipLaunchKernelGGL((k_untile<unsigned short>), dim3(cdiv(wf.N * wf.K, 256)), dim3(256), 0, st,
+                       (const unsigned short*)(u->w16 + wf.fwd_off), wf.N, wf.K, (unsigned short*)w);
+  if (bias) DH_CHECK_HIP(hipMemcpyAsync(bias, u->pf + f.bias, (size_t)wf.N * 4, hipMemcpyDeviceToDevice, st));
+  DH_LAUNCH_CHECK();
+  return DH_OK;
+}
diff --git a/diffusionhandles_amd/csrc/unet_kernels.h b/diffusionhandles_amd/csrc/unet_kernels.h
--- a/diffusionhandles_amd/csrc/unet_kernels.h
+++ b/diffusionhandles_amd/csrc/unet_kernels.h
@@ -43,13 +43,13 @@
   const void* gnb_x = nullptr; long gnb_ldx = 0; const float *gnb_gamma = nullptr, *gnb_beta = nullptr, *gnb_stats = nullptr;
   int gnb_silu = 0;
   const float* ln_s = nullptr; const float* ln_t = nullptr; float* ln_stats = nullptr; float ln_eps = 1e-5f;
-  const void* lnb_x = nullptr; const float *lnb_gamma = nullptr, *lnb_stats = nullptr; const void* lnb_add = nullptr;
+  const void* lnb_x = nullptr; long lnb_ldx = 0; const float *lnb_gamma = nullptr, *lnb_stats = nullptr; const void* lnb_add = nullptr;
   void* lnb_dx = nullptr; int* lnb_done = nullptr;
   void* glu_y = nullptr; long glu_ldy = 0;
-  const void* glub_x = nullptr; void* glub_dx = nullptr;
+  const void* glub_x = nullptr; void* glub_dx = nullptr; int glub_f = 0;
 };
 void launch_splitk_reduce_ln_bwd(int dtype, const float* partial, int splits, const void* x, const float* gamma,
-                                 const float* stats, const void* add, void* dx, int rows, int C, hipStream_t st);
+                                 const float* stats, const void* add, void* dx, int rows, int C, hipStream_t st, long ldx = 0);
 double launch_gemm(int dtype, const GemmArgs& a, hipStream_t st);
 bool gemm_profiling_on();
 void launch_tile_weights(int dtype, const void* src, void* dst, int N, int K, hipStream_t st, int conv_cin = 0);
@@ -81,9 +81,9 @@
                           int accumulate, hipStream_t st, int have_partials = 0, GnBwdSplit split = GnBwdSplit());
 void launch_gelu(int dtype, const void* x, void* y, size_t n, hipStream_t st);
 void launch_layernorm_fwd(int dtype, const void* x, const float* gamma, const float* beta, void* y, float* stats,
-                          int rows, int C, float eps, hipStream_t st);
+                          int rows, int C, float eps, hipStream_t st, long ldx = 0);
 void launch_layernorm_bwd(int dtype, const void* x, const void* dy, const float* gamma, const float* stats,
-                          const void* add, void* dx, int rows, int C, hipStream_t st);
+                          const void* add, void* dx, int rows, int C, hipStream_t st, long ldx = 0);
 void launch_geglu_fwd(int dtype, const void* x, void* y, int rows, int F, hipStream_t st);
 void launch_geglu_bwd(int dtype, const void* x, const void* dy, void* dx, int rows, int F, hipStream_t st);
 void launch_copy_cols(int dtype, const void* src, long lds, void* dst, long ldd, int rows, int cols, int accumulate,
diff --git a/diffusionhandles_amd/csrc/unet_kernels.hip b/diffusionhandles_amd/csrc/unet_kernels.hip
--- a/diffusionhandles_amd/csrc/unet_kernels.hip
+++ b/diffusionhandles_amd/csrc/unet_kernels.hip
@@ -555,7 +555,7 @@
 
 template <class T, int NCH>
 __global__ void __launch_bounds__(256, NCH <= 3 ? 4 : 1) k_ln_fwd(const T* x, const float* gamma, const float* beta, T* y, float* stats, int rows, int C,
-                         float eps) {
+                         float eps, long ldx) {
   const int lane = threadIdx.x & 63;
   const int row = blockIdx.x * (blockDim.x >> 6) + (threadIdx.x >> 6);
   if (row >= rows) return;
@@ -566,7 +566,7 @@
   for (int k = 0; k < NCH; ++k) {
     const int ch = lane + 64 * k;
     if (ch < nch) {
-      raw[k] = *reinterpret_cast<const uint4*>(x + (size_t)row * C + ch * 8);
+      raw[k] = *reinterpret_cast<const uint4*>(x + (size_t)row * ldx + ch * 8);
       const T* v = reinterpret_cast<const T*>(&raw[k]);
 #pragma unroll
       for (int i = 0; i < 8; ++i) s += to_f32<T>(v[i]);
@@ -603,18 +603,18 @@
 
 template <class T, int NCH>
 __global__ void __launch_bounds__(256, NCH == 1 ? 8 : (NCH <= 3 ? 4 : 1)) k_ln_bwd(const T* x, const T* dy, const float* gamma, const float* stats,
-                                                                  const T* add, T* dx, int rows, int C) {
+                                                                  const T* add, T* dx, int rows, int C, long ldx) {
   const int lane = threadIdx.x & 63;
   const int row = blockIdx.x * (blockDim.x >> 6) + (threadIdx.x >> 6);
   if (row >= rows) return;
   const int nch = C / 8;
-  const size_t base = (size_t)row * C;
+  const size_t base = (size_t)row * C, xbase = (size_t)row * ldx;
   uint4 rx[NCH], rd[NCH];
 #pragma unroll
   for (int k = 0; k < NCH; ++k) {
     const int ch = lane + 64 * k;
     if (ch < nch) {
-      rx[k] = *reinterpret_cast<const uint4*>(x + base + ch * 8);
+      rx[k] = *reinterpret_cast<const uint4*>(x + xbase + ch * 8);
       rd[k] = *reinterpret_cast<const uint4*>(dy + base + ch * 8);
     }
   }
@@ -668,7 +668,7 @@
 
 template <class T, int NCH>
 __global__ void __launch_bounds__(256, NCH == 1 ? 4 : (NCH <= 3 ? 2 : 1)) k_splitk_reduce_ln_bwd(const float* part, int splits, const T* x, const float* gamma,
-                                                                       const float* stats, const T* add, T* dx, int rows, int C) {
+                                                                       const float* stats, const T* add, T* dx, int rows, int C, long ldx) {
   const int lane = threadIdx.x & 63;
   const int row = blockIdx.x * (blockDim.x >> 6) + (threadIdx.x >> 6);
   if (row >= rows) return;
@@ -679,7 +679,7 @@
 #pragma unroll
   for (int k = 0; k < NCH; ++k) {
     const int ch = lane + 64 * k;
-    if (ch < nch) rx[k] = *reinterpret_cast<const uint4*>(x + base + ch * 8);
+    if (ch < nch) rx[k] = *reinterpret_cast<const uint4*>(x + (size_t)row * ldx + ch * 8);
 #pragma unroll
     for (int i = 0; i < 8; ++i) d[k][i] = 0.f;
   }
@@ -768,9 +768,10 @@
   }
 }
 void launch_splitk_reduce_ln_bwd(int dtype, const float* partial, int splits, const void* x, const float* gamma,
-                                 const float* stats, const void* add, void* dx, int rows, int C, hipStream_t st) {
+                                 const float* stats, const void* add, void* dx, int rows, int C, hipStream_t st, long ldx) {
+  if (ldx <= 0) ldx = C;
   const int wpb = rows <= 1024 ? 1 : 4;
-#define DH_RLN(TT, N) hipLaunchKernelGGL((k_splitk_reduce_ln_bwd<TT, N>), dim3(cdiv(rows, wpb)), dim3(64 * wpb), 0, st, partial, splits, (const TT*)x, gamma, stats, (const TT*)add, (TT*)dx, rows, C)
+#define DH_RLN(TT, N) hipLaunchKernelGGL((k_splitk_reduce_ln_bwd<TT, N>), dim3(cdiv(rows, wpb)), dim3(64 * wpb), 0, st, partial, splits, (const TT*)x, gamma, stats, (const TT*)add, (TT*)dx, rows, C, ldx)
   const int n = C <= 512 ? 1 : (C <= 1024 ? 2 : (C <= 1536 ? 3 : LN_MAXCH));
   if (dtype == DH_DTYPE_F16) {
     if (n == 1) DH_RLN(f16, 1); else if (n == 2) DH_RLN(f16, 2); else if (n == 3) DH_RLN(f16, 3); else DH_RLN(f16, LN_MAXCH);
@@ -781,9 +782,10 @@
 }
 
 void launch_layernorm_fwd(int dtype, const void* x, const float* gamma, const float* beta, void* y, float* stats,
-                          int rows, int C, float eps, hipStream_t st) {
+                          int rows, int C, float eps, hipStream_t st, long ldx) {
   DH_ABLATE(1);
-#define DH_LN_FWD(TT, N) hipLaunchKernelGGL((k_ln_fwd<TT, N>), dim3(cdiv(rows, 4)), dim3(256), 0, st, (const TT*)x, gamma, beta, (TT*)y, stats, rows, C, eps)
+  if (ldx <= 0) ldx = C;
+#define DH_LN_FWD(TT, N) hipLaunchKernelGGL((k_ln_fwd<TT, N>), dim3(cdiv(rows, 4)), dim3(256), 0, st, (const TT*)x, gamma, beta, (TT*)y, stats, rows, C, eps, ldx)
   const int n = C <= 512 ? 1 : (C <= 1024 ? 2 : (C <= 1536 ? 3 : LN_MAXCH));
   if (dtype == DH_DTYPE_F16) {
     if (n == 1) DH_LN_FWD(f16, 1); else if (n == 2) DH_LN_FWD(f16, 2); else if (n == 3) DH_LN_FWD(f16, 3); else DH_LN_FWD(f16, LN_MAXCH);
@@ -793,10 +795,11 @@
 #undef DH_LN_FWD
 }
 void launch_layernorm_bwd(int dtype, const void* x, const void* dy, const float* gamma, const float* stats,
-                          const void* add, void* dx, int rows, int C, hipStream_t st) {
+                          const void* add, void* dx, int rows, int C, hipStream_t st, long ldx) {
   DH_ABLATE(1);
+  if (ldx <= 0) ldx = C;
   const int wpb = rows <= 1024 ? 1 : 4;
-#define DH_LN_BWD(TT, N) hipLaunchKernelGGL((k_ln_bwd<TT, N>), dim3(cdiv(rows, wpb)), dim3(64 * wpb), 0, st, (const TT*)x, (const TT*)dy, gamma, stats, (const TT*)add, (TT*)dx, rows, C)
+#define DH_LN_BWD(TT, N) hipLaunchKernelGGL((k_ln_bwd<TT, N>), dim3(cdiv(rows, wpb)), dim3(64 * wpb), 0, st, (const TT*)x, (const TT*)dy, gamma, stats, (const TT*)add, (TT*)dx, rows, C, ldx)
   const int n = C <= 512 ? 1 : (C <= 1024 ? 2 : (C <= 1536 ? 3 : LN_MAXCH));
   if (dtype == DH_DTYPE_F16) {
     if (n == 1) DH_LN_BWD(f16, 1); else if (n == 2) DH_LN_BWD(f16, 2); else if (n == 3) DH_LN_BWD(f16, 3); else DH_LN_BWD(f16, LN_MAXCH);
```

Measured after the change: 37.66 steps/s (median of 6 runs). +2.9%, better.
